# octree-nn/octfusion

Hardware: AMD Instinct MI355X
Metric: denoising-steps/sec (depth-8 octree, batch 8) (higher is better)
Workload: dtype f32 storage, fp16x3 products (fp16 hi + lo operand pairs = 22 significand bits, three fp16 MFMAs per product, fp32 accumulate)

## Files before the change

include/ofx.h:

```cpp
#ifndef OFX_H_
#define OFX_H_

#include <stddef.h>
#include <stdint.h>

#ifdef __cplusplus
extern "C" {
#endif

#define OFX_OK 0
#define OFX_EINVAL (-1)
#define OFX_ELAUNCH (-2)
#define OFX_ENODEV (-3)

#define OFX_ACT_NONE 0
#define OFX_ACT_SILU 1
#define OFX_ACT_GELU 2

#define OFX_MAX_DEPTH 16

int ofx_version(void);
const char* ofx_status_string(int status);
int ofx_device_check(void);
const char* ofx_build_hash(void);
// ... 58 lines not shown
int ofx_graph_reverse_count(const int32_t* seg_ptr, const int32_t* col, int64_t n_nodes, int32_t* rev_cnt,
                            void* stream);
int ofx_graph_reverse_fill(const int32_t* seg_ptr, const int32_t* col, int64_t n_nodes, const int32_t* rev_ptr,
                           int32_t* cursor, int32_t* rev_row, float* rev_w, void* stream);
int ofx_graph_primary_w(const int32_t* seg_ptr, const int32_t* col, const float* w, int64_t n_nodes, int32_t* nbr,
                        void* stream);
int ofx_graph_multi_flag_w(const int32_t* seg_ptr, const float* w, int64_t n_nodes, int32_t* flag, void* stream);
int ofx_graph_primary_ext_w(const int32_t* seg_ptr, const int32_t* col, const float* w, int64_t n_nodes,
                            const int32_t* rank, int32_t* nbr_ext, int32_t* multi_seg, void* stream);
int ofx_graphconv_bwd_data(const float* dy, int64_t ldy, int cout, int64_t n_nodes, const int32_t* nbr_rev,
                           const int32_t* rev_ptr, const int32_t* rev_row, const float* rev_w,
                           const int32_t* nbr_ext_rev, const int32_t* multi_seg, int64_t n_multi, float* aux,
                           const float* WpT, int64_t KpT, int cin, float* dx, int64_t ldx, void* ws, size_t ws_bytes,
                           void* stream);
int ofx_graphconv_bwd_weight(const float* x, int64_t ldx, int cin, int64_t n_nodes, const int32_t* nbr,
                             const int32_t* seg_ptr, const int32_t* col, const int32_t* nbr_ext,
                             const int32_t* multi_seg, int64_t n_multi, float* aux, const float* type_frac, int64_t ldt,
                             int nt_pad, const float* dy, int64_t ldy, int cout, float* dWp, int64_t Kp, void* ws,
                             size_t ws_bytes, void* stream);
int ofx_gn_backward(const float* x, int64_t ldx, const float* dy, int64_t ldy, int64_t n, int C,
                    const int32_t* batch_id, int batch_size, const float* count, int groups, float count_eps,
                    const float* mean, const float* rstd, const float* w, const float* bias, int act, double* sums,
                    float* coef, float* dx, int64_t lddx, float* dgamma, float* dbeta, void* stream);
int ofx_gemm_tn_f32(const float* P, int64_t ldp, const float* Q, int64_t ldq, int64_t rows, int64_t K, int64_t N,
                    float* out, void* ws, size_t ws_bytes, void* stream);
int ofx_table_reverse_count(const int32_t* nbr, int64_t n_out, int ndir, int64_t n_in, int32_t* rev_cnt, void* stream);
int ofx_table_reverse_fill(const int32_t* nbr, int64_t n_out, int ndir, int64_t n_in, const int32_t* rev_ptr,
                           int32_t* cursor, int32_t* rev_row, float* rev_w, void* stream);
int ofx_seg_primary_w(const int32_t* seg_ptr, const int32_t* col, const float* w, int64_t nseg, int32_t* nbr,
                      void* stream);
int ofx_seg_multi_flag_w(const int32_t* seg_ptr, const float* w, int64_t nseg, int32_t* flag, void* stream);
int ofx_seg_primary_ext_w(const int32_t* seg_ptr, const int32_t* col, const float* w, int64_t nseg, int64_t n_src,
                          const int32_t* rank, int32_t* nbr_ext, int32_t* multi_seg, void* stream);
int ofx_gridconv_bwd_data(const float* dy, int64_t ldy, int cout, int64_t n_out, int64_t n_in, const int32_t* nbr_rev,
                          const int32_t* rev_ptr, const int32_t* rev_row, const float* rev_w,
                          const int32_t* nbr_ext_rev, const int32_t* multi_seg, int64_t n_multi, float* aux,
                          const float* WpT, int cin, float* dx, int64_t ldx, void* ws, size_t ws_bytes, void* stream);
int ofx_gridconv_bwd_weight(const float* x, int64_t ldx, int cin, int64_t n_in, int64_t n_out, const int32_t* nbr27,
                            const int32_t* nbr27_ext, const float* zero_row, const float* dy, int64_t ldy, int cout,
                            float* dWp, void* ws, size_t ws_bytes, void* stream);
int ofx_adamw_step(float* param, const float* grad, float* exp_avg, float* exp_avg_sq, int64_t n, float lr,
                   float beta1, float beta2, float eps, float weight_decay, int step, void* stream);
int ofx_ema_update(float* ema, const float* param, int64_t n, float beta, void* stream);
int ofx_mpu_eval(const ofx_tree_t* tree, int depth_start, int depth_end, const float* pts, int64_t n_pts,
                 const float* code, float* sdf, uint8_t* mask, void* stream);
int ofx_mpu_eval_grid(const ofx_tree_t* tree, int depth_start, int depth_end, const float* code, int size,
                      float step, float bbmin, int batch_index, int64_t head, int64_t count, float* sdf,
                      uint8_t* mask, void* stream);
int ofx_mpu_eval_grad(const ofx_tree_t* tree, int depth_start, int depth_end, const float* pts, int64_t n_pts,
                      const float* code, float* sdf, float* grad, uint8_t* mask, void* stream);
int ofx_mpu_backward(const ofx_tree_t* tree, int depth_start, int depth_end, const float* pts, int64_t n_pts,
                     const float* code, const float* dsdf, const float* dgrad, float* dcode, void* stream);
int ofx_octree_ce(const float* logits, int64_t ld, const int32_t* child, int64_t n, float dscale, double* sums,
                  float* dlogits, int64_t ldd, void* stream);
int ofx_sdf_reg_loss(const float* sdf, const float* grad, const float* sdf_gt, const float* grad_gt, int64_t n,
                     float w_sdf, float w_grad, double* sums, float* dsdf, float* dgrad, void* stream);
int ofx_kl_sample_fwd(const float* params, int64_t ld, const float* noise, int64_t n, int embed_dim, float* z,
                      double* kl_sum, void* stream);
int ofx_kl_sample_bwd(const float* params, int64_t ld, const float* noise, const float* dz, int64_t n,
                      int embed_dim, float kl_scale, float* dparams, int64_t ldp, void* stream);
int ofx_graph_multi_flag(const int32_t* seg_ptr, int64_t n_nodes, int32_t* flag, void* stream);
int ofx_graph_primary_ext(const int32_t* seg_ptr, const int32_t* col, int64_t n_nodes,
                          const int32_t* rank, int32_t* nbr_ext, int32_t* multi_seg, void* stream);
int ofx_graph_type_frac(const int32_t* seg_ptr, const int32_t* col, const uint8_t* node_type,
                        int64_t n_nodes, int nt, float* type_frac, int64_t ld, void* stream);

int ofx_set_precision(int mode);
int ofx_get_precision(void);
int64_t ofx_packed_floats(int64_t Kp, int64_t N);
int64_t ofx_packed_k(int64_t K);
int64_t ofx_graphconv_packed_k(int cin, int nt);
int ofx_pack_weights(const float* W, int64_t sk, int64_t sn, int64_t K, int64_t N,
                     int cin, int nt, float* Wp, int64_t Kp, void* stream);

int ofx_gemm_f32(const float* A, int64_t lda, const int32_t* a_rows, int64_t M, int64_t K,
                 const float* Wp, int64_t Kp, int64_t N, const float* bias,
                 const float* res, int64_t ldr, float* out, int64_t ldc,
                 const int32_t* out_rows, void* ws, size_t ws_bytes, void* stream);
int ofx_gemm_f32_planes(const float* A, int64_t lda, const int32_t* a_rows, int64_t M, int64_t K,
                        const float* Wp, int64_t Kp, int64_t N, const float* bias,
                        const float* res, int64_t ldr, float* out, int64_t ldc,
                        const int32_t* out_rows, void* ws, size_t ws_bytes, int out_mode, void* stream);

int ofx_graphconv_fwd(const float* x, int64_t ldx, int cin, int64_t n_nodes,
                      const int32_t* nbr, const int32_t* seg_ptr, const int32_t* col,
                      const int32_t* nbr_ext, const int32_t* multi_seg, int64_t n_multi, float* aux,
                      const float* type_frac, int64_t ldt, int nt_pad,
                      const float* Wp, int64_t Kp, int cout, const float* bias,
                      const float* emb, int64_t lde, const int32_t* batch_id,
                      const float* res, int64_t ldr, float* out, int64_t ldc,
                      double* stats , int64_t stats_ld,
                      void* ws, size_t ws_bytes, void* stream);

int ofx_graphconv_narrow_in(const float* x, int64_t ldx, int cin, int64_t n_nodes, const int32_t* seg_ptr,
                            const int32_t* col, const uint8_t* node_type, int nt, const float* W, int cout,
                            const float* bias, const int32_t* batch_id, float* out, int64_t ldc,
                            double* stats , int64_t stats_ld, void* ws, size_t ws_bytes, void* stream);
int ofx_graphconv_narrow_in_tab(const float* x, int64_t ldx, int cin, int64_t n_nodes, const int32_t* seg_ptr,
                                const int32_t* col, const int32_t* nbr_ext, const int32_t* multi_seg, int64_t n_multi,
                                void* aux, const uint8_t* node_type, int nt, const float* W, int cout, const float* bias,
                                const int32_t* batch_id, float* out, int64_t ldc, double* stats ,
                                int64_t stats_ld, void* ws, size_t ws_bytes, void* stream);
int ofx_narrow_out_pack(const float* W, int C, int nt, int cout, int pw, float* Wd, void* stream);
int ofx_narrow_out_type_term(const float* type_frac, int64_t ldt, int nt, int64_t n_nodes, const float* W, int C,
                             int cout, const float* bias, float* type_term, void* stream);
int ofx_graphconv_narrow_out(const float* P, int64_t ldp, int cout, int64_t n_nodes, const int32_t* seg_ptr,
                             const int32_t* col, const float* type_term , float* out, int64_t ldc,
                             void* stream);

int ofx_planes_split(const float* x, int64_t ldx, int64_t n, int C, int Cpad, int mode, void* out,
                     int64_t ldo_bytes, void* stream);
int ofx_planes_merge(const void* planes, int64_t ldp_bytes, int64_t n, int C, int mode, float* out, int64_t ldo,
                     void* stream);
int ofx_gn_apply_planes(const float* x, int64_t ldx, int64_t n, int C, const int32_t* batch_id, const float* mean,
                        const float* rstd, const double* sums, const float* count, int groups, float eps,
                        float count_eps, const float* w, const float* bias, int act, int mode, void* out,
                        int64_t ldo_bytes, const int32_t* seg_ptr, const int32_t* col, const int32_t* multi_seg,
                        int64_t n_multi, void* aux , const int32_t* aux_plan ,
                        int64_t aux_left, void* stream);
int ofx_gn_apply_planes_oct(const float* x, int64_t ldx, int64_t n, int C, const int32_t* batch_id, const float* mean,
                            const float* rstd, const double* sums, const float* count, int groups, float eps,
                            float count_eps, const float* w, const float* bias, int act, int mode, void* out,
                            int64_t ldo_bytes, int64_t n_multi, void* aux, const int32_t* oct_ptr,
                            const int32_t* oct_ent, int64_t n_own, int shift, const int32_t* left_head,
                            const int32_t* left_src, int64_t n_left, void* stream);
int ofx_gn_apply_rows(void);
int64_t ofx_planes_packed_ktiles(int cin, int nt, int mode);
int64_t ofx_planes_packed_bytes(int cin, int nt, int cout, int mode);
int ofx_pack_weights_planes(const float* W, int64_t sk, int64_t sn, int cin, int nt, int cout, int mode, void* out,
                            void* stream);
int ofx_graphconv_fwd_planes(const void* xp, int64_t ldx_bytes, int cin, int64_t n_nodes, const int32_t* seg_ptr,
                             const int32_t* col, const int32_t* nbr_ext, const int32_t* multi_seg, int64_t n_multi,
                             void* aux, size_t aux_bytes, const void* tfp, int64_t ldt_bytes, int nt, const void* W2,
                             int cout, const float* bias, const float* emb, int64_t lde, const int32_t* batch_id,
                             const float* res, int64_t ldr, float* out, int64_t ldc, double* stats ,
                             int64_t stats_ld, void* ws, size_t ws_bytes, void* sync , size_t sync_bytes,
                             int mode, int aux_ready, void* stream);
int ofx_set_gconv_persistent(int on);
int64_t ofx_gemm_planes_packed_bytes(int K, int N, int mode);
int ofx_pack_gemm_planes(const float* W, int64_t sk, int64_t sn, int K, int N, int mode, void* out, void* stream);
int ofx_gemm_planes(const void* ap, int64_t lda_bytes, int64_t n_a, int64_t M, int K, const int32_t* row_tab,
                    const void* W2, int N, const float* bias, float* out, int64_t ldc, int out_mode, void* ws,
                    size_t ws_bytes, void* sync, size_t sync_bytes, int mode, void* stream);
int ofx_set_gconv_cus(int cus);
int ofx_gconv3_plan(int64_t n_rows, int cout, int nkt, int wm, int ni, int cus, int32_t* out, int64_t out_len);
int ofx_set_gconv2_tile(int wm);

int ofx_grid_conv_table(int mode, int depth_out, int batch_size, int32_t pad, int32_t* nbr27,
                        void* stream);
int64_t ofx_conv3d_packed_k(int cin);
int ofx_pack_conv3d(const float* W, int cin, int cout, float* Wp, void* stream);
int ofx_gridconv_fwd(const float* x, int64_t ldx, int cin, int64_t n_in, int64_t n_out,
                     const int32_t* nbr27 ,
                     const int32_t* nbr27_ext ,
                     const float* zero_row ,
                     const float* Wp, int cout, const float* bias, const float* emb, int64_t lde,
                     const int32_t* batch_id, const float* res, int64_t ldr, float* out,
                     int64_t ldc, void* ws, size_t ws_bytes, void* stream);
int ofx_gather_gemm_f32(const float* x, int64_t ldx, int cin, int ntap, int64_t n_src, int64_t n_out, const int32_t* tab,
                        const float* zero_row, const float* Wp, int64_t Kp, int cout, const float* bias,
                        const float* res, int64_t ldr, float* out, int64_t ldc, const int32_t* out_rows, void* ws,
                        size_t ws_bytes, int out_mode, void* stream);
int ofx_set_attention_split(int on);
int ofx_attention(const float* qkv, int64_t ldq, int batch_size, int T, int heads, int ch,
                  float* out, int64_t ldo, void* stream);

int ofx_attention_bwd(const float* qkv, int64_t ldq, const float* dout, int64_t ldo, int batch_size, int T, int heads,
                      int ch, float* rowstat, float* dqkv, int64_t ldd, void* stream);

int ofx_gather_mean(const float* x, int64_t ldx, int cin, int64_t n_nodes,
                    const int32_t* seg_ptr, const int32_t* col, float* col_data,
                    void* stream);

int ofx_gn_stats(const float* x, int64_t ldx, int64_t n, int C, const int32_t* batch_id,
                 int batch_size, double* sums, void* stream);
int ofx_gn_stats_acc(const float* x, int64_t ldx, int64_t n, int C, const int32_t* batch_id, int batch_size,
                     double* sums, void* stream);
int ofx_gn_finalize(const double* sums, const float* count, int batch_size, int C, int groups,
                    float eps, float count_eps, float* mean, float* rstd, void* stream);
int ofx_gn_apply(const float* x, int64_t ldx, int64_t n, int C, const int32_t* batch_id,
                 const float* mean , const float* rstd , const double* sums ,
                 const float* count, int groups, float eps, float count_eps, const float* w, const float* bias,
                 int act, float* out, int64_t ldo, void* stream);

int ofx_gn_fused_rows(const float* x, int64_t ldx, int rows_per_batch, int batch_size, int C, int groups, float eps,
                      float count_eps, const float* w, const float* bias, int act, float* out, int64_t ldo,
                      void* stream);

int ofx_set_gn_rows16(int on);

int ofx_rows_copy(const float* src, int64_t lds, const int32_t* smap, float* dst, int64_t ldd,
                  const int32_t* dmap, int64_t n, int C, void* stream);
int ofx_rows_copy_planes(const float* src, int64_t lds, const int32_t* smap, float* dst, int64_t ldd,
                         const int32_t* dmap, int64_t n, int C, int mode, void* stream);
int ofx_act(const float* x, float* y, int64_t n, int act, void* stream);
int ofx_timestep_embedding(const float* t, int batch_size, int dim, float max_period,
                           float* out, void* stream);
int ofx_learned_sinusoid(const float* t, const float* w, int batch_size, int half, float* out, void* stream);
int ofx_linear_small(const float* a, int64_t lda, int M, int K, const float* W, int64_t ldw, int N, const float* bias,
                     const float* res, int64_t ldr, int act_in, int act_out, float* out, int64_t ldo, void* stream);
int ofx_ddim_eps_update(float* x, const float* eps, const float* coef, float* x0_out, int64_t n,
                        void* stream);
int ofx_ddim_x0_update(float* x, const float* x0, const float* noise, const float* coef,
                       int64_t n, void* stream);

size_t ofx_mc_ws_bytes(int batch, int size);
int ofx_mc_count(const float* sdf, int batch, int size, float level, void* ws, int64_t* counts, void* stream);
int ofx_mc_emit(const float* sdf, int batch, int size, float level, float step, float bbmin, float scale, void* ws,
                const int64_t* vert_off, const int64_t* tri_off, float* verts, int32_t* faces, void* stream);
int ofx_mc_table_host(int8_t* tri_table, uint8_t* ntri);

size_t ofx_mesh_cc_ws_bytes(int64_t total_verts, int64_t total_faces, int batch);
int ofx_mesh_cc_label(const int32_t* faces, const int64_t* vert_off, const int64_t* tri_off, int batch,
                      int64_t total_verts, int64_t total_faces, int32_t* label, void* ws, int32_t* status,
                      void* stream);
int ofx_mesh_cc_table(const int32_t* faces, const int32_t* label, const int64_t* vert_off, const int64_t* tri_off,
                      int batch, int64_t total_verts, int64_t total_faces, int32_t* comp_of_vert, int32_t* comp_off,
                      void* ws, const int32_t* status, void* stream);
int ofx_mesh_cc_stats(const float* verts, const int32_t* faces, const int32_t* label, const int64_t* vert_off,
                      const int64_t* tri_off, int batch, int64_t total_verts, int64_t total_faces, int64_t n_comp,
                      int32_t* table, void* ws, const int32_t* status, void* stream);
int ofx_mesh_cc_select(const float* verts, const int32_t* faces, const int32_t* label, const int64_t* vert_off,
                       const int64_t* tri_off, int batch, int64_t total_verts, int64_t total_faces,
                       int32_t* winner_label, int64_t* keep_counts, void* ws, const int32_t* status, void* stream);
int ofx_mesh_cc_extract(const float* verts, const int32_t* faces, const int64_t* vert_off, const int64_t* tri_off,
                        int batch, int64_t total_verts, int64_t total_faces, const int64_t* new_vert_off,
                        const int64_t* new_tri_off, float* out_verts, int32_t* out_faces, void* ws,
                        const int32_t* status, void* stream);

#define OFX_EMD_MAX_POINTS 2048
size_t ofx_surface_sample_ws_bytes(int batch, int64_t total_faces);
int ofx_surface_sample(const float* verts, const int32_t* faces, const int64_t* offs, const int64_t* ids, int batch,
                       int64_t total_faces, int n, uint64_t seed, int normalize, void* ws, float* out, void* stream);
int ofx_nn_matrix(const float* a, int64_t na, int n, const float* b, int64_t nb, int m, float* d, void* stream);
int ofx_emd_matrix(const float* x, int64_t nx, const float* y, int64_t ny, int n, int m, float* e, void* stream);
uint64_t ofx_metrics_hash(uint64_t seed, int64_t shape, int64_t point, int draw);

#ifdef __cplusplus
}
#endif
#endif
// ... 1 lines not shown
```

octfusion_amd/_lib.py:

```python
import ctypes
import os

import torch

_HERE = os.path.dirname(os.path.abspath(__file__))
LIB_PATH = os.environ.get('OFX_LIB', os.path.join(_HERE, 'libofx.so'))

c_p = ctypes.c_void_p
c_i = ctypes.c_int
c_l = ctypes.c_int64
c_f = ctypes.c_float
c_sz = ctypes.c_size_t
c_u64 = ctypes.c_uint64


class OfxTree(ctypes.Structure):
    _fields_ = [('depth', c_i), ('full_depth', c_i), ('batch_size', c_i),
                ('child_all', c_p), ('key_all', c_p), ('leafrank_all', c_p),
                ('nnum_host', c_p), ('nnum_nempty_host', c_p)]


_SIGS = {
    'ofx_version': (c_i, [], False),
    'ofx_status_string': (ctypes.c_char_p, [c_i], False),
# ... 23 lines not shown
    'ofx_graph_reverse_count': (c_i, [c_p, c_p, c_l, c_p, c_p], True),
    'ofx_graph_reverse_fill': (c_i, [c_p, c_p, c_l, c_p, c_p, c_p, c_p, c_p], True),
    'ofx_graph_primary_w': (c_i, [c_p, c_p, c_p, c_l, c_p, c_p], True),
    'ofx_graph_multi_flag_w': (c_i, [c_p, c_p, c_l, c_p, c_p], True),
    'ofx_graph_primary_ext_w': (c_i, [c_p, c_p, c_p, c_l, c_p, c_p, c_p, c_p], True),
    'ofx_graphconv_bwd_data': (c_i, [c_p, c_l, c_i, c_l, c_p, c_p, c_p, c_p, c_p, c_p, c_l, c_p, c_p, c_l, c_i, c_p,
                                     c_l, c_p, c_sz, c_p], True),
    'ofx_graphconv_bwd_weight': (c_i, [c_p, c_l, c_i, c_l, c_p, c_p, c_p, c_p, c_p, c_l, c_p, c_p, c_l, c_i, c_p, c_l,
                                       c_i, c_p, c_l, c_p, c_sz, c_p], True),
    'ofx_gn_backward': (c_i, [c_p, c_l, c_p, c_l, c_l, c_i, c_p, c_i, c_p, c_i, c_f, c_p, c_p, c_p, c_p, c_i, c_p, c_p,
                              c_p, c_l, c_p, c_p, c_p], True),
    'ofx_gemm_tn_f32': (c_i, [c_p, c_l, c_p, c_l, c_l, c_l, c_l, c_p, c_p, c_sz, c_p], True),
    'ofx_table_reverse_count': (c_i, [c_p, c_l, c_i, c_l, c_p, c_p], True),
    'ofx_table_reverse_fill': (c_i, [c_p, c_l, c_i, c_l, c_p, c_p, c_p, c_p, c_p], True),
    'ofx_seg_primary_w': (c_i, [c_p, c_p, c_p, c_l, c_p, c_p], True),
    'ofx_seg_multi_flag_w': (c_i, [c_p, c_p, c_l, c_p, c_p], True),
    'ofx_seg_primary_ext_w': (c_i, [c_p, c_p, c_p, c_l, c_l, c_p, c_p, c_p, c_p], True),
    'ofx_gridconv_bwd_data': (c_i, [c_p, c_l, c_i, c_l, c_l, c_p, c_p, c_p, c_p, c_p, c_p, c_l, c_p, c_p, c_i, c_p, c_l,
                                    c_p, c_sz, c_p], True),
    'ofx_gridconv_bwd_weight': (c_i, [c_p, c_l, c_i, c_l, c_l, c_p, c_p, c_p, c_p, c_l, c_i, c_p, c_p, c_sz, c_p], True),
    'ofx_attention_bwd': (c_i, [c_p, c_l, c_p, c_l, c_i, c_i, c_i, c_i, c_p, c_p, c_l, c_p], True),
    'ofx_adamw_step': (c_i, [c_p, c_p, c_p, c_p, c_l, c_f, c_f, c_f, c_f, c_f, c_i, c_p], True),
    'ofx_ema_update': (c_i, [c_p, c_p, c_l, c_f, c_p], True),
    'ofx_gn_fused_rows': (c_i, [c_p, c_l, c_i, c_i, c_i, c_i, c_f, c_f, c_p, c_p, c_i, c_p, c_l, c_p], True),
    'ofx_set_gn_rows16': (c_i, [c_i], True),
    'ofx_mpu_eval': (c_i, [ctypes.POINTER(OfxTree), c_i, c_i, c_p, c_l, c_p, c_p, c_p, c_p], True),
    'ofx_mpu_eval_grid': (c_i, [ctypes.POINTER(OfxTree), c_i, c_i, c_p, c_i, c_f, c_f, c_i, c_l, c_l, c_p, c_p, c_p], True),
    'ofx_mpu_eval_grad': (c_i, [ctypes.POINTER(OfxTree), c_i, c_i, c_p, c_l, c_p, c_p, c_p, c_p, c_p], True),
    'ofx_mpu_backward': (c_i, [ctypes.POINTER(OfxTree), c_i, c_i, c_p, c_l, c_p, c_p, c_p, c_p, c_p], True),
    'ofx_octree_ce': (c_i, [c_p, c_l, c_p, c_l, c_f, c_p, c_p, c_l, c_p], True),
    'ofx_sdf_reg_loss': (c_i, [c_p, c_p, c_p, c_p, c_l, c_f, c_f, c_p, c_p, c_p, c_p], True),
    'ofx_kl_sample_fwd': (c_i, [c_p, c_l, c_p, c_l, c_i, c_p, c_p, c_p], True),
    'ofx_kl_sample_bwd': (c_i, [c_p, c_l, c_p, c_p, c_l, c_i, c_f, c_p, c_l, c_p], True),
    'ofx_graph_fill': (c_i, [ctypes.POINTER(OfxTree), c_i, c_p, c_p, c_p], True),
    'ofx_graph_expand': (c_i, [c_p, c_l, c_p, c_p, c_p, c_p, c_p], True),
    'ofx_graph_type_frac': (c_i, [c_p, c_p, c_p, c_l, c_i, c_p, c_l, c_p], True),
    'ofx_set_precision': (c_i, [c_i], True),
    'ofx_set_range_words': (c_i, [c_p], True),
    'ofx_get_precision': (c_i, [], False),
    'ofx_gn_apply_rows': (c_i, [], False),
    'ofx_set_attention_split': (c_i, [c_i], True),
    'ofx_gather_gemm_f32': (c_i, [c_p, c_l, c_i, c_i, c_l, c_l, c_p, c_p, c_p, c_l, c_i, c_p, c_p, c_l, c_p, c_l, c_p, c_p, c_sz, c_i, c_p], True),
    'ofx_graphconv_narrow_in_tab': (c_i, [c_p, c_l, c_i, c_l, c_p, c_p, c_p, c_p, c_l, c_p, c_p, c_i, c_p, c_i, c_p, c_p, c_p, c_l, c_p, c_l,
                                          c_p, c_sz, c_p], True),
    'ofx_graphconv_narrow_in': (c_i, [c_p, c_l, c_i, c_l, c_p, c_p, c_p, c_i, c_p, c_i, c_p, c_p, c_p, c_l, c_p, c_l, c_p, c_sz, c_p], True),
    'ofx_narrow_out_pack': (c_i, [c_p, c_i, c_i, c_i, c_i, c_p, c_p], True),
    'ofx_narrow_out_type_term': (c_i, [c_p, c_l, c_i, c_l, c_p, c_i, c_i, c_p, c_p, c_p], True),
    'ofx_graphconv_narrow_out': (c_i, [c_p, c_l, c_i, c_l, c_p, c_p, c_p, c_p, c_l, c_p], True),
    'ofx_packed_floats': (c_l, [c_l, c_l], False),
    'ofx_packed_k': (c_l, [c_l], False),
    'ofx_graphconv_packed_k': (c_l, [c_i, c_i], False),
    'ofx_pack_weights': (c_i, [c_p, c_l, c_l, c_l, c_l, c_i, c_i, c_p, c_l, c_p], True),
    'ofx_gemm_f32': (c_i, [c_p, c_l, c_p, c_l, c_l, c_p, c_l, c_l, c_p, c_p, c_l, c_p, c_l, c_p, c_p, c_sz, c_p], True),
    'ofx_gemm_f32_planes': (c_i, [c_p, c_l, c_p, c_l, c_l, c_p, c_l, c_l, c_p, c_p, c_l, c_p, c_l, c_p, c_p, c_sz, c_i, c_p], True),
    'ofx_graphconv_fwd': (c_i, [c_p, c_l, c_i, c_l, c_p, c_p, c_p, c_p, c_p, c_l, c_p, c_p, c_l, c_i, c_p, c_l,
                                c_i, c_p, c_p, c_l, c_p, c_p, c_l, c_p, c_l, c_p, c_l, c_p, c_sz, c_p], True),
    'ofx_planes_split': (c_i, [c_p, c_l, c_l, c_i, c_i, c_i, c_p, c_l, c_p], True),
    'ofx_planes_merge': (c_i, [c_p, c_l, c_l, c_i, c_i, c_p, c_l, c_p], True),
    'ofx_gn_apply_planes': (c_i, [c_p, c_l, c_l, c_i, c_p, c_p, c_p, c_p, c_p, c_i, c_f, c_f, c_p, c_p, c_i, c_i, c_p,
                                  c_l, c_p, c_p, c_p, c_l, c_p, c_p, c_l, c_p], True),
    'ofx_gn_apply_planes_oct': (c_i, [c_p, c_l, c_l, c_i, c_p, c_p, c_p, c_p, c_p, c_i, c_f, c_f, c_p, c_p, c_i, c_i, c_p,
                                      c_l, c_l, c_p, c_p, c_p, c_l, c_i, c_p, c_p, c_l, c_p], True),
    'ofx_planes_packed_ktiles': (c_l, [c_i, c_i, c_i], False),
    'ofx_planes_packed_bytes': (c_l, [c_i, c_i, c_i, c_i], False),
    'ofx_pack_weights_planes': (c_i, [c_p, c_l, c_l, c_i, c_i, c_i, c_i, c_p, c_p], True),
    'ofx_graphconv_fwd_planes': (c_i, [c_p, c_l, c_i, c_l, c_p, c_p, c_p, c_p, c_l, c_p, c_sz, c_p, c_l, c_i, c_p, c_i,
                                       c_p, c_p, c_l, c_p, c_p, c_l, c_p, c_l, c_p, c_l, c_p, c_sz, c_p, c_sz, c_i, c_i,
                                       c_p], True),
    'ofx_set_gconv_persistent': (c_i, [c_i], True),
    'ofx_set_gconv_cus': (c_i, [c_i], True),
    'ofx_gemm_planes_packed_bytes': (c_l, [c_i, c_i, c_i], False),
    'ofx_pack_gemm_planes': (c_i, [c_p, c_l, c_l, c_i, c_i, c_i, c_p, c_p], True),
    'ofx_gemm_planes': (c_i, [c_p, c_l, c_l, c_l, c_i, c_p, c_p, c_i, c_p, c_p, c_l, c_i, c_p, c_sz, c_p, c_sz, c_i, c_p], False),
    'ofx_gconv3_plan': (c_i, [c_l, c_i, c_i, c_i, c_i, c_i, c_p, c_l], False),
    'ofx_set_gconv2_tile': (c_i, [c_i], True),
    'ofx_graph_multi_flag': (c_i, [c_p, c_l, c_p, c_p], True),
    'ofx_graph_primary_ext': (c_i, [c_p, c_p, c_l, c_p, c_p, c_p, c_p], True),
    'ofx_graph_primary': (c_i, [c_p, c_p, c_l, c_p, c_p], True),
    'ofx_grid_conv_table': (c_i, [c_i, c_i, c_i, c_i, c_p, c_p], True),
    'ofx_conv3d_packed_k': (c_l, [c_i], False),
    'ofx_pack_conv3d': (c_i, [c_p, c_i, c_i, c_p, c_p], True),
    'ofx_gridconv_fwd': (c_i, [c_p, c_l, c_i, c_l, c_l, c_p, c_p, c_p, c_p, c_i, c_p, c_p, c_l, c_p, c_p, c_l, c_p,
                               c_l, c_p, c_sz, c_p], True),
    'ofx_attention': (c_i, [c_p, c_l, c_i, c_i, c_i, c_i, c_p, c_l, c_p], True),
    'ofx_gather_mean': (c_i, [c_p, c_l, c_i, c_l, c_p, c_p, c_p, c_p], True),
    'ofx_gn_stats': (c_i, [c_p, c_l, c_l, c_i, c_p, c_i, c_p, c_p], True),
    'ofx_gn_stats_acc': (c_i, [c_p, c_l, c_l, c_i, c_p, c_i, c_p, c_p], True),
    'ofx_gn_finalize': (c_i, [c_p, c_p, c_i, c_i, c_i, c_f, c_f, c_p, c_p, c_p], True),
    'ofx_gn_apply': (c_i, [c_p, c_l, c_l, c_i, c_p, c_p, c_p, c_p, c_p, c_i, c_f, c_f, c_p, c_p, c_i, c_p, c_l, c_p], True),
    'ofx_rows_copy': (c_i, [c_p, c_l, c_p, c_p, c_l, c_p, c_l, c_i, c_p], True),
    'ofx_rows_copy_planes': (c_i, [c_p, c_l, c_p, c_p, c_l, c_p, c_l, c_i, c_i, c_p], True),
    'ofx_act': (c_i, [c_p, c_p, c_l, c_i, c_p], True),
    'ofx_timestep_embedding': (c_i, [c_p, c_i, c_i, c_f, c_p, c_p], True),
    'ofx_learned_sinusoid': (c_i, [c_p, c_p, c_i, c_i, c_p, c_p], True),
    'ofx_linear_small': (c_i, [c_p, c_l, c_i, c_i, c_p, c_l, c_i, c_p, c_p, c_l, c_i, c_i, c_p, c_l, c_p], True),
    'ofx_ddim_eps_update': (c_i, [c_p, c_p, c_p, c_p, c_l, c_p], True),
    'ofx_ddim_x0_update': (c_i, [c_p, c_p, c_p, c_p, c_l, c_p], True),
    'ofx_mc_ws_bytes': (c_sz, [c_i, c_i], False),
    'ofx_mc_count': (c_i, [c_p, c_i, c_i, c_f, c_p, c_p, c_p], True),
    'ofx_mc_emit': (c_i, [c_p, c_i, c_i, c_f, c_f, c_f, c_f, c_p, c_p, c_p, c_p, c_p, c_p], True),
    'ofx_mc_table_host': (c_i, [c_p, c_p], True),
    'ofx_mesh_cc_ws_bytes': (c_sz, [c_l, c_l, c_i], False),
    'ofx_mesh_cc_label': (c_i, [c_p, c_p, c_p, c_i, c_l, c_l, c_p, c_p, c_p, c_p], True),
    'ofx_mesh_cc_table': (c_i, [c_p, c_p, c_p, c_p, c_i, c_l, c_l, c_p, c_p, c_p, c_p, c_p], True),
    'ofx_mesh_cc_stats': (c_i, [c_p, c_p, c_p, c_p, c_p, c_i, c_l, c_l, c_l, c_p, c_p, c_p, c_p], True),
    'ofx_mesh_cc_select': (c_i, [c_p, c_p, c_p, c_p, c_p, c_i, c_l, c_l, c_p, c_p, c_p, c_p, c_p], True),
    'ofx_mesh_cc_extract': (c_i, [c_p, c_p, c_p, c_p, c_i, c_l, c_l, c_p, c_p, c_p, c_p, c_p, c_p, c_p], True),
    'ofx_surface_sample_ws_bytes':(c_sz, [c_i, c_l], False),
    'ofx_surface_sample': (c_i, [c_p, c_p, c_p, c_p, c_i, c_l, c_i, c_u64, c_i, c_p, c_p, c_p], True),
    'ofx_nn_matrix': (c_i, [c_p, c_l, c_i, c_p, c_l, c_i, c_p, c_p], True),
    'ofx_emd_matrix': (c_i, [c_p, c_l, c_p, c_l, c_i, c_i, c_p, c_p], True),
    'ofx_metrics_hash': (c_u64, [c_u64, c_l, c_l, c_i], False),
}

EXPORTS = sorted(_SIGS)


class OfxError(RuntimeError):
    pass


_lib = None


def lib():
    global _lib
    if _lib is None:
        if not os.path.exists(LIB_PATH):
            raise OfxError('libofx.so not built: run `python -m octfusion_amd.build` '
                           '(the product has no CPU / eager fallback)')
        L = ctypes.CDLL(LIB_PATH)
        for name, (res, args, _) in _SIGS.items():
            fn = getattr(L, name)
            fn.restype = res
            fn.argtypes = args
        _check_fresh(L)
        _lib = L
    return _lib


def _check_fresh(L):
    if 'OFX_LIB' in os.environ:
        return
    from . import build
    try:
        want = build.source_hash()
    except OSError:
        return
    have = L.ofx_build_hash().decode()
    if have != want:
        raise OfxError('libofx.so is stale: built from sources %s, the tree is %s -- run `python -m octfusion_amd.build`'
                       % (have, want))


PROFILE = None
META = None


def _timed(prof, name, args, always):
    global META
    meta, META = META, None
    e0 = torch.cuda.Event(enable_timing=True)
    e1 = torch.cuda.Event(enable_timing=True)
    e0.record()
    rc = getattr(lib(), name)(*args)
    e1.record()
# ... 45 lines not shown
```

octfusion_amd/csrc/ofx_gemm.hip:

```cpp
#include "ofx_gemm_common.h"

constexpr int BM = 128;
constexpr int BK = 32;
constexpr int A_LD = BK + 4;
constexpr int MODE_DENSE = 0;
constexpr int MODE_GATHER = 1;


__device__ __forceinline__ float4 gather_seg4(const GemmArgs& g, int64_t row, int dir, int cc) {
  const int64_t s = row * g.ndir + dir;
  const int32_t a = g.seg_ptr[s], e = g.seg_ptr[s + 1];
  float4 acc = f4zero();
  if (g.edge_w) {
    for (int32_t p = a; p < e; ++p) {
      const float w = g.edge_w[p];
      const float4 v = *reinterpret_cast<const float4*>(g.x + (int64_t)g.col[p] * g.ldx + cc);
      acc.x += w * v.x; acc.y += w * v.y; acc.z += w * v.z; acc.w += w * v.w;
    }
    return acc;
  }
  for (int32_t p = a; p < e; ++p) f4add(acc, *reinterpret_cast<const float4*>(g.x + (int64_t)g.col[p] * g.ldx + cc));
  if (e - a > 1) {
    const float inv = 1.f / (float)(e - a);
    acc.x *= inv; acc.y *= inv; acc.z *= inv; acc.w *= inv;
  }
  return acc;
}

__device__ __forceinline__ float gather_elem(const GemmArgs& g, int64_t row, int64_t k) {
  if (k >= (int64_t)g.ndir * g.cin) return 0.f;
  const int dir = (int)(k / g.cin), c = (int)(k - (int64_t)dir * g.cin);
  const int32_t nb = g.nbr[row * g.ndir + dir];
  if (nb >= 0) return g.x[(int64_t)nb * g.ldx + c];
  if (nb == -1) return 0.f;
  const int64_t s = row * g.ndir + dir;
  const int32_t a = g.seg_ptr[s], e = g.seg_ptr[s + 1];
  float acc = 0.f;
  if (g.edge_w) {
    for (int32_t p = a; p < e; ++p) acc += g.edge_w[p] * g.x[(int64_t)g.col[p] * g.ldx + c];
    return acc;
  }
  for (int32_t p = a; p < e; ++p) acc += g.x[(int64_t)g.col[p] * g.ldx + c];
  if (e - a > 1) acc /= (float)(e - a);
  return acc;
}

__device__ __forceinline__ void load_a_dense(const GemmArgs& g, int64_t m0, int64_t k0, float4 (&va)[4]) {
  const int c4 = threadIdx.x & 7, r0 = threadIdx.x >> 3;
  const int64_t k = k0 + c4 * 4;
  const bool vec = ((g.lda & 3) == 0) && (k + 3 < g.K) && ((((uintptr_t)g.A) & 15) == 0);
#pragma unroll
  for (int i = 0; i < 4; ++i) {
    const int64_t m = m0 + r0 + 32 * i;
    float4 v = f4zero();
    if (m < g.M) {
      const int64_t ar = g.a_rows ? (int64_t)g.a_rows[m] : m;
      const float* p = g.A + ar * g.lda + k;
      if (vec) {
        v = *reinterpret_cast<const float4*>(p);
      } else {
        if (k + 0 < g.K) v.x = p[0];
        if (k + 1 < g.K) v.y = p[1];
        if (k + 2 < g.K) v.z = p[2];
        if (k + 3 < g.K) v.w = p[3];
      }
    }
    va[i] = v;
  }
}

template <int BN>
__device__ __forceinline__ void load_b_tile(const GemmArgs& g, int64_t n0, int64_t k0, float4 (&vb)[BN / 32]) {
#pragma unroll
  for (int i = 0; i < BN / 32; ++i) {
    const int idx = threadIdx.x + 256 * i;
    const int kql = idx / BN, n = idx % BN;
    const int64_t nn = n0 + n;
    vb[i] = (nn < g.N) ? *reinterpret_cast<const float4*>(g.Wp + (((k0 >> 2) + kql) * g.N + nn) * 4) : f4zero();
  }
}



// ... 341 lines not shown
      float* bs = b_st + (buf ^ 1) * 8 * BN * 4;
      *reinterpret_cast<float4*>(as) = va0;
      *reinterpret_cast<float4*>(as + 32 * A_LD) = va1;
      *reinterpret_cast<float4*>(as + 64 * A_LD) = va2;
      *reinterpret_cast<float4*>(as + 96 * A_LD) = va3;
      *reinterpret_cast<float4*>(bs) = vb0;
      if (NB > 1) *reinterpret_cast<float4*>(bs + 1024) = vb1;
      if (NB > 2) { *reinterpret_cast<float4*>(bs + 2048) = vb2; *reinterpret_cast<float4*>(bs + 3072) = vb3; }
      ia0 = ib0; ia1 = ib1; ia2 = ib2; ia3 = ib3;
      __syncthreads();
    }
  }

  for (int kt = t_begin; kt < kt_end; ++kt) {
    const int cc = (kt - nkt_g) * BK + c4 * 4;
    va0 = ldg4(tfp + m_0 * ldt + cc);
    va1 = ldg4(tfp + m_1 * ldt + cc);
    va2 = ldg4(tfp + m_2 * ldt + cc);
    va3 = ldg4(tfp + m_3 * ldt + cc);
    const gfp wk = wp + (int64_t)kt * 8 * Ncols * 4;
    vb0 = ldg4(wk + bo0);
    if (NB > 1) vb1 = ldg4(wk + bo1);
    if (NB > 2) { vb2 = ldg4(wk + bo2); vb3 = ldg4(wk + bo3); }
    *reinterpret_cast<float4*>(a_st) = va0;
    *reinterpret_cast<float4*>(a_st + 32 * A_LD) = va1;
    *reinterpret_cast<float4*>(a_st + 64 * A_LD) = va2;
    *reinterpret_cast<float4*>(a_st + 96 * A_LD) = va3;
    *reinterpret_cast<float4*>(b_st) = vb0;
    if (NB > 1) *reinterpret_cast<float4*>(b_st + 1024) = vb1;
    if (NB > 2) { *reinterpret_cast<float4*>(b_st + 2048) = vb2; *reinterpret_cast<float4*>(b_st + 3072) = vb3; }
    __syncthreads();
    mfma_tile<WM, WN, MI, NI>(a_ld, b_ld, acc);
    __syncthreads();
  }

  epilogue_store<WM, WN, MI, NI>(g, acc, m0, n0, wm, wn, l31, h, split);
}


typedef __bf16 bf16x8_t __attribute__((ext_vector_type(8)));
typedef _Float16 f16x8h_t __attribute__((ext_vector_type(8)));
typedef unsigned u32x4h __attribute__((ext_vector_type(4)));

__device__ __forceinline__ unsigned cvt_pk_bf16(float a, float b) {
  unsigned r;
  asm("v_cvt_pk_bf16_f32 %0, %1, %2" : "=v"(r) : "v"(a), "v"(b));
  return r;
}
__device__ __forceinline__ void split_bf16x4(const float4& v, uint2& hi, uint2& lo) {
  hi.x = cvt_pk_bf16(v.x, v.y);
  hi.y = cvt_pk_bf16(v.z, v.w);
  const float hx = __uint_as_float(hi.x << 16), hy = __uint_as_float(hi.x & 0xffff0000u);
  const float hz = __uint_as_float(hi.y << 16), hw = __uint_as_float(hi.y & 0xffff0000u);
  lo.x = cvt_pk_bf16(v.x - hx, v.y - hy);
  lo.y = cvt_pk_bf16(v.z - hz, v.w - hw);
}
__device__ __forceinline__ unsigned cvt_pk_f16(float a, float b) {
  const _Float16 x = (_Float16)a, y = (_Float16)b;
  return (unsigned)__builtin_bit_cast(unsigned short, x) | ((unsigned)__builtin_bit_cast(unsigned short, y) << 16);
}
__device__ __forceinline__ float f16_lo_f32(unsigned p) { return (float)__builtin_bit_cast(_Float16, (unsigned short)(p & 0xffffu)); }
__device__ __forceinline__ float f16_hi_f32(unsigned p) { return (float)__builtin_bit_cast(_Float16, (unsigned short)(p >> 16)); }
__device__ __forceinline__ float sat_f16(float v) { return fminf(fmaxf(v, -65504.f), 65504.f); }
template <int H16>
__device__ __forceinline__ void split16x4(const float4& v, uint2& hi, uint2& lo) {
  if constexpr (H16 == 0) {
    split_bf16x4(v, hi, lo);
  } else {
    const float x = v.x, y = v.y, z = v.z, w = v.w;
    hi.x = cvt_pk_f16(x, y);
    hi.y = cvt_pk_f16(z, w);
    lo.x = cvt_pk_f16(x - f16_lo_f32(hi.x), y - f16_hi_f32(hi.x));
    lo.y = cvt_pk_f16(z - f16_lo_f32(hi.y), w - f16_hi_f32(hi.y));
  }
}
template <int H16>
__device__ __forceinline__ f32x16 mfma16(u32x4h a, u32x4h b, f32x16 c) {
  if constexpr (H16 == 0)
    return __builtin_amdgcn_mfma_f32_32x32x16_bf16(__builtin_bit_cast(bf16x8_t, a), __builtin_bit_cast(bf16x8_t, b), c, 0, 0, 0);
  else
    return __builtin_amdgcn_mfma_f32_32x32x16_f16(__builtin_bit_cast(f16x8h_t, a), __builtin_bit_cast(f16x8h_t, b), c, 0, 0, 0);
}

template <int MODE, int WM, int WN, int MI, int NI, int H16>
__global__ void __launch_bounds__(256, 2) gemm_pairs_x3_kernel(const GemmArgs g) {
  constexpr int BN = WN * NI * 32;
  constexpr int A_BYTES = BM * 80;
  constexpr int BUF_BYTES = 2 * A_BYTES;
  static_assert(WM * MI * 32 == BM, "BM");
  extern __shared__ __attribute__((aligned(16))) char smem8[];
  typedef unsigned u32x4 __attribute__((ext_vector_type(4)));
  typedef const u32x4 __attribute__((address_space(1)))* gqp;

  const int ntile = g.ntm * g.ntn;
  const int nblk = ntile * g.nsplit;
  int bid = blockIdx.x;
  {
    const int q = nblk / 8, r = nblk % 8, xcd = bid % 8, j = bid / 8;
    bid = (xcd < r ? xcd * (q + 1) : r * (q + 1) + (xcd - r) * q) + j;
  }
  const int split = bid / ntile;
  bid -= split * ntile;
  const int tm = bid / g.ntn, tn = bid - tm * g.ntn;
  const int64_t m0 = (int64_t)tm * BM, n0 = (int64_t)tn * BN;

  const int lane = threadIdx.x & 63, wid = threadIdx.x >> 6;
  const int wm = wid / WN, wn = wid % WN;
  const int l31 = lane & 31, h = lane >> 5;
  const int c4 = threadIdx.x & 7;
  const int r0 = ((threadIdx.x >> 4) & 3) + 8 * (threadIdx.x >> 6) + 4 * ((threadIdx.x >> 3) & 1);

  const gfp xp = (gfp)sgpr64((uint64_t)(MODE == MODE_DENSE ? g.A : g.x));
  const gfp tfp = (gfp)sgpr64((uint64_t)g.tf);
  const gqp w16 = (gqp)sgpr64((uint64_t)g.W16);
  const gip tab = (gip)sgpr64((uint64_t)g.nbr_ext);
  const int64_t ldx = (int64_t)sgpr64((uint64_t)(MODE == MODE_DENSE ? g.lda : g.ldx));
  const int64_t ldt = (int64_t)sgpr64((uint64_t)g.ldt), n_src = (int64_t)sgpr64((uint64_t)g.n_src);
  const int64_t Ncols = (int64_t)sgpr64((uint64_t)g.N);
  const int64_t lo_off = (int64_t)sgpr64((uint64_t)(g.Kp / 8 * g.N));
  const int64_t aux_delta = (int64_t)sgpr64((uint64_t)((g.aux - g.x) - g.n_src * g.ldx));
  const int ndir = g.ndir;

  f32x16 acc[MI][NI];
#pragma unroll
  for (int i = 0; i < MI; ++i)
#pragma unroll
    for (int j = 0; j < NI; ++j)
#pragma unroll
      for (int r = 0; r < 16; ++r) acc[i][j][r] = 0.f;

  const int nkt_all = (int)(g.Kp / BK);
  const int kt_begin = split * g.kt_per_split;
  const int kt_end = (kt_begin + g.kt_per_split < nkt_all) ? kt_begin + g.kt_per_split : nkt_all;
  const int tpd = MODE == MODE_DENSE ? nkt_all : g.cin / BK;
  const int nkt_g = MODE == MODE_DENSE ? nkt_all : ndir * tpd;
  const int g_begin = kt_begin < nkt_g ? kt_begin : nkt_g;
  const int g_end = kt_end < nkt_g ? kt_end : nkt_g;
  const int t_begin = kt_begin > nkt_g ? kt_begin : nkt_g;

  int64_t m_0 = m0 + r0, m_1 = m_0 + 32, m_2 = m_0 + 64, m_3 = m_0 + 96;
  const int64_t mmax = g.M - 1;
  m_0 = m_0 < mmax ? m_0 : mmax; m_1 = m_1 < mmax ? m_1 : mmax;
  m_2 = m_2 < mmax ? m_2 : mmax; m_3 = m_3 < mmax ? m_3 : mmax;
  const gip t0 = tab + m_0 * ndir;
  const gip t1 = tab + m_1 * ndir;
  const gip t2 = tab + m_2 * ndir;
  const gip t3 = tab + m_3 * ndir;
  int64_t dr0 = m_0, dr1 = m_1, dr2 = m_2, dr3 = m_3;
  if (MODE == MODE_DENSE && g.a_rows) { dr0 = g.a_rows[m_0]; dr1 = g.a_rows[m_1]; dr2 = g.a_rows[m_2]; dr3 = g.a_rows[m_3]; }
  const gfp dp0 = xp + dr0 * ldx, dp1 = xp + dr1 * ldx, dp2 = xp + dr2 * ldx, dp3 = xp + dr3 * ldx;
  const int kclamp = (int)g.K - 4;

  int64_t bcol[NI];
#pragma unroll
  for (int j = 0; j < NI; ++j) {
    int64_t nn = n0 + (wn * NI + j) * 32 + l31;
    bcol[j] = (nn < Ncols ? nn : Ncols - 1) + (int64_t)h * Ncols;
  }
  char* const a_st = smem8 + (r0 * 80 + c4 * 8);
  const char* const a_ld = smem8 + ((wm * MI * 32 + l31) * 80 + 16 * h);

  struct BFrag { u32x4 h[2][NI], l[2][NI]; };
  struct RegSet { float4 a0, a1, a2, a3; };
  struct IdxSet { uint32_t i0, i1, i2, i3; };

  auto load_bfrag = [&](int ktw, BFrag& F) {
    const gqp wk = w16 + (int64_t)ktw * 4 * Ncols;
#pragma unroll
    for (int c = 0; c < 2; ++c)
#pragma unroll
      for (int j = 0; j < NI; ++j) {
        F.h[c][j] = wk[(int64_t)(2 * c) * Ncols + bcol[j]];
        F.l[c][j] = wk[lo_off + (int64_t)(2 * c) * Ncols + bcol[j]];
      }
  };
  auto store_a = [&](int buf, const RegSet& R) {
    char* a = a_st + buf * BUF_BYTES;
    uint2 hi, lo;
    split16x4<H16>(R.a0, hi, lo);
    *reinterpret_cast<uint2*>(a) = hi; *reinterpret_cast<uint2*>(a + A_BYTES) = lo;
    split16x4<H16>(R.a1, hi, lo);
    *reinterpret_cast<uint2*>(a + 32 * 80) = hi; *reinterpret_cast<uint2*>(a + 32 * 80 + A_BYTES) = lo;
    split16x4<H16>(R.a2, hi, lo);
    *reinterpret_cast<uint2*>(a + 64 * 80) = hi; *reinterpret_cast<uint2*>(a + 64 * 80 + A_BYTES) = lo;
    split16x4<H16>(R.a3, hi, lo);
    *reinterpret_cast<uint2*>(a + 96 * 80) = hi; *reinterpret_cast<uint2*>(a + 96 * 80 + A_BYTES) = lo;
  };
  auto compute = [&](int buf, const BFrag& F) {
    const char* a = a_ld + buf * BUF_BYTES;
    u32x4h ah[2][MI], al[2][MI];
#pragma unroll
    for (int c = 0; c < 2; ++c)
#pragma unroll
      for (int i = 0; i < MI; ++i) {
        ah[c][i] = *reinterpret_cast<const u32x4h*>(a + i * 32 * 80 + 32 * c);
        al[c][i] = *reinterpret_cast<const u32x4h*>(a + i * 32 * 80 + 32 * c + A_BYTES);
      }
#pragma unroll
    for (int c = 0; c < 2; ++c) {
#pragma unroll
      for (int i = 0; i < MI; ++i)
#pragma unroll
        for (int j = 0; j < NI; ++j)
          acc[i][j] = mfma16<H16>(al[c][i], F.h[c][j], acc[i][j]);
#pragma unroll
      for (int i = 0; i < MI; ++i)
#pragma unroll
        for (int j = 0; j < NI; ++j)
          acc[i][j] = mfma16<H16>(ah[c][i], F.l[c][j], acc[i][j]);
#pragma unroll
      for (int i = 0; i < MI; ++i)
#pragma unroll
        for (int j = 0; j < NI; ++j)
          acc[i][j] = mfma16<H16>(ah[c][i], F.h[c][j], acc[i][j]);
    }
  };

  if (g_begin < g_end) {
    RegSet R0, R1;
    IdxSet I0 = {0, 0, 0, 0}, I1 = {0, 0, 0, 0};
    BFrag F0, F1;
    auto clampg = [&](int it) { return it < nkt_g ? it : nkt_g - 1; };
    auto ktw_of = [&](int it) {
      const int itc = clampg(it);
      return MODE == MODE_DENSE ? itc : (itc % ndir) * tpd + itc / ndir;
    };
    auto load_idx = [&](int it, IdxSet& I) {
      if (MODE == MODE_DENSE) return;
      const int dc = clampg(it) % ndir;
      I.i0 = (uint32_t)t0[dc]; I.i1 = (uint32_t)t1[dc]; I.i2 = (uint32_t)t2[dc]; I.i3 = (uint32_t)t3[dc];
    };
    auto load_rows = [&](int it, const IdxSet& I, RegSet& R) {
      const int itc = clampg(it);
      if (MODE == MODE_DENSE) {
        int cc = itc * BK + c4 * 4;
        cc = cc < kclamp ? cc : kclamp;
        R.a0 = ldg4(dp0 + cc); R.a1 = ldg4(dp1 + cc); R.a2 = ldg4(dp2 + cc); R.a3 = ldg4(dp3 + cc);
      } else {
        const int cc = (itc / ndir) * BK + c4 * 4;
        R.a0 = ldg4(xp + src_off(I.i0, ldx, n_src, aux_delta) + cc);
        R.a1 = ldg4(xp + src_off(I.i1, ldx, n_src, aux_delta) + cc);
        R.a2 = ldg4(xp + src_off(I.i2, ldx, n_src, aux_delta) + cc);
        R.a3 = ldg4(xp + src_off(I.i3, ldx, n_src, aux_delta) + cc);
      }
    };
    auto load_bchunk = [&](int ktw, int c, BFrag& F) {
      const gqp wk = w16 + (int64_t)ktw * 4 * Ncols + (int64_t)(2 * c) * Ncols;
#pragma unroll
      for (int j = 0; j < NI; ++j) { F.h[c][j] = wk[bcol[j]]; F.l[c][j] = wk[lo_off + bcol[j]]; }
    };
    auto store_half = [&](int buf, const float4& v0, const float4& v1, int row_off) {
      char* a = a_st + buf * BUF_BYTES + row_off * 80;
      uint2 hi, lo;
      split16x4<H16>(v0, hi, lo);
      *reinterpret_cast<uint2*>(a) = hi; *reinterpret_cast<uint2*>(a + A_BYTES) = lo;
      split16x4<H16>(v1, hi, lo);
      *reinterpret_cast<uint2*>(a + 32 * 80) = hi; *reinterpret_cast<uint2*>(a + 32 * 80 + A_BYTES) = lo;
    };
#define OFX_FENCE() __builtin_amdgcn_sched_barrier(0)
    auto step = [&](int it, int buf, const IdxSet& Iuse, IdxSet& Iload, const BFrag& Fcur, BFrag& Fnext,
                    RegSet& Rnew, const RegSet& Rold) {
      const char* a = a_ld + buf * BUF_BYTES;
      const int ktw = ktw_of(it + 1);
      u32x4h ah[2][MI], al[2][MI];
#pragma unroll
      for (int c = 0; c < 2; ++c)
#pragma unroll
        for (int i = 0; i < MI; ++i) {
          ah[c][i] = *reinterpret_cast<const u32x4h*>(a + i * 32 * 80 + 32 * c);
          al[c][i] = *reinterpret_cast<const u32x4h*>(a + i * 32 * 80 + 32 * c + A_BYTES);
        }
      load_idx(it + 3, Iload);
      OFX_FENCE();
#define OFX_MFMA_GROUP(AOP, BOP, C)                                                                        \
      _Pragma("unroll") for (int i = 0; i < MI; ++i)                                                        \
        _Pragma("unroll") for (int j = 0; j < NI; ++j)                                                      \
          acc[i][j] = mfma16<H16>(AOP[C][i], Fcur.BOP[C][j], acc[i][j]);
      OFX_MFMA_GROUP(al, h, 0);
      OFX_FENCE();
      load_bchunk(ktw, 0, Fnext);
      OFX_FENCE();
      OFX_MFMA_GROUP(ah, l, 0);
      OFX_FENCE();
      load_bchunk(ktw, 1, Fnext);
      OFX_FENCE();
      OFX_MFMA_GROUP(ah, h, 0);
      OFX_FENCE();
      load_rows(it + 2, Iuse, Rnew);
      OFX_FENCE();
      OFX_MFMA_GROUP(al, h, 1);
      OFX_FENCE();
      store_half(buf ^ 1, Rold.a0, Rold.a1, 0);
      OFX_FENCE();
      OFX_MFMA_GROUP(ah, l, 1);
      OFX_FENCE();
      store_half(buf ^ 1, Rold.a2, Rold.a3, 64);
      OFX_FENCE();
      OFX_MFMA_GROUP(ah, h, 1);
#undef OFX_MFMA_GROUP
      __syncthreads();
    };

    load_idx(g_begin, I0);
    load_idx(g_begin + 1, I1);
    OFX_FENCE();
    load_rows(g_begin, I0, R0);
    load_bchunk(ktw_of(g_begin), 0, F0);
    load_bchunk(ktw_of(g_begin), 1, F0);
    OFX_FENCE();
    load_idx(g_begin + 2, I0);
    OFX_FENCE();
    load_rows(g_begin + 1, I1, R1);
    OFX_FENCE();
    store_half(0, R0.a0, R0.a1, 0);
    store_half(0, R0.a2, R0.a3, 64);
    __syncthreads();
    int it = g_begin;
    for (; it + 1 < g_end; it += 2) {
      step(it, 0, I0, I1, F0, F1, R0, R1);
      step(it + 1, 1, I1, I0, F1, F0, R1, R0);
    }
    if (it < g_end) step(it, 0, I0, I1, F0, F1, R0, R1);
    __syncthreads();
#undef OFX_FENCE
  }

  for (int kt = t_begin; kt < kt_end; ++kt) {
    const int cc = (kt - nkt_g) * BK + c4 * 4;
    RegSet R;
    BFrag F;
    R.a0 = ldg4(tfp + m_0 * ldt + cc);
    R.a1 = ldg4(tfp + m_1 * ldt + cc);
    R.a2 = ldg4(tfp + m_2 * ldt + cc);
    R.a3 = ldg4(tfp + m_3 * ldt + cc);
    load_bfrag(kt, F);
    store_a(0, R);
    __syncthreads();
    compute(0, F);
    __syncthreads();
  }

  epilogue_store<WM, WN, MI, NI>(g, acc, m0, n0, wm, wn, l31, h, split);
}

__device__ __forceinline__ uint32_t bf16_rne_bits(float f) {
  const uint32_t u = __float_as_uint(f);
  return (u + 0x7fffu + ((u >> 16) & 1u)) >> 16;
}
__global__ void pack_bf16x3_kernel(const float* __restrict__ Wp, int64_t Kp, int64_t N, uint16_t* __restrict__ W16,
                                   int h16) {
  const int64_t total = Kp * N;
  const float wscale = h16 ? reinterpret_cast<const float*>(W16 + 2 * total)[1] : 1.f;
  for (int64_t t = (int64_t)blockIdx.x * blockDim.x + threadIdx.x; t < total; t += (int64_t)gridDim.x * blockDim.x) {
    const int64_t kg = t / (N * 8), rem = t - kg * N * 8;
    const int64_t n = rem / 8;
    const int kk = (int)(rem - n * 8);
    const int64_t k = kg * 8 + kk;
    const float w = Wp[((k >> 2) * N + n) * 4 + (k & 3)];
    if (h16) {
      const float ws = sat_f16(w * wscale);
      const _Float16 hi = (_Float16)ws;
      const _Float16 lo = (_Float16)(ws - (float)hi);
      W16[t] = __builtin_bit_cast(unsigned short, hi);
      W16[total + t] = __builtin_bit_cast(unsigned short, lo);
    } else {
      const uint32_t hi = bf16_rne_bits(w);
      const float wl = w - __uint_as_float(hi << 16);
      W16[t] = (uint16_t)hi;
      W16[total + t] = (uint16_t)bf16_rne_bits(wl);
    }
  }
}
static int g_precision = 3;
static int pack_bf16x3(const float* Wp, int64_t Kp, int64_t N, hipStream_t st) {
  uint16_t* W16 = reinterpret_cast<uint16_t*>(const_cast<float*>(Wp) + Kp * N);
  if (ofx_launch_weight_scale(Wp, 1, 0, Kp * N, 1, g_precision == 3 ? 1 : 0, const_cast<float*>(Wp) + 2 * Kp * N, st))
    return OFX_ELAUNCH;
  pack_bf16x3_kernel<<<ofx_grid(Kp * N, 256), 256, 0, st>>>(Wp, Kp, N, W16, g_precision == 3 ? 1 : 0);
  return hipGetLastError() == hipSuccess ? OFX_OK : OFX_ELAUNCH;
}

extern "C" int ofx_set_precision(int mode) {
  if (mode < 0 || mode > 3) return OFX_EINVAL;
  g_precision = mode;
  return OFX_OK;
}
extern "C" int ofx_get_precision(void) { return g_precision; }
extern "C" int64_t ofx_packed_floats(int64_t Kp, int64_t N) { return 2 * Kp * N + 32; }

__global__ void __launch_bounds__(256) multi_mean_kernel(const float* __restrict__ x, int64_t ldx, int cin,
                                                         const int32_t* __restrict__ seg_ptr,
                                                         const int32_t* __restrict__ col,
                                                         const int32_t* __restrict__ multi_seg, int64_t V,
                                                         float* __restrict__ aux, int64_t ldaux,
                                                         const float* __restrict__ w) {
  const int c4n = cin >> 2;
  const int64_t total = (V + 1) * c4n;
  for (int64_t t = (int64_t)blockIdx.x * blockDim.x + threadIdx.x; t < total; t += (int64_t)gridDim.x * blockDim.x) {
// ... 27 lines not shown
    for (int s = 0; s < g.nsplit; ++s) v += g.ws[(int64_t)s * total + t];
    if (g.oscale_p) v *= *g.oscale_p;
    if (g.bias) v += g.bias[n];
    if (g.emb) v += g.emb[(int64_t)g.bid[m] * g.lde + n];
    if (g.res) v += g.res[m * g.ldr + n];
    int64_t om = m;
    if (g.out_rows) { om = g.out_rows[m]; if (om < 0) continue; }
    g.out[om * g.ldc + n] = v;
  }
}

__global__ void __launch_bounds__(256) splitk_reduce_v4_kernel(const GemmArgs g) {
  const int64_t n4 = g.N >> 2, total4 = g.M * n4, total = g.M * g.N;
  for (int64_t t = (int64_t)blockIdx.x * blockDim.x + threadIdx.x; t < total4; t += (int64_t)gridDim.x * blockDim.x) {
    const int64_t m = t / n4, n = (t - m * n4) * 4;
    const float* p = g.ws + m * g.N + n;
    float4 v = f4zero();
    int s = 0;
    for (; s + 7 < g.nsplit; s += 8) {
      float4 a[8];
#pragma unroll
      for (int u = 0; u < 8; ++u) a[u] = *reinterpret_cast<const float4*>(p + (int64_t)(s + u) * total);
#pragma unroll
      for (int u = 0; u < 8; ++u) f4add(v, a[u]);
    }
    for (; s + 3 < g.nsplit; s += 4) {
      const float4 a0 = *reinterpret_cast<const float4*>(p + (int64_t)s * total);
      const float4 a1 = *reinterpret_cast<const float4*>(p + (int64_t)(s + 1) * total);
      const float4 a2 = *reinterpret_cast<const float4*>(p + (int64_t)(s + 2) * total);
      const float4 a3 = *reinterpret_cast<const float4*>(p + (int64_t)(s + 3) * total);
      f4add(v, a0); f4add(v, a1); f4add(v, a2); f4add(v, a3);
    }
    for (; s < g.nsplit; ++s) f4add(v, *reinterpret_cast<const float4*>(p + (int64_t)s * total));
    if (g.oscale_p) { const float osc = *g.oscale_p; v.x *= osc; v.y *= osc; v.z *= osc; v.w *= osc; }
    if (g.bias) f4add(v, *reinterpret_cast<const float4*>(g.bias + n));
    if (g.emb) f4add(v, *reinterpret_cast<const float4*>(g.emb + (int64_t)g.bid[m] * g.lde + n));
    if (g.res) f4add(v, *reinterpret_cast<const float4*>(g.res + m * g.ldr + n));
    int64_t om = m;
    if (g.out_rows) { om = g.out_rows[m]; if (om < 0) continue; }
    if (g.out_planes) ofx_store_planes4(g.out, om * g.ldc + n, v, g.out_planes);
    else *reinterpret_cast<float4*>(g.out + om * g.ldc + n) = v;
  }
}

template <int MODE, int WM, int WN, int MI, int NI>
static int launch_cfg(GemmArgs& g, hipStream_t st) {
  constexpr int BN = WN * NI * 32;
  constexpr size_t lds = (2 * BM * A_LD + 2 * 8 * BN * 4) * sizeof(float);
  static bool attr_set[OFX_MAX_DEVICES] = {};
  if (lds > 64 * 1024 &&
      !ofx_raise_lds_limit(reinterpret_cast<const void*>(&gemm_kernel<MODE, WM, WN, MI, NI>), (int)lds, attr_set))
    return OFX_ELAUNCH;
  gemm_kernel<MODE, WM, WN, MI, NI><<<g.ntm * g.ntn * g.nsplit, 256, lds, st>>>(g);
  return OFX_OK;
}

template <int MODE, int WM, int WN, int MI, int NI>
static int launch_fast_cfg(GemmArgs& g, hipStream_t st) {
  constexpr int BN = WN * NI * 32;
  constexpr size_t lds = (2 * BM * A_LD + 2 * 8 * BN * 4) * sizeof(float);
  static bool attr_set[OFX_MAX_DEVICES] = {};
  if (lds > 64 * 1024 &&
      !ofx_raise_lds_limit(reinterpret_cast<const void*>(&gemm_fast_kernel<MODE, WM, WN, MI, NI>), (int)lds, attr_set))
    return OFX_ELAUNCH;
  gemm_fast_kernel<MODE, WM, WN, MI, NI><<<g.ntm * g.ntn * g.nsplit, 256, lds, st>>>(g);
  return OFX_OK;
}

template <int MODE, int WM, int WN, int MI, int NI, int H16>
static int launch_bf16x3_h(GemmArgs& g, hipStream_t st) {
  constexpr int BN = WN * NI * 32;
  constexpr size_t lds = 2 * (2 * BM * 80);
  static bool attr_set[OFX_MAX_DEVICES] = {};
  if (lds > 64 * 1024 &&
      !ofx_raise_lds_limit(reinterpret_cast<const void*>(&gemm_pairs_x3_kernel<MODE, WM, WN, MI, NI, H16>), (int)lds, attr_set))
    return OFX_ELAUNCH;
  gemm_pairs_x3_kernel<MODE, WM, WN, MI, NI, H16><<<g.ntm * g.ntn * g.nsplit, 256, lds, st>>>(g);
  return OFX_OK;
}
template <int MODE, int WM, int WN, int MI, int NI>
static int launch_bf16x3_cfg(GemmArgs& g, hipStream_t st) {
  return g_precision == 3 ? launch_bf16x3_h<MODE, WM, WN, MI, NI, 1>(g, st) : launch_bf16x3_h<MODE, WM, WN, MI, NI, 0>(g, st);
}

__global__ void __launch_bounds__(256) stats_reduce_kernel(const float* __restrict__ part, int64_t nwr, int wr_rows,
                                                            int64_t N, const int32_t* __restrict__ bid,
                                                            double* __restrict__ stats, int64_t stats_ld) {
  __shared__ double red[3][64][2];
  const int c = threadIdx.x & 63, rg = threadIdx.x >> 6;
  const int64_t n = (int64_t)blockIdx.y * 64 + c;
  const int64_t w0 = (int64_t)blockIdx.x * 64;
  const int64_t nc = n < N ? n : N - 1;
  int b[16];
  float2 v[16];
#pragma unroll
  for (int i = 0; i < 16; ++i) {
    const int64_t w = w0 + rg * 16 + i;
    const int64_t wc = w < nwr ? w : nwr - 1;
    b[i] = bid[wc * wr_rows];
    v[i] = *reinterpret_cast<const float2*>(part + (wc * N + nc) * 2);
    if (w >= nwr) { b[i] = -1; v[i] = make_float2(0.f, 0.f); }
  }
  const int bfirst = bid[w0 * wr_rows];
  bool ok = true;
#pragma unroll
  for (int i = 0; i < 16; ++i) ok = ok && (b[i] == bfirst || b[i] < 0);
  const bool uni = __syncthreads_and(ok);
  auto flush = [&](int bb, double s, double q) {
    double* o = stats + ((int64_t)bb * stats_ld + n) * 2;
    unsafeAtomicAdd(o, s); unsafeAtomicAdd(o + 1, q);
  };
  if (uni) {
    double s = 0.0, q = 0.0;
#pragma unroll
    for (int i = 0; i < 16; ++i) { s += (double)v[i].x; q += (double)v[i].y; }
    if (rg > 0) { red[rg - 1][c][0] = s; red[rg - 1][c][1] = q; }
    __syncthreads();
    if (rg == 0 && n < N) {
#pragma unroll
      for (int r = 0; r < 3; ++r) { s += red[r][c][0]; q += red[r][c][1]; }
      flush(bfirst, s, q);
    }
  } else if (n < N) {
    double s = 0.0, q = 0.0;
    int sb = -1;
#pragma unroll
    for (int i = 0; i < 16; ++i) {
      if (b[i] < 0) continue;
      if (b[i] != sb) {
        if (sb >= 0) flush(sb, s, q);
        sb = b[i]; s = 0.0; q = 0.0;
      }
      s += (double)v[i].x; q += (double)v[i].y;
    }
    if (sb >= 0) flush(sb, s, q);
  }
}

int ofx_launch_stats_reduce(const GemmArgs& g, int wr_rows, hipStream_t st) {
  const int64_t nwr = ofx_cdiv(g.M, wr_rows);
  stats_reduce_kernel<<<dim3((unsigned)ofx_cdiv(nwr, 64), (unsigned)ofx_cdiv(g.N, 64)), 256, 0, st>>>(
      g.stats_part, nwr, wr_rows, g.N, g.bid, g.stats, g.stats_ld);
  OFX_LAUNCH_CHECK();
  return OFX_OK;
}

template <int MODE>
static int launch_gemm(GemmArgs& g, float* ws, size_t ws_bytes, hipStream_t st) {
  if (g.M <= 0 || g.N <= 0) return OFX_OK;
  {
    auto al16 = [](const void* p) { return (reinterpret_cast<uintptr_t>(p) & 15) == 0; };
    g.vec4 = g.N % 4 == 0 && al16(g.out) && g.ldc % 4 == 0 && (!g.res || (al16(g.res) && g.ldr % 4 == 0)) &&
             (!g.emb || (al16(g.emb) && g.lde % 4 == 0)) && (!g.bias || al16(g.bias));
  }
  const int bn = g.N <= 32 ? 32 : (g.N <= 64 ? 64 : 128);
  g.ntm = (int)ofx_cdiv(g.M, BM);
  g.ntn = (int)ofx_cdiv(g.N, bn);
  const int nkt = (int)(g.Kp / BK);
  int nsplit = 1;
  const int tiles = g.ntm * g.ntn;
  if (ws && tiles < 256 && nkt >= 8) {
    nsplit = (int)ofx_cdiv(512, tiles);
    if (nsplit > nkt / 4) nsplit = nkt / 4;
    if (nsplit > 64) nsplit = 64;
    const size_t per = (size_t)g.M * g.N * sizeof(float);
    if ((size_t)nsplit * per > ws_bytes) nsplit = (int)(ws_bytes / per);
    if (nsplit < 2) nsplit = 1;
  }
  g.kt_per_split = (int)ofx_cdiv(nkt, nsplit);
  nsplit = (int)ofx_cdiv(nkt, g.kt_per_split);
  g.nsplit = nsplit;
  g.ws = ws;
  int rc;
  bool fast;
  if (MODE == MODE_GATHER) {
    fast = g.fast && g.nbr_ext && g.aux && (!g.out_rows || g.gather_out_rows);
  } else {
    fast = ((g.lda & 3) == 0) && ((g.K & 3) == 0) && g.K >= 4 && ((((uintptr_t)g.A) & 15) == 0);
    if (fast) { g.ndir = 1; g.n_src = 0; g.aux = g.A; g.tf = g.A; g.ldt = g.lda; g.nbr_ext = (const int32_t*)g.A; }
  }
  g.W16 = (g_precision != 1) ? reinterpret_cast<const uint16_t*>(g.Wp + g.Kp * g.N) : nullptr;
  const int wr_rows = bn == 32 ? 32 : 64;
  const int64_t nwr = ofx_cdiv(g.M, wr_rows);
  if (!(g.stats && g.vec4 && nsplit == 1 && g.stats_part &&
        (size_t)nwr * g.N * 2 * sizeof(float) <= g.stats_part_bytes && (((uintptr_t)g.stats_part) & 15) == 0))
    g.stats_part = nullptr;
  g.oscale_p = (fast && g.W16) ? g.Wp + 2 * g.Kp * g.N : nullptr;
  if (fast && g.W16) {
    if (bn == 32) rc = launch_bf16x3_cfg<MODE, 4, 1, 1, 1>(g, st);
    else if (bn == 64) rc = launch_bf16x3_cfg<MODE, 2, 2, 2, 1>(g, st);
    else rc = launch_bf16x3_cfg<MODE, 2, 2, 2, 2>(g, st);
  } else if (fast) {
    if (bn == 32) rc = launch_fast_cfg<MODE, 4, 1, 1, 1>(g, st);
    else if (bn == 64) rc = launch_fast_cfg<MODE, 2, 2, 2, 1>(g, st);
    else rc = launch_fast_cfg<MODE, 2, 2, 2, 2>(g, st);
  } else if (bn == 32) rc = launch_cfg<MODE, 4, 1, 1, 1>(g, st);
  else if (bn == 64) rc = launch_cfg<MODE, 2, 2, 2, 1>(g, st);
  else rc = launch_cfg<MODE, 2, 2, 2, 2>(g, st);
  if (rc) return rc;
  if (nsplit > 1) {
    const bool ws16 = (((uintptr_t)g.ws) & 15) == 0;
    if (g.vec4 && ws16) splitk_reduce_v4_kernel<<<ofx_grid(g.M * (g.N >> 2), 256), 256, 0, st>>>(g);
    else splitk_reduce_kernel<<<ofx_grid(g.M * g.N, 256), 256, 0, st>>>(g);
  }
  if (g.stats_part) {
    rc = ofx_launch_stats_reduce(g, wr_rows, st);
    if (rc) return rc;
  }
  OFX_LAUNCH_CHECK();
  return OFX_OK;
}

static inline int64_t pad32(int64_t v) { return (v + 31) / 32 * 32; }
static int pack_bf16x3(const float* Wp, int64_t Kp, int64_t N, hipStream_t st);

extern "C" int64_t ofx_packed_k(int64_t K) { return pad32(K); }
extern "C" int64_t ofx_graphconv_packed_k(int cin, int nt) {
  return pad32(7 * (int64_t)cin) + (nt > 1 ? pad32(7 * (int64_t)nt) : 0);
}

__global__ void pack_weights_kernel(const float* __restrict__ W, int64_t sk, int64_t sn, int64_t K, int64_t N, int cin,
                                    int nt, float* __restrict__ Wp, int64_t Kp) {
  const int64_t total = (Kp / 4) * N;
  const int ntc = nt > 1 ? nt : 0;
  const int64_t Kf = (7 * (int64_t)cin + 31) / 32 * 32;
  for (int64_t t = (int64_t)blockIdx.x * blockDim.x + threadIdx.x; t < total; t += (int64_t)gridDim.x * blockDim.x) {
    const int64_t kq = t / N, n = t - kq * N;
    float v[4];
#pragma unroll
    for (int kk = 0; kk < 4; ++kk) {
      const int64_t k = kq * 4 + kk;
      int64_t src = -1;
      if (cin > 0) {
        if (k < 7 * (int64_t)cin) {
          const int64_t dir = k / cin, c = k - dir * cin;
          src = dir * (cin + ntc) + c;
        } else if (k >= Kf && ntc > 0 && k - Kf < 7 * (int64_t)ntc) {
          const int64_t kt = k - Kf, dir = kt / ntc, ty = kt - dir * ntc;
          src = dir * (cin + ntc) + cin + ty;
        }
      } else if (k < K) {
        src = k;
      }
      v[kk] = src >= 0 ? W[src * sk + n * sn] : 0.f;
    }
    *reinterpret_cast<float4*>(Wp + t * 4) = make_float4(v[0], v[1], v[2], v[3]);
  }
}

extern "C" int ofx_pack_weights(const float* W, int64_t sk, int64_t sn, int64_t K, int64_t N, int cin, int nt,
                                float* Wp, int64_t Kp, void* stream) {
  if (!W || !Wp || K < 1 || N < 1 || (Kp & 31) || cin < 0 || nt < 0) return OFX_EINVAL;
  if (cin > 0) {
    if (Kp != ofx_graphconv_packed_k(cin, nt) || K != 7 * (int64_t)(cin + (nt > 1 ? nt : 0))) return OFX_EINVAL;
  } else if (Kp != pad32(K)) {
    return OFX_EINVAL;
  }
  if (((uintptr_t)Wp & 15) != 0) return OFX_EINVAL;
  pack_weights_kernel<<<ofx_grid((Kp / 4) * N, 256), 256, 0, ofx_stream(stream)>>>(W, sk, sn, K, N, cin, nt, Wp, Kp);
  if (int rc = pack_bf16x3(Wp, Kp, N, ofx_stream(stream))) return rc;
  OFX_LAUNCH_CHECK();
  return OFX_OK;
}

__global__ void pack_conv3d_kernel(const float* __restrict__ W, int cin, int64_t N, float* __restrict__ Wp, int64_t Kp) {
  const int64_t total = (Kp / 4) * N;
  for (int64_t t = (int64_t)blockIdx.x * blockDim.x + threadIdx.x; t < total; t += (int64_t)gridDim.x * blockDim.x) {
    const int64_t kq = t / N, n = t - kq * N;
    float v[4];
#pragma unroll
    for (int kk = 0; kk < 4; ++kk) {
      const int64_t k = kq * 4 + kk;
      float w = 0.f;
      if (k < 27 * (int64_t)cin) {
        const int64_t tap = k / cin, c = k - tap * cin;
        w = W[(n * cin + c) * 27 + tap];
      }
      v[kk] = w;
    }
    *reinterpret_cast<float4*>(Wp + t * 4) = make_float4(v[0], v[1], v[2], v[3]);
  }
}

extern "C" int64_t ofx_conv3d_packed_k(int cin) { return pad32(27 * (int64_t)cin); }

extern "C" int ofx_pack_conv3d(const float* W, int cin, int cout, float* Wp, void* stream) {
  if (!W || !Wp || cin < 1 || cout < 1 || ((uintptr_t)Wp & 15)) return OFX_EINVAL;
  const int64_t Kp = ofx_conv3d_packed_k(cin);
  pack_conv3d_kernel<<<ofx_grid((Kp / 4) * cout, 256), 256, 0, ofx_stream(stream)>>>(W, cin, cout, Wp, Kp);
  if (int rc = pack_bf16x3(Wp, Kp, cout, ofx_stream(stream))) return rc;
  OFX_LAUNCH_CHECK();
  return OFX_OK;
}

extern "C" int ofx_gemm_f32_planes(const float* A, int64_t lda, const int32_t* a_rows, int64_t M, int64_t K,
                                   const float* Wp, int64_t Kp, int64_t N, const float* bias, const float* res, int64_t ldr,
                                   float* out, int64_t ldc, const int32_t* out_rows, void* ws, size_t ws_bytes,
                                   int out_mode, void* stream) {
  if (M == 0 && K >= 1 && N >= 1) return OFX_OK;
  if (M < 0 || K < 1 || N < 1 || !Wp || !out || (M > 0 && !A) || Kp != pad32(K) || lda < K || ldc < N ||
      (res && ldr < N) || ((uintptr_t)Wp & 15))
    return OFX_EINVAL;
  if (out_mode != 0 && out_mode != 2 && out_mode != 3) return OFX_EINVAL;
  if (out_mode && ((N & 3) || (ldc & 31) || ((uintptr_t)out & 127) || (res && ((ldr & 3) || ((uintptr_t)res & 15))) ||
                   (bias && ((uintptr_t)bias & 15)) || ((uintptr_t)ws & 15)))
    return OFX_EINVAL;
  GemmArgs g = {};
  g.A = A; g.lda = lda; g.a_rows = a_rows;
  g.M = M; g.K = K; g.Wp = Wp; g.Kp = Kp; g.N = N; g.bias = bias;
  g.res = res; g.ldr = ldr; g.out = out; g.ldc = ldc; g.out_rows = out_rows; g.out_planes = out_mode;
  return launch_gemm<MODE_DENSE>(g, (float*)ws, ws_bytes, ofx_stream(stream));
}
extern "C" int ofx_gemm_f32(const float* A, int64_t lda, const int32_t* a_rows, int64_t M, int64_t K, const float* Wp,
                            int64_t Kp, int64_t N, const float* bias, const float* res, int64_t ldr, float* out,
                            int64_t ldc, const int32_t* out_rows, void* ws, size_t ws_bytes, void* stream) {
  return ofx_gemm_f32_planes(A, lda, a_rows, M, K, Wp, Kp, N, bias, res, ldr, out, ldc, out_rows, ws, ws_bytes, 0, stream);
}

static int gather_common(GemmArgs& g, const float* x, int64_t ldx, int cin, int ndir, int64_t n_rows,
                         const int32_t* nbr, const int32_t* seg_ptr, const int32_t* col, const float* Wp, int64_t Kp,
                         int cout, const float* bias, const float* emb, int64_t lde, const int32_t* batch_id,
                         const float* res, int64_t ldr, float* out, int64_t ldc) {
  if (n_rows < 0 || cin < 1 || cout < 1 || !x || !nbr || !Wp || !out || ldx < cin || ldc < cout ||
      (res && ldr < cout) || (emb && (!batch_id || lde < cout)) || ((uintptr_t)Wp & 15))
    return OFX_EINVAL;
  g.x = x; g.ldx = ldx; g.cin = cin; g.ndir = ndir;
  g.fast = (cin % 32 == 0) && ((ldx & 3) == 0) && (((uintptr_t)x & 15) == 0);
  g.nbr = nbr; g.seg_ptr = seg_ptr; g.col = col;
  g.Kf = pad32((int64_t)ndir * cin);
  g.M = n_rows; g.K = Kp; g.Wp = Wp; g.Kp = Kp; g.N = cout; g.bias = bias;
  g.emb = emb; g.lde = lde; g.bid = batch_id; g.res = res; g.ldr = ldr; g.out = out; g.ldc = ldc;
  return OFX_OK;
}

__global__ void __launch_bounds__(256) col_rows_kernel(const GemmArgs g, int64_t row0, int64_t rows,
                                                       float* __restrict__ colbuf) {
  const int64_t k4n = g.Kp >> 2, total = rows * k4n;
  for (int64_t t = (int64_t)blockIdx.x * blockDim.x + threadIdx.x; t < total; t += (int64_t)gridDim.x * blockDim.x) {
    const int64_t r = t / k4n, k = (t - r * k4n) * 4;
    const int64_t row = row0 + r;
    float v[4];
#pragma unroll
    for (int kk = 0; kk < 4; ++kk)
      v[kk] = (k + kk < g.Kf) ? gather_elem(g, row, k + kk) : g.tf[row * g.ldt + (k + kk - g.Kf)];
    *reinterpret_cast<float4*>(colbuf + t * 4) = make_float4(v[0], v[1], v[2], v[3]);
  }
}

template <int MODE> static int launch_gemm(GemmArgs& g, float* ws, size_t ws_bytes, hipStream_t st);

static int launch_gather_via_col(const GemmArgs& g, float* ws, size_t ws_bytes, hipStream_t st) {
  if (!ws || (((uintptr_t)ws) & 15)) return -1;
  size_t tail = ws_bytes / 8;
  if (tail > (size_t(16) << 20)) tail = size_t(16) << 20;
  tail &= ~size_t(15);
  const size_t row_bytes = (size_t)g.Kp * sizeof(float);
  int64_t chunk = (int64_t)((ws_bytes - tail) / row_bytes) / 128 * 128;
  if (chunk < 128) return -1;
  float* tail_ws = reinterpret_cast<float*>(reinterpret_cast<char*>(ws) + (ws_bytes - tail));
  for (int64_t r0 = 0; r0 < g.M; r0 += chunk) {
    const int64_t rows = g.M - r0 < chunk ? g.M - r0 : chunk;
    col_rows_kernel<<<ofx_grid(rows * (g.Kp >> 2), 256), 256, 0, st>>>(g, r0, rows, ws);
    GemmArgs d = {};
    d.A = ws; d.lda = g.Kp; d.M = rows; d.K = g.Kp; d.Wp = g.Wp; d.Kp = g.Kp; d.N = g.N; d.bias = g.bias;
    d.emb = g.emb; d.lde = g.lde; d.bid = g.bid ? g.bid + r0 : nullptr;
    d.res = g.res ? g.res + r0 * g.ldr : nullptr; d.ldr = g.ldr;
    d.out = g.out + r0 * g.ldc; d.ldc = g.ldc;
    d.stats = g.stats; d.stats_ld = g.stats_ld;
    if (g.stats) { d.stats_part = tail_ws; d.stats_part_bytes = tail; }
    const int rc = launch_gemm<MODE_DENSE>(d, g.stats ? nullptr : tail_ws, tail, st);
    if (rc) return rc;
  }
  return OFX_OK;
}

extern "C" int ofx_graphconv_fwd(const float* x, int64_t ldx, int cin, int64_t n_nodes, const int32_t* nbr,
                                 const int32_t* seg_ptr, const int32_t* col, const int32_t* nbr_ext,
                                 const int32_t* multi_seg, int64_t n_multi, float* aux, const float* type_frac,
                                 int64_t ldt, int nt_pad, const float* Wp, int64_t Kp, int cout, const float* bias,
                                 const float* emb, int64_t lde, const int32_t* batch_id, const float* res, int64_t ldr,
                                 float* out, int64_t ldc, double* stats, int64_t stats_ld, void* ws, size_t ws_bytes,
                                 void* stream) {
  if (n_nodes == 0 && cin >= 1 && cout >= 1) return OFX_OK;
  GemmArgs g = {};
  int rc = gather_common(g, x, ldx, cin, 7, n_nodes, nbr, seg_ptr, col, Wp, Kp, cout, bias, emb, lde, batch_id, res,
                         ldr, out, ldc);
  if (rc) return rc;
  if (!seg_ptr || !col) return OFX_EINVAL;
  if (nt_pad < 0 || (nt_pad & 31) || Kp != g.Kf + nt_pad) return OFX_EINVAL;
  if (nt_pad > 0 && (!type_frac || ldt < nt_pad || (ldt & 3) || ((uintptr_t)type_frac & 15))) return OFX_EINVAL;
  g.tf = type_frac; g.ldt = ldt;
  if (stats) {
    if (!batch_id || stats_ld < cout) return OFX_EINVAL;
    g.stats = stats; g.stats_ld = stats_ld; g.bid = batch_id;
    g.stats_part = (float*)ws; g.stats_part_bytes = ws_bytes;
    ws = nullptr;
  }
  hipStream_t st = ofx_stream(stream);
  if (g.fast && nbr_ext && aux && n_nodes > 0 && (((uintptr_t)aux & 15) == 0)) {
    if (n_multi < 0 || (n_multi > 0 && !multi_seg)) return OFX_EINVAL;
    multi_mean_kernel<<<ofx_grid((n_multi + 1) * (cin / 4), 256), 256, 0, st>>>(x, ldx, cin, seg_ptr, col, multi_seg,
                                                                               n_multi, aux, ldx, nullptr);
    g.nbr_ext = nbr_ext; g.aux = aux; g.ldaux = ldx; g.n_src = n_nodes;
    if (!g.tf) { g.tf = x; g.ldt = ldx; }
  }
  if (!g.nbr_ext && n_nodes > 0) {
    rc = launch_gather_via_col(g, stats ? g.stats_part : (float*)ws, stats ? g.stats_part_bytes : ws_bytes, st);
    if (rc >= 0) return rc;
  }
  return launch_gemm<MODE_GATHER>(g, (float*)ws, ws_bytes, st);
}

extern "C" int ofx_graphconv_bwd_data(const float* dy, int64_t ldy, int cout, int64_t n_nodes, const int32_t* nbr_rev,
                                      const int32_t* rev_ptr, const int32_t* rev_row, const float* rev_w,
                                      const int32_t* nbr_ext_rev, const int32_t* multi_seg, int64_t n_multi, float* aux,
                                      const float* WpT, int64_t KpT, int cin, float* dx, int64_t ldx, void* ws,
                                      size_t ws_bytes, void* stream) {
  if (n_nodes == 0 && cin >= 1 && cout >= 1) return OFX_OK;
  GemmArgs g = {};
  int rc = gather_common(g, dy, ldy, cout, 7, n_nodes, nbr_rev, rev_ptr, rev_row, WpT, KpT, cin, nullptr, nullptr, 0,
                         nullptr, nullptr, 0, dx, ldx);
  if (rc) return rc;
  if (!rev_ptr || !rev_row || !rev_w || KpT != g.Kf) return OFX_EINVAL;
  g.edge_w = rev_w;
  hipStream_t st = ofx_stream(stream);
  if (g.fast && nbr_ext_rev && aux && (((uintptr_t)aux & 15) == 0)) {
    if (n_multi < 0 || (n_multi > 0 && !multi_seg)) return OFX_EINVAL;
    multi_mean_kernel<<<ofx_grid((n_multi + 1) * (cout / 4), 256), 256, 0, st>>>(dy, ldy, cout, rev_ptr, rev_row,
                                                                                multi_seg, n_multi, aux, ldy, rev_w);
    g.nbr_ext = nbr_ext_rev; g.aux = aux; g.ldaux = ldy; g.n_src = n_nodes;
    g.tf = dy; g.ldt = ldy;
  } else {
// ... 294 lines not shown
    OFX_LAUNCH_CHECK();
    return OFX_OK;
  }
  if (!nbr27) return OFX_EINVAL;
  GemmArgs g = {};
  g.x = x; g.ldx = ldx; g.cin = cin; g.ndir = 27; g.nbr = nbr27; g.tf = x; g.ldt = ldx; g.Kf = Kp; g.Kp = Kp; g.M = n_out;
  int slices = (int)ofx_cdiv(512, tiles);
  if (slices > 64) slices = 64;
  const size_t part_bytes = ((size_t)slices * total * sizeof(float) + 255) & ~size_t(255);
  if (part_bytes >= ws_bytes) return OFX_EINVAL;
  int64_t chunk = (int64_t)((ws_bytes - part_bytes) / ((size_t)Kp * sizeof(float))) / 32 * 32;
  if (chunk < 32) return OFX_EINVAL;
  float* colbuf = reinterpret_cast<float*>(reinterpret_cast<char*>(ws) + part_bytes);
  a.P = colbuf; a.ldp = Kp;
  int first = 1;
  for (int64_t r0 = 0; r0 < n_out; r0 += chunk) {
    const int64_t rows = n_out - r0 < chunk ? n_out - r0 : chunk;
    col_rows_kernel<<<ofx_grid(rows * (Kp >> 2), 256), 256, 0, st>>>(g, r0, rows, colbuf);
    a.Q = dy + r0 * ldy; a.rows = rows; a.row0 = r0;
    a.rows_per_slice = ofx_cdiv(ofx_cdiv(rows, slices), 32) * 32;
    const int sl = (int)ofx_cdiv(rows, a.rows_per_slice);
    launch_tn<true>(a, dim3((unsigned)ofx_cdiv(Kp, 128), (unsigned)ofx_cdiv(cout, 128), (unsigned)sl), st);
    tn_reduce_kernel<<<ofx_grid(total, 256), 256, 0, st>>>(a.part, sl, total, dWp, first ? 0 : 1);
    first = 0;
  }
  OFX_LAUNCH_CHECK();
  return OFX_OK;
}

extern "C" int ofx_gemm_tn_f32(const float* P, int64_t ldp, const float* Q, int64_t ldq, int64_t rows, int64_t K,
                               int64_t N, float* out, void* ws, size_t ws_bytes, void* stream) {
  if (rows < 0 || K < 4 || N < 4 || (K & 3) || (N & 3) || !out || !ws || ldp < K || ldq < N || ((ldp | ldq) & 3) ||
      (rows > 0 && (!P || !Q)) || (((uintptr_t)P | (uintptr_t)Q | (uintptr_t)ws) & 15))
    return OFX_EINVAL;
  hipStream_t st = ofx_stream(stream);
  const int64_t total = K * N;
  if (rows == 0) {
    if (hipMemsetAsync(out, 0, (size_t)total * sizeof(float), st) != hipSuccess) return OFX_ELAUNCH;
    return OFX_OK;
  }
  const int tiles = (int)(ofx_cdiv(K, 128) * ofx_cdiv(N, 128));
  int slices = (int)ofx_cdiv(1024, tiles);
  if (slices > 256) slices = 256;
  if (slices > (int)ofx_cdiv(rows, 32)) slices = (int)ofx_cdiv(rows, 32);
  while (slices > 1 && (size_t)slices * total * sizeof(float) > ws_bytes) --slices;
  if ((size_t)slices * total * sizeof(float) > ws_bytes) return OFX_EINVAL;
  TnArgs a = {};
  a.P = P; a.ldp = ldp; a.Q = Q; a.ldq = ldq; a.Kp = K; a.N = N; a.Kf = K; a.rows = rows; a.row0 = 0;
  a.rows_per_slice = ofx_cdiv(ofx_cdiv(rows, slices), 32) * 32;
  slices = (int)ofx_cdiv(rows, a.rows_per_slice);
  a.part = (float*)ws;
  launch_tn<true>(a, dim3((unsigned)ofx_cdiv(K, 128), (unsigned)ofx_cdiv(N, 128), (unsigned)slices), st);
  tn_reduce_kernel<<<ofx_grid(total, 256), 256, 0, st>>>(a.part, slices, total, out, 0);
  OFX_LAUNCH_CHECK();
  return OFX_OK;
}

extern "C" int ofx_gridconv_fwd(const float* x, int64_t ldx, int cin, int64_t n_in, int64_t n_out,
                                const int32_t* nbr27, const int32_t* nbr27_ext, const float* zero_row,
                                const float* Wp, int cout,
                                const float* bias, const float* emb, int64_t lde, const int32_t* batch_id,
                                const float* res, int64_t ldr, float* out, int64_t ldc, void* ws, size_t ws_bytes,
                                void* stream) {
  if (n_out == 0 && cin >= 1 && cout >= 1) return OFX_OK;
  GemmArgs g = {};
  const int64_t Kp = ofx_conv3d_packed_k(cin);
  int rc = gather_common(g, x, ldx, cin, 27, n_out, nbr27 ? nbr27 : nbr27_ext, nullptr, nullptr, Wp, Kp, cout, bias,
                         emb, lde, batch_id, res, ldr, out, ldc);
  if (rc) return rc;
  if (n_in < 1) return OFX_EINVAL;
  if (g.fast && nbr27_ext && zero_row && (((uintptr_t)zero_row & 15) == 0)) {
    g.nbr_ext = nbr27_ext; g.aux = zero_row; g.ldaux = ldx; g.n_src = n_in;
    g.tf = x; g.ldt = ldx;
  } else if (!nbr27) {
    return OFX_EINVAL;
  }
  if (!g.nbr_ext) {
    rc = launch_gather_via_col(g, (float*)ws, ws_bytes, ofx_stream(stream));
    if (rc >= 0) return rc;
  }
  return launch_gemm<MODE_GATHER>(g, (float*)ws, ws_bytes, ofx_stream(stream));
}

extern "C" int ofx_gather_gemm_f32(const float* x, int64_t ldx, int cin, int ntap, int64_t n_src, int64_t n_out,
                                   const int32_t* tab, const float* zero_row, const float* Wp, int64_t Kp, int cout,
                                   const float* bias, const float* res, int64_t ldr, float* out, int64_t ldc,
                                   const int32_t* out_rows, void* ws, size_t ws_bytes, int out_mode, void* stream) {
  if (n_out == 0 && cin >= 1 && cout >= 1) return OFX_OK;
  if (ntap < 1 || ntap > 64 || n_src < 1 || !tab || !zero_row || ((uintptr_t)zero_row & 15) || (cin & 31) || (ldx & 3) ||
      ((uintptr_t)x & 15) || Kp != pad32((int64_t)ntap * cin))
    return OFX_EINVAL;
  if (out_mode != 0 && out_mode != 2 && out_mode != 3) return OFX_EINVAL;
  if (out_mode && ((cout & 3) || (ldc & 31) || ((uintptr_t)out & 127) || (res && ((ldr & 3) || ((uintptr_t)res & 15))) ||
                   (bias && ((uintptr_t)bias & 15)) || ((uintptr_t)ws & 15)))
    return OFX_EINVAL;
  GemmArgs g = {};
  int rc = gather_common(g, x, ldx, cin, ntap, n_out, tab, nullptr, nullptr, Wp, Kp, cout, bias, nullptr, 0, nullptr, res,
                         ldr, out, ldc);
  if (rc) return rc;
  if (!g.fast) return OFX_EINVAL;
  g.nbr_ext = tab; g.aux = zero_row; g.ldaux = ldx; g.n_src = n_src;
  g.tf = x; g.ldt = ldx;
  g.out_rows = out_rows; g.gather_out_rows = 1; g.out_planes = out_mode;
  return launch_gemm<MODE_GATHER>(g, (float*)ws, ws_bytes, ofx_stream(stream));
}

__global__ void __launch_bounds__(256) gather_mean_kernel(const float* __restrict__ x, int64_t ldx, int cin, int64_t nseg,
                                                          const int32_t* __restrict__ seg_ptr,
                                                          const int32_t* __restrict__ col, float* __restrict__ out) {
  const int c4n = cin >> 2;
  const int64_t total = nseg * c4n;
  for (int64_t t = (int64_t)blockIdx.x * blockDim.x + threadIdx.x; t < total; t += (int64_t)gridDim.x * blockDim.x) {
    const int64_t s = t / c4n;
    const int c = (int)(t - s * c4n) * 4;
    const int32_t a = seg_ptr[s], e = seg_ptr[s + 1];
    float4 acc = f4zero();
    for (int32_t p = a; p < e; ++p) f4add(acc, *reinterpret_cast<const float4*>(x + (int64_t)col[p] * ldx + c));
    if (e - a > 1) {
      const float inv = 1.f / (float)(e - a);
      acc.x *= inv; acc.y *= inv; acc.z *= inv; acc.w *= inv;
    }
    *reinterpret_cast<float4*>(out + s * cin + c) = acc;
  }
}
__global__ void __launch_bounds__(256) gather_mean_scalar_kernel(const float* __restrict__ x, int64_t ldx, int cin,
                                                                 int64_t nseg, const int32_t* __restrict__ seg_ptr,
                                                                 const int32_t* __restrict__ col,
                                                                 float* __restrict__ out) {
  const int64_t total = nseg * cin;
  for (int64_t t = (int64_t)blockIdx.x * blockDim.x + threadIdx.x; t < total; t += (int64_t)gridDim.x * blockDim.x) {
    const int64_t s = t / cin;
    const int c = (int)(t - s * cin);
    const int32_t a = seg_ptr[s], e = seg_ptr[s + 1];
    float acc = 0.f;
    for (int32_t p = a; p < e; ++p) acc += x[(int64_t)col[p] * ldx + c];
    if (e - a > 1) acc /= (float)(e - a);
    out[t] = acc;
  }
}

extern "C" int ofx_gather_mean(const float* x, int64_t ldx, int cin, int64_t n_nodes, const int32_t* seg_ptr,
                               const int32_t* col, float* col_data, void* stream) {
  if (!x || !seg_ptr || !col || !col_data || cin < 1 || ldx < cin || n_nodes < 0) return OFX_EINVAL;
  const int64_t nseg = n_nodes * 7;
  hipStream_t st = ofx_stream(stream);
  const bool vec = (cin % 4 == 0) && ((ldx & 3) == 0) && (((uintptr_t)x & 15) == 0) && (((uintptr_t)col_data & 15) == 0);
  if (vec)
    gather_mean_kernel<<<ofx_grid(nseg * (cin / 4), 256), 256, 0, st>>>(x, ldx, cin, nseg, seg_ptr, col, col_data);
  else
    gather_mean_scalar_kernel<<<ofx_grid(nseg * cin, 256), 256, 0, st>>>(x, ldx, cin, nseg, seg_ptr, col, col_data);
  OFX_LAUNCH_CHECK();
  return OFX_OK;
}
```

octfusion_amd/csrc/ofx_norm.hip:

```cpp
#include "ofx_planes.h"

constexpr int GN_ROWS_PER_BLOCK = 64;

static inline int64_t gn_stats_rows(int64_t n, int batch_size, int C = 128) {
  const int64_t chunks = (n + GN_ROWS_PER_BLOCK - 1) / GN_ROWS_PER_BLOCK;
  const int64_t bytes_per_batch = n * (int64_t)C * 4 / (batch_size > 0 ? batch_size : 1);
  int64_t per_batch = bytes_per_batch / (512 << 10);
  per_batch = per_batch < 8 ? 8 : (per_batch > 128 ? 128 : per_batch);
  int64_t cap = per_batch * (int64_t)batch_size;
  if (cap < 64) cap = 64;
  return chunks <= cap ? GN_ROWS_PER_BLOCK : GN_ROWS_PER_BLOCK * ((chunks + cap - 1) / cap);
}

__global__ void __launch_bounds__(256) gn_stats_kernel(const float* __restrict__ x, int64_t ldx, int64_t n, int C,
                                                       const int32_t* __restrict__ bid, double* __restrict__ sums,
                                                       int64_t rpb) {
  __shared__ int sb[256];
  __shared__ float sv[256][8];
  const int CT = C >> 2;
  const int RP = 256 / CT;
  const int cl = threadIdx.x % CT, rl = threadIdx.x / CT;
  int cb = -1;
  float s[4] = {0, 0, 0, 0}, q[4] = {0, 0, 0, 0};
  auto flush_direct = [&](int b, const float* ps, const float* pq) {
    if (b < 0) return;
    double* o = sums + ((int64_t)b * C + cl * 4) * 2;
#pragma unroll
    for (int k = 0; k < 4; ++k) {
      unsafeAtomicAdd(o + 2 * k, (double)ps[k]);
      unsafeAtomicAdd(o + 2 * k + 1, (double)pq[k]);
    }
  };
  auto accum = [&](int b, const float4& v) {
    if (b != cb) {
      flush_direct(cb, s, q);
      cb = b;
      s[0] = s[1] = s[2] = s[3] = 0.f;
      q[0] = q[1] = q[2] = q[3] = 0.f;
    }
    s[0] += v.x; s[1] += v.y; s[2] += v.z; s[3] += v.w;
    q[0] += v.x * v.x; q[1] += v.y * v.y; q[2] += v.z * v.z; q[3] += v.w * v.w;
  };
  const int64_t r_begin = (int64_t)blockIdx.x * rpb;
  const int64_t r_end = r_begin + rpb < n ? r_begin + rpb : n;
  if (rl < RP) {
    int64_t r = r_begin + rl;
    for (; r + 3 * (int64_t)RP < r_end; r += 4 * (int64_t)RP) {
      const int b0 = bid[r], b1 = bid[r + RP], b2 = bid[r + 2 * RP], b3 = bid[r + 3 * RP];
      const float4 v0 = *reinterpret_cast<const float4*>(x + r * ldx + cl * 4);
      const float4 v1 = *reinterpret_cast<const float4*>(x + (r + RP) * ldx + cl * 4);
      const float4 v2 = *reinterpret_cast<const float4*>(x + (r + 2 * RP) * ldx + cl * 4);
      const float4 v3 = *reinterpret_cast<const float4*>(x + (r + 3 * RP) * ldx + cl * 4);
      accum(b0, v0); accum(b1, v1); accum(b2, v2); accum(b3, v3);
    }
    for (; r < r_end; r += RP) accum(bid[r], *reinterpret_cast<const float4*>(x + r * ldx + cl * 4));
  }
  sb[threadIdx.x] = (rl < RP) ? cb : -1;
#pragma unroll
  for (int k = 0; k < 4; ++k) { sv[threadIdx.x][k] = s[k]; sv[threadIdx.x][4 + k] = q[k]; }
  __syncthreads();
  if (rl == 0) {
    double ds[4] = {0, 0, 0, 0}, dq[4] = {0, 0, 0, 0};
    for (int j = 0; j < RP; ++j) {
      const int t = j * CT + cl;
      const int b = sb[t];
      if (b < 0) continue;
      if (b == cb) {
#pragma unroll
        for (int k = 0; k < 4; ++k) { ds[k] += (double)sv[t][k]; dq[k] += (double)sv[t][4 + k]; }
      } else {
        flush_direct(b, &sv[t][0], &sv[t][4]);
      }
    }
    if (cb >= 0) {
      double* o = sums + ((int64_t)cb * C + cl * 4) * 2;
#pragma unroll
      for (int k = 0; k < 4; ++k) { unsafeAtomicAdd(o + 2 * k, ds[k]); unsafeAtomicAdd(o + 2 * k + 1, dq[k]); }
    }
  }
}

extern "C" int ofx_gn_stats(const float* x, int64_t ldx, int64_t n, int C, const int32_t* batch_id, int batch_size,
                            double* sums, void* stream) {
  if (!x || !batch_id || !sums || n < 0 || C < 4 || (C & 3) || C > 1024 || ldx < C || (ldx & 3) ||
      ((uintptr_t)x & 15) || batch_size < 1)
    return OFX_EINVAL;
  hipStream_t st = ofx_stream(stream);
  if (hipMemsetAsync(sums, 0, sizeof(double) * 2 * (size_t)batch_size * C, st) != hipSuccess) return OFX_ELAUNCH;
  if (n > 0) gn_stats_kernel<<<(int)ofx_cdiv(n, gn_stats_rows(n, batch_size, C)), 256, 0, st>>>(x, ldx, n, C, batch_id, sums,
                                                                                             gn_stats_rows(n, batch_size, C));
  OFX_LAUNCH_CHECK();
  return OFX_OK;
}

extern "C" int ofx_gn_stats_acc(const float* x, int64_t ldx, int64_t n, int C, const int32_t* batch_id, int batch_size,
                                double* sums, void* stream) {
  if (!x || !batch_id || !sums || n < 0 || C < 4 || (C & 3) || C > 1024 || ldx < C || (ldx & 3) ||
      ((uintptr_t)x & 15) || batch_size < 1)
    return OFX_EINVAL;
  if (n > 0) gn_stats_kernel<<<(int)ofx_cdiv(n, gn_stats_rows(n, batch_size, C)), 256, 0, ofx_stream(stream)>>>(
      x, ldx, n, C, batch_id, sums, gn_stats_rows(n, batch_size, C));
  OFX_LAUNCH_CHECK();
  return OFX_OK;
}

__global__ void gn_finalize_kernel(const double* __restrict__ sums, const float* __restrict__ count, int B, int C, int G,
                                   float eps, float count_eps, float* __restrict__ mean, float* __restrict__ rstd) {
  const int cpg = C / G;
  for (int t = blockIdx.x * blockDim.x + threadIdx.x; t < B * G; t += gridDim.x * blockDim.x) {
    const int b = t / G, g = t - b * G;
    double S = 0, SS = 0;
    for (int c = g * cpg; c < (g + 1) * cpg; ++c) {
      S += sums[((int64_t)b * C + c) * 2];
      SS += sums[((int64_t)b * C + c) * 2 + 1];
    }
    const float cnt = count[b] * (float)cpg;
    const float inv = 1.0f / (cnt + count_eps);
    const double m = S * (double)inv;
    const double ssd = SS - 2.0 * m * S + (double)cnt * m * m;
    const double var = (ssd > 0 ? ssd : 0) * (double)inv;
    const float rs = (float)(1.0 / sqrt(var + (double)eps));
    for (int c = g * cpg; c < (g + 1) * cpg; ++c) {
      mean[(int64_t)b * C + c] = (float)m;
      rstd[(int64_t)b * C + c] = rs;
    }
  }
}

extern "C" int ofx_gn_finalize(const double* sums, const float* count, int batch_size, int C, int groups, float eps,
                               float count_eps, float* mean, float* rstd, void* stream) {
  if (!sums || !count || !mean || !rstd || batch_size < 1 || C < 1 || groups < 1 || C % groups) return OFX_EINVAL;
  gn_finalize_kernel<<<ofx_grid((int64_t)batch_size * groups, 64), 64, 0, ofx_stream(stream)>>>(
      sums, count, batch_size, C, groups, eps, count_eps, mean, rstd);
  OFX_LAUNCH_CHECK();
  return OFX_OK;
}

__device__ __forceinline__ float ofx_apply_act(float v, int act) {
  if (act == OFX_ACT_SILU) return v / (1.f + __expf(-v));
  if (act == OFX_ACT_GELU) return 0.5f * v * (1.f + erff(v * 0.70710678118654752440f));
  return v;
}

constexpr int GN_APPLY_ROWS = 64;
struct GnFin { const double* sums; const float* count; int G; float eps, count_eps; };
__device__ __forceinline__ void gn_group_stats(const GnFin& f, int b, int g, int C, float& mean, float& rstd) {
  const int cpg = C / f.G;
  double S = 0, SS = 0;
  for (int c = g * cpg; c < (g + 1) * cpg; ++c) {
    S += f.sums[((int64_t)b * C + c) * 2];
    SS += f.sums[((int64_t)b * C + c) * 2 + 1];
  }
  const float cnt = f.count[b] * (float)cpg;
  const float inv = 1.0f / (cnt + f.count_eps);
  const double m = S * (double)inv;
  const double ssd = SS - 2.0 * m * S + (double)cnt * m * m;
  const double var = (ssd > 0 ? ssd : 0) * (double)inv;
  mean = (float)m;
  rstd = (float)(1.0 / sqrt(var + (double)f.eps));
}
template <int MODE, bool FIN>
__global__ void __launch_bounds__(256) gn_apply_kernel(const float* __restrict__ x, int64_t ldx, int64_t n, int C,
                                                       const int32_t* __restrict__ bid, const float* __restrict__ mean,
                                                       const float* __restrict__ rstd, const GnFin fin,
                                                       const float* __restrict__ w,
                                                       const float* __restrict__ bias, int act, char* __restrict__ out,
                                                       int64_t ldo, int64_t aux_blocks,
                                                       const int32_t* __restrict__ seg_ptr,
                                                       const int32_t* __restrict__ col,
                                                       const int32_t* __restrict__ multi_seg, int64_t n_multi,
                                                       char* __restrict__ aux, const int32_t* __restrict__ aux_plan) {
  const int CT = C >> 2, RP = 256 / CT;
  const int cl = threadIdx.x % CT, rl = threadIdx.x / CT;
  __shared__ float fin_ms[FIN ? 2 * 2 * 1024 : 1];
  constexpr int AUX_LDS = 64;
  __shared__ int aux_v[AUX_LDS], aux_n[AUX_LDS], aux_src[AUX_LDS][4];
  int fb0 = -1, fb1 = -1;
  const int64_t gT = gridDim.x;
  const int64_t a_before = aux_blocks > 0 ? ((int64_t)blockIdx.x * aux_blocks) / gT : 0;
  const bool is_aux = aux_blocks > 0 && (((int64_t)blockIdx.x + 1) * aux_blocks) / gT > a_before;
  const int64_t aux_id = a_before, main_id = (int64_t)blockIdx.x - a_before;
  const int64_t r_begin0 = main_id * GN_APPLY_ROWS;
  const int64_t r_end0 = r_begin0 + GN_APPLY_ROWS < n ? r_begin0 + GN_APPLY_ROWS : n;
  const bool pre = FIN && !is_aux && rl < RP && r_begin0 + rl + 3 * (int64_t)RP < r_end0;
  float4 pv0, pv1, pv2, pv3;
  int pb0 = 0, pb1 = 0, pb2 = 0, pb3 = 0;
  if (pre) {
    const int64_t r = r_begin0 + rl;
    const int c_ = cl * 4;
    pb0 = bid[r]; pb1 = bid[r + RP]; pb2 = bid[r + 2 * RP]; pb3 = bid[r + 3 * RP];
    pv0 = *reinterpret_cast<const float4*>(x + r * ldx + c_);
    pv1 = *reinterpret_cast<const float4*>(x + (r + RP) * ldx + c_);
    pv2 = *reinterpret_cast<const float4*>(x + (r + 2 * RP) * ldx + c_);
    pv3 = *reinterpret_cast<const float4*>(x + (r + 3 * RP) * ldx + c_);
  }
  if (FIN) {
    if (!is_aux) {
      fb0 = bid[r_begin0];
      fb1 = bid[r_end0 - 1];
    } else {
      const int64_t v0 = aux_id * RP, v1e = v0 + RP - 1 < n_multi ? v0 + RP - 1 : n_multi;
      if (n_multi > 0) {
        fb0 = bid[multi_seg[(v0 > 0 ? v0 : 1) - 1] / 7];
        fb1 = bid[multi_seg[(v1e > 0 ? v1e : 1) - 1] / 7];
      }
    }
    const int cpg = C / fin.G;
    for (int t = threadIdx.x; t < 2 * fin.G && fb0 >= 0; t += 256) {
      const int slot = t / fin.G, g = t - slot * fin.G;
      if (slot == 1 && fb1 == fb0) continue;
      float mm, rr;
      gn_group_stats(fin, slot ? fb1 : fb0, g, C, mm, rr);
      for (int cc = g * cpg; cc < (g + 1) * cpg; ++cc) {
        fin_ms[(slot * 2 + 0) * 1024 + cc] = mm;
        fin_ms[(slot * 2 + 1) * 1024 + cc] = rr;
      }
    }
    __syncthreads();
  }
  int own_b = 0, own_e = 0;
  if (!is_aux && aux && aux_plan && MODE != 0) {
    const int64_t mb_ = (n + GN_APPLY_ROWS - 1) / GN_APPLY_ROWS;
    own_b = aux_plan[main_id]; own_e = aux_plan[main_id + 1];
    const int i = own_b + (int)threadIdx.x;
    if (i < own_e && (int)threadIdx.x < AUX_LDS) {
      const int v = aux_plan[mb_ + 1 + i];
      const int64_t sgm = multi_seg[v - 1];
      const int32_t pa = seg_ptr[sgm], pz = seg_ptr[sgm + 1];
      aux_v[threadIdx.x] = v;
      aux_n[threadIdx.x] = pz - pa;
#pragma unroll
      for (int k = 0; k < 4; ++k) aux_src[threadIdx.x][k] = col[pa + k < pz ? pa + k : pa];
      if (pz - pa > 4) aux_n[threadIdx.x] = -(int)(pa + 1);
    }
  }
  const bool active = rl < RP;
  const int c = cl * 4;
  const float4 ww = *reinterpret_cast<const float4*>(w + c);
  const float4 bb = *reinterpret_cast<const float4*>(bias + c);
  int cb = -1;
  float4 m = make_float4(0.f, 0.f, 0.f, 0.f), rs = m;
  auto norm = [&](int b, const float4& v) {
    if (b != cb) {
// ... 794 lines not shown
```

octfusion_amd/graph_unet_hr.py:

```python
import inspect

import torch
import torch.nn as nn

from . import ops
from .modules import (GraphConv, GraphDownsample, GraphResBlockEmbed, GraphUpsample, _Linear,
                      graphnormalization)


def level_plan(input_depth, channel_mult, num_res_blocks):
    enc, dec = [], []
    d = input_depth
    last = len(channel_mult) - 1
    for level in range(len(channel_mult)):
        enc += [('res', d, level)] * num_res_blocks[level]
        if level != last:
            enc.append(('down', d, level))
            d -= 1
    for level in range(last, -1, -1):
        for i in range(num_res_blocks[level] + 1):
            dec.append(('res', d, level))
            if level and i == num_res_blocks[level]:
                dec.append(('up', d, level))
                d += 1
# ... 121 lines not shown
            lab = None
            if self.num_classes is not None:
                assert label.shape == (doctree.batch_size,)
                lab = self.label_emb(label)
            e_act = self.time_embed[2](self.time_embed[0](t_emb, act_out='silu'), res=lab, act_out='silu')
            return e_act, self._all_emb_outs(e_act)
        emb_main, emb_fork = ops.fork_stream(x.device)
        if emb_fork is not None:
            with torch.cuda.stream(emb_fork):
                emb_act, emb_outs = embed()
            if unet_lr is not None and hasattr(unet_lr, 'precompute_embeddings'):
                unet_lr.precompute_embeddings(timesteps, label, doctree.batch_size)
        else:
            emb_act, emb_outs = embed()

        dev = x.device
        n_at = {dd: doctree.csr(dd)[2] for dd in range(self._d_mid, self.input_depth + 1)}
        cat_bufs = []
        for (c_h, c_skip, dd) in self._cat_plan:
            cat_bufs.append(torch.empty(n_at[dd], c_h + c_skip, dtype=torch.float32, device=dev))

        def skip_slot(i):
            c_h, c_skip, _ = self._cat_plan[i]
            return cat_bufs[i][:, c_h:]

        d = self.input_depth
        if as_middle:
            h = x
            ops.rows_copy(x, skip_slot(0), x.shape[0])
            hs = [skip_slot(0)]
        else:
            h = self.input_blocks[0](x, doctree, d, out=skip_slot(0))
            hs = [h]
        if emb_fork is not None:
            emb_main.wait_stream(emb_fork)
        for k, ((kind, dd, _), module) in enumerate(zip(self._enc, self.input_blocks[1:])):
            slot = skip_slot(k + 1)
            if kind == 'res':
                h = module(h, emb, doctree, dd, emb_act=emb_act, out=slot, emb_out=emb_outs[id(module)])
            else:
                h = module(h, doctree, dd, out=slot)
            hs.append(h)
        d = self._d_mid

        if unet_lr is not None:
            c_mid = self.middle_block1.out_channels
            mid = torch.empty(n_at[d], 2 * c_mid, dtype=torch.float32, device=dev)
            h = self.middle_block1(h, emb, doctree, d, emb_act=emb_act, out=mid[:, :c_mid], emb_out=emb_outs[id(self.middle_block1)])
            if 'out' in inspect.signature(unet_lr.forward_as_middle).parameters:
                h_lr = unet_lr.forward_as_middle(h, doctree, timesteps, label, context, out=mid[:, c_mid:])
            else:
                h_lr = unet_lr.forward_as_middle(h, doctree, timesteps, label, context)
            if h_lr.data_ptr() == mid[:, c_mid:].data_ptr() and h_lr.shape[1] == c_mid:
                h = ops.cat_channels(h, h_lr, buf=mid)
            else:
                h = ops.cat_channels(h, h_lr)
            h = self.middle_block2(h, emb, doctree, d, emb_act=emb_act, emb_out=emb_outs[id(self.middle_block2)])

        n_skip = len(hs)
        j = 0
        pending = h
        for idx, ((kind, dd, _), module) in enumerate(zip(self._dec, self.output_blocks)):
            nxt_is_res = idx + 1 < len(self._dec) and self._dec[idx + 1][0] == 'res'
            out_slot = None
            if nxt_is_res:
                c_h_n = self._cat_plan[n_skip - 1 - (j + (1 if kind == 'res' else 0))][0]
                out_slot = cat_bufs[n_skip - 1 - (j + (1 if kind == 'res' else 0))][:, :c_h_n]
            if kind == 'res':
                si = n_skip - 1 - j
                c_h = self._cat_plan[si][0]
                left = cat_bufs[si][:, :c_h]
                if pending.data_ptr() != left.data_ptr():
                    ops.rows_copy(pending, left, pending.shape[0])
                    st = ops.get_stats(pending)
                    if st is not None:
                        setattr(left, ops.STATS_ATTR, st)
                    pending = left
                hcat = ops.cat_channels(pending, hs[si], buf=cat_bufs[si])
                pending = module(hcat, emb, doctree, dd, emb_act=emb_act, out=out_slot, emb_out=emb_outs[id(module)])
                j += 1
            else:
                pending = module(pending, doctree, dd, out=out_slot)
        h = pending
        h = self.end_norm(h, doctree, self.input_depth, act='silu', out=out_mid if as_middle else None)
        if as_middle:
            return h
        out = self.out(h, doctree, self.input_depth)
        assert out.shape[0] == x.shape[0]
        return out
```

octfusion_amd/graph_unet_lr.py:

```python
import math

import torch
import torch.nn as nn

from . import ops
from .modules import _Linear


class _GridCache:

    _cache = {}

    @classmethod
    def get(cls, batch_size, device):
        key = (batch_size, device.type, device.index)
        c = cls._cache.get(key)
        if c is None:
            c = cls(batch_size, device)
            cls._cache[key] = c
        return c

    def __init__(self, batch_size, device):
        self.B = batch_size
        self.device = device
# ... 4 lines not shown
    def table(self, mode, depth_out, fast):
        k = (mode, depth_out, fast)
        if k not in self._tab:
            d_in = depth_out + (0, 1, -1)[mode]
            pad = self.B * 8 ** d_in if fast else -1
            self._tab[k] = ops.grid_conv_table(mode, depth_out, self.B, self.device, pad)
        return self._tab[k]

    def rev(self, mode, depth_out):
        k = ('rev', mode, depth_out)
        if k not in self._tab:
            from ._lib import call, ptr, stream, lib
            d_in = depth_out + (0, 1, -1)[mode]
            n_in, n_out = self.B * 8 ** d_in, self.B * 8 ** depth_out
            tab = self.table(mode, depth_out, False)
            dev = self.device
            nseg = n_in * 27
            cnt = torch.empty(nseg, dtype=torch.int32, device=dev)
            call('ofx_table_reverse_count', ptr(tab), n_out, 27, n_in, ptr(cnt), stream())
            rev_ptr = torch.empty(nseg + 1, dtype=torch.int32, device=dev)
            ws = torch.empty(lib().ofx_scan_ws_bytes(nseg), dtype=torch.uint8, device=dev)
            call('ofx_scan_i32', ptr(cnt), ptr(rev_ptr), nseg, ptr(ws), stream())
            E = int(rev_ptr[-1].item())
            rev_row = torch.empty(max(E, 1), dtype=torch.int32, device=dev)
            rev_w = torch.empty(max(E, 1), dtype=torch.float32, device=dev)
            call('ofx_table_reverse_fill', ptr(tab), n_out, 27, n_in, ptr(rev_ptr), ptr(cnt), ptr(rev_row), ptr(rev_w),
                 stream())
            nbr = torch.empty(nseg, dtype=torch.int32, device=dev)
            call('ofx_seg_primary_w', ptr(rev_ptr), ptr(rev_row), ptr(rev_w), nseg, ptr(nbr), stream())
            call('ofx_seg_multi_flag_w', ptr(rev_ptr), ptr(rev_w), nseg, ptr(cnt), stream())
            rank = torch.empty(nseg + 1, dtype=torch.int32, device=dev)
            call('ofx_scan_i32', ptr(cnt), ptr(rank), nseg, ptr(ws), stream())
            V = int(rank[-1].item())
            nbr_ext = torch.empty(nseg, dtype=torch.int32, device=dev)
            multi_seg = torch.empty(max(V, 1), dtype=torch.int32, device=dev)
            call('ofx_seg_primary_ext_w', ptr(rev_ptr), ptr(rev_row), ptr(rev_w), nseg, n_out, ptr(rank), ptr(nbr_ext),
                 ptr(multi_seg), stream())
            self._tab[k] = dict(rev_ptr=rev_ptr, rev_row=rev_row, rev_w=rev_w, nbr=nbr, nbr_ext=nbr_ext,
                                multi_seg=multi_seg, V=V, n_in=n_in, n_out=n_out)
        return self._tab[k]

    def batch_id(self, depth):
        if depth not in self._bid:
            per = 8 ** depth
            self._bid[depth] = (torch.arange(self.B * per, device=self.device) // per).to(torch.int32)
            self._cnt[depth] = torch.full((self.B,), float(per), dtype=torch.float32, device=self.device)
        return self._bid[depth]

    def count(self, depth):
        self.batch_id(depth)
        return self._cnt[depth]


class GridState:

    def __init__(self, batch_size, depth, device):
        self.B, self.depth = batch_size, depth
        self.cache = _GridCache.get(batch_size, device)

    def at(self, depth):
        g = GridState.__new__(GridState)
        g.B, g.depth, g.cache = self.B, depth, self.cache
        return g


def _dense_io(x):
    assert x.dim() == 5 and x.shape[2] == x.shape[3] == x.shape[4], 'dense blocks take cubic [b, c, S, S, S] grids'
    S = x.shape[2]
    depth = S.bit_length() - 1
    assert 1 << depth == S, 'grid edge must be a power of two'
    B = x.shape[0]
    rows = ops.voxel2octree_cf(x.float().contiguous(), depth)
    return rows, GridState(B, depth, x.device), (lambda r, d: ops.octree2voxel_cf(r, B, d))


class GroupNorm32(nn.GroupNorm):

    @torch.no_grad()
    def forward(self, x, gs, act=None, out=None):
        return ops.group_norm(x, gs.cache.batch_id(gs.depth), gs.cache.count(gs.depth), gs.B, self.weight,
                              self.bias, self.num_groups, self.eps, act, out, count_eps=0.0,
                              rows_per_batch=8 ** gs.depth)


def convnormalization(channels):
    return GroupNorm32(min(channels, 32), channels)


class our_Identity(nn.Module):
    def forward(self, x, *args, **kwargs):
        return x


class GridConv3d(nn.Module):

    def __init__(self, cin, cout, mode=0):
        super().__init__()
        self.in_channels, self.out_channels, self.mode = cin, cout, mode
        self.weight = nn.Parameter(torch.empty(cout, cin, 3, 3, 3))
        self.bias = nn.Parameter(torch.empty(cout))
        nn.init.kaiming_uniform_(self.weight, a=math.sqrt(5))
        bound = 1 / math.sqrt(cin * 27)
        nn.init.uniform_(self.bias, -bound, bound)
        self._pw = ops.PackedConv3d()

    def out_depth(self, depth):
        return depth + (0, -1, 1)[self.mode]

    @torch.no_grad()
    def forward(self, x, gs, emb=None, res=None, out=None):
        d_out = self.out_depth(gs.depth)
        n_out = gs.B * 8 ** d_out
        bid = gs.cache.batch_id(d_out) if emb is not None else None
        mode = self.mode
        return ops.gridconv(x, lambda fast: gs.cache.table(mode, d_out, fast), n_out, self._pw.get(self.weight),
                            self.bias, emb, bid, res, out)


class _PointConv(nn.Module):

    def __init__(self, cin, cout, kdims):
        super().__init__()
        self.weight = nn.Parameter(torch.empty(cout, cin, *([1] * kdims)))
        self.bias = nn.Parameter(torch.empty(cout))
        nn.init.kaiming_uniform_(self.weight, a=math.sqrt(5))
        nn.init.uniform_(self.bias, -1 / math.sqrt(cin), 1 / math.sqrt(cin))
        self._pw = ops.PackedWeight()

    @torch.no_grad()
    def forward(self, x, res=None, out=None):
        w = self.weight.view(self.weight.shape[0], self.weight.shape[1])
        return ops.gemm(x, self._pw.get(w, 'nk'), self.bias, res, out)


class ConvUpsample(nn.Module):

    def __init__(self, channels, use_conv=True, dims=3):
        super().__init__()
        self.channels = channels
        self.conv = GridConv3d(channels, channels, mode=2)

    def forward(self, x, gs=None, out=None):
        if gs is None:
            rows, gs, back = _dense_io(x)
            return back(self.conv(rows, gs), gs.depth + 1)
        return self.conv(x, gs, out=out), gs.at(gs.depth + 1)


class ConvDownsample(nn.Module):

    def __init__(self, channels, use_conv=True, dims=3):
        super().__init__()
        self.channels = channels
        self.op = GridConv3d(channels, channels, mode=1)

    def forward(self, x, gs=None):
        if gs is None:
            rows, gs, back = _dense_io(x)
            return back(self.op(rows, gs), gs.depth - 1)
        return self.op(x, gs), gs.at(gs.depth - 1)


class ResnetBlock(nn.Module):

    def __init__(self, world_dims, dim_in, dim_out, emb_dim, dropout=0.1, use_text_condition=False):
        super().__init__()
        assert world_dims == 3 and not use_text_condition
        self.time_mlp = nn.Sequential(nn.SiLU(), _Linear(emb_dim, dim_out))
        self.block1 = nn.Sequential(convnormalization(dim_in), nn.SiLU(), GridConv3d(dim_in, dim_out))
        conv2 = GridConv3d(dim_out, dim_out)
        for p in conv2.parameters():
            p.detach().zero_()
        self.block2 = nn.Sequential(convnormalization(dim_out), nn.SiLU(), nn.Dropout(dropout), conv2)
        self.res_conv = _PointConv(dim_in, dim_out, 3) if dim_in != dim_out else nn.Identity()

    @torch.no_grad()
    def forward(self, x, emb_act, gs=None, out=None, t=None):
        if gs is None:
            rows, gs, back = _dense_io(x)
            return back(self.forward(rows, ops.act(emb_act.float().contiguous(), 'silu'), gs), gs.depth)
        skip, main, fork = x, None, None
        if not isinstance(self.res_conv, nn.Identity):
            main, fork = ops.fork_stream(x.device, level=2)
            if fork is not None:
                with torch.cuda.stream(fork):
                    skip = self.res_conv(x)
            else:
                skip = self.res_conv(x)
        h = self.block1[0](x, gs, act='silu')
        if t is None:
            t = self.time_mlp[1](emb_act)
        h = self.block1[2](h, gs, emb=t)
        h = self.block2[0](h, gs, act='silu', out=h)
        if fork is not None:
            main.wait_stream(fork)
        return self.block2[3](h, gs, res=skip, out=out)


class QKVAttention(nn.Module):
    """reference modules.py:538-547 -- computed by ofx_attention."""


class AttentionBlock(nn.Module):

    def __init__(self, channels, num_heads=1):
        super().__init__()
        self.channels = channels
        self.num_heads = num_heads
        self.norm = convnormalization(channels)
        self.qkv = _PointConv(channels, channels * 3, 1)
        self.attention = QKVAttention()
        self.proj_out = _PointConv(channels, channels, 1)
        for p in self.proj_out.parameters():
            p.detach().zero_()

    @torch.no_grad()
    def forward(self, x, gs=None, out=None):
        if gs is None:
            rows, gs, back = _dense_io(x)
            return back(self.forward(rows, gs), gs.depth)
        qkv = self.qkv(self.norm(x, gs))
        h = ops.attention(qkv, gs.B, 8 ** gs.depth, self.num_heads)
        return self.proj_out(h, res=x, out=out)


class _AttnSeq(nn.Sequential):

    def forward(self, x, gs, out=None):
        return self[2](self[0](x, gs, act='silu'), gs, out=out)


class LearnedSinusoidalPosEmb(nn.Module):

    def __init__(self, dim):
        super().__init__()
        assert dim % 2 == 0
        self.weights = nn.Parameter(torch.randn(dim // 2))

    def forward(self, x):
        x = x[:, None]
        freqs = x * self.weights[None, :] * 2 * math.pi
        return torch.cat((x, freqs.sin(), freqs.cos()), dim=-1)


class UNet3DModel(nn.Module):
    def __init__(self, full_depth, in_split_channels, model_channels, out_split_channels,
                 attention_resolutions, dropout=0, channel_mult=(1, 2, 4, 8), dims=2, num_classes=None,
                 use_checkpoint=False, num_heads=-1, use_text_condition=False, context_dim=None,
                 n_embed=None, **kwargs):
        super().__init__()
        assert dims == 3
        self.full_depth = full_depth
        self.in_channels = in_split_channels
        self.model_channels = model_channels
        self.out_channels = out_split_channels
        self.attention_resolutions = attention_resolutions
        self.channel_mult = list(channel_mult)
        self.num_classes = num_classes
        self.num_heads = num_heads
        mc = model_channels
        chans = [mc] + [mc * m for m in self.channel_mult]
        in_out = list(zip(chans[:-1], chans[1:]))
        ted = mc * 4
        self.time_pos_emb = LearnedSinusoidalPosEmb(mc)
        self.time_emb = nn.Sequential(_Linear(mc + 1, ted), nn.SiLU(), _Linear(ted, ted))
        if num_classes is not None:
            self.label_emb = nn.Embedding(num_classes, ted)
        self.input_emb = GridConv3d(2 * self.in_channels, mc)

        def attn(c, ds):
            if ds in attention_resolutions:
                return _AttnSeq(convnormalization(c), nn.SiLU(), AttentionBlock(c, num_heads=num_heads))
            return our_Identity()

        self.downs = nn.ModuleList()
        self.ups = nn.ModuleList()
        nres = len(in_out)
        ds = 1
        for ind, (ci, co) in enumerate(in_out):
            last = ind >= nres - 1
            self.downs.append(nn.ModuleList([
                ResnetBlock(dims, ci, co, emb_dim=ted, dropout=dropout), attn(co, ds),
                ConvDownsample(co, dims=dims) if not last else our_Identity()]))
            if not last:
                ds *= 2
        mid = chans[-1]
        self.mid_block1 = ResnetBlock(dims, mid, mid, emb_dim=ted, dropout=dropout)
        self.mid_self_attn = attn(mid, ds)
        self.mid_block2 = ResnetBlock(dims, mid, mid, emb_dim=ted, dropout=dropout)
        for ci, co in reversed(in_out[1:]):
            self.ups.append(nn.ModuleList([
                ResnetBlock(dims, co * 2, ci, emb_dim=ted, dropout=dropout), attn(ci, ds),
                ConvUpsample(ci, dims=dims)]))
            ds //= 2
        self.end = nn.Sequential(convnormalization(mc), nn.SiLU())
        self.out = GridConv3d(mc, self.out_channels)

    @torch.no_grad()
    def _embed(self, timesteps, label, batch_size):
        pe = ops.learned_sinusoid(timesteps.float(), self.time_pos_emb.weights)
        lab = None
        if self.num_classes is not None:
            assert label.shape == (batch_size,)
            lab = self.label_emb(label)
# ... 105 lines not shown
```

octfusion_amd/modules.py:

```python
import math

import torch
import torch.nn as nn

from . import ops


def _gn_groups(channels, group=32):
    if channels <= 32:
        group = channels // 4
    elif channels % group != 0:
        group = 30
    assert channels % group == 0
    return group


class GraphConv(nn.Module):

    def __init__(self, in_channels, out_channels, n_edge_type=7, avg_degree=7, n_node_type=0,
                 use_bias=False):
        super().__init__()
        assert n_edge_type == 7, 'the dual octree graph has 7 edge types'
        self.in_channels = in_channels
        self.out_channels = out_channels
        self.use_bias = use_bias
        self.n_edge_type = n_edge_type
        self.avg_degree = avg_degree
        self.n_node_type = n_node_type
        node_channel = n_node_type if n_node_type > 1 else 0
        self.weights = nn.Parameter(torch.empty(n_edge_type * (in_channels + node_channel), out_channels))
        if use_bias:
            self.bias = nn.Parameter(torch.empty(out_channels))
        self.reset_parameters()
        self._pw = ops.PackedWeight()
        self._pw2 = ops.PackedPlanes()
        self._pno = ops.PackedNarrowOut()
        self.emit_stats = True

    def planes_mode(self, doctree, d, cin=None):
        mode = ops.planes_mode()
        if not mode:
            return 0
        cin = self.in_channels if cin is None else (cin if ops.planes_pairs(mode) else 64)
        N = doctree.csr(d)[2]
        tiles = ((N + 255) // 256) * ((self.out_channels + 127) // 128)
        if (cin % (32 if ops.planes_pairs(mode) else 64) or self.out_channels % 4 or self.out_channels < 64 or
                tiles < ops.PLANES_MIN_TILES):
            return 0
        return mode

    def reset_parameters(self):
        fan_in = self.avg_degree * self.in_channels
        fan_out = self.avg_degree * self.out_channels
        a = math.sqrt(3.0) * math.sqrt(2.0 / float(fan_in + fan_out))
        nn.init.uniform_(self.weights, -a, a)
        if self.use_bias:
            nn.init.zeros_(self.bias)

    @torch.no_grad()
    def forward(self, x, doctree, d, emb=None, res=None, out=None, split_input=False):
        nt = self.n_node_type if self.n_node_type > 1 else 0
        seg_ptr, col, N, E = doctree.csr(d)
        assert x.shape[0] == N, 'x has %d rows, graph depth %d has %d nodes' % (x.shape[0], d, N)
        stats = None
        if self.emit_stats and N * self.out_channels >= (1 << 14) and self.out_channels % 4 == 0:
            stats = ops.stats_zeros(doctree.batch_size * self.out_channels * 2, x.device)
        mode = ops.planes_of(x)
        cin_k = self.in_channels
        if not mode and emb is None and res is None:
            if ops.narrow_in_ok(self.in_channels, self.out_channels, nt):
                y = ops.graphconv_narrow_in(x, seg_ptr, col, self.weights, self.in_channels, nt,
                                            doctree.node_type8(d) if nt else None, self.bias if self.use_bias else None,
                                            doctree.batch_id32(d) if stats is not None else None, out, stats,
                                            ext=doctree.ext(d))
                if stats is not None:
                    setattr(y, ops.STATS_ATTR, stats)
                return y
            if ops.NARROW_OUT and self.out_channels <= 8 and self.in_channels % 32 == 0 and N >= 4096:
                pno = self._pno.get(self.weights, self.in_channels, nt)
                bias = self.bias if self.use_bias else None
                tkey = ('narrow_tt', d, nt, self.weights.data_ptr(), self.weights._version,
                        None if bias is None else (bias.data_ptr(), bias._version))
                tt = doctree._tf.get(tkey)
                if tt is None and (nt or bias is not None):
                    tt = doctree._tf[tkey] = pno.type_term(doctree.type_frac(d, nt) if nt else None, nt, N, self.in_channels, bias)
                return ops.graphconv_narrow_out(x, seg_ptr, col, pno, self.in_channels, tt, out)
        if not mode and split_input:
            mode = self.planes_mode(doctree, d)
            if mode:
                x = ops.planes_split(x, mode)
        if not mode and self.in_channels < 32:
            mode = self.planes_mode(doctree, d, cin=32)
            if mode:
                cin_k = 32 if ops.planes_pairs(mode) else 64
                x = ops.planes_split(x, mode, Cpad=cin_k)
        if mode:
            pw2 = self._pw2.get(self.weights, self.in_channels, nt, mode, cin_pad=cin_k)
            y = ops.graphconv_planes(x, mode, seg_ptr, col, doctree.ext(d), pw2, cin_k, nt,
                                     doctree.type_frac_planes(d, nt, mode) if nt else None,
                                     self.bias if self.use_bias else None, emb,
                                     doctree.batch_id32(d) if (emb is not None or stats is not None) else None,
                                     res, out, stats=stats)
            if stats is not None:
                setattr(y, ops.STATS_ATTR, stats)
            return y
        pw = self._pw.get(self.weights, 'graphconv', self.in_channels, nt)
        tf = doctree.type_frac(d, nt) if nt else None
        y = ops.graphconv(x, doctree.nbr(d), seg_ptr, col, pw, self.in_channels, tf,
                          self.bias if self.use_bias else None, emb,
                          doctree.batch_id32(d) if (emb is not None or stats is not None) else None, res, out,
                          ext=doctree.ext(d), stats=stats)
        if stats is not None:
            setattr(y, ops.STATS_ATTR, stats)
        return y

    def extra_repr(self):
        return 'channel_in={}, channel_out={}, n_edge_type={}, avg_degree={}, n_node_type={}'.format(
            self.in_channels, self.out_channels, self.n_edge_type, self.avg_degree, self.n_node_type)


class DualOctreeGroupNorm(nn.Module):

    def __init__(self, in_channels, group=32, nempty=False):
        super().__init__()
        self.eps = 1e-5
        self.nempty = nempty
        self.in_channels = in_channels
        self.group = _gn_groups(in_channels, group)
        self.channels_per_group = in_channels // self.group
        self.weights = nn.Parameter(torch.ones(1, in_channels))
        self.bias = nn.Parameter(torch.zeros(1, in_channels))

    @torch.no_grad()
    def forward(self, data, doctree, depth, act=None, out=None, planes=0):
        assert doctree.batch_id32(depth).shape[0] == data.shape[0]
        stats = ops.get_stats(data)
        if ops.planes_pairs(planes) and out is not None and not ops.planes_ok(out, planes):
            out = None
        aux_graph = None
        if planes:
            seg_ptr, col, _, _ = doctree.csr(depth)
            _, multi_seg, n_multi = doctree.ext(depth)
            oct_plan = doctree.oct_plan(depth) if ops.AUX_PLAN == 'oct' else None
            block_plan = doctree.aux_plan(depth) if ops.AUX_PLAN and oct_plan is None else None
            aux_graph = ops.AuxGraph(seg_ptr, col, multi_seg, n_multi, oct_plan, block_plan)
        y = ops.group_norm(data, doctree.batch_id32(depth), doctree.count(depth), doctree.batch_size,
                           self.weights, self.bias, self.group, self.eps, act, out, stats=stats, planes=planes,
                           aux_graph=aux_graph)
        if out is data and stats is not None:
            delattr(data, ops.STATS_ATTR)
        return y

    def extra_repr(self):
        return 'in_channels={}, group={}, nempty={}'.format(self.in_channels, self.group, self.nempty)


class _Linear(nn.Module):

    def __init__(self, cin, cout, bias=True):
        super().__init__()
        self.in_features, self.out_features = cin, cout
        self.weight = nn.Parameter(torch.empty(cout, cin))
        self.bias = nn.Parameter(torch.empty(cout)) if bias else None
        nn.init.kaiming_uniform_(self.weight, a=math.sqrt(5))
        if bias:
            bound = 1 / math.sqrt(cin)
            nn.init.uniform_(self.bias, -bound, bound)
        self._pw = ops.PackedWeight()

# ... 282 lines not shown
```

octfusion_amd/ops.py:

```python
import contextlib
import os
from typing import NamedTuple

import torch

from . import _lib
from ._lib import call, call_may_decline, ptr, stream

ACT = {None: 0, 'none': 0, 'silu': 1, 'gelu': 2}

GRAPHCONV_PROFILE = None
_NO_BRACKET = contextlib.nullcontext()


@contextlib.contextmanager
def _timed_layer(prof, *rec):
    e0 = torch.cuda.Event(enable_timing=True)
    e1 = torch.cuda.Event(enable_timing=True)
    e0.record()
    yield
    e1.record()
    prof.append((e0, e1) + rec)


# ... 307 lines not shown

def reset_range_words(device):
    t = _SCRATCH.get(_scratch_key('range', device))
    if t is not None:
        t.zero_()


def range_error(device, result=None):
    t = _SCRATCH.get(_scratch_key('range', device))
    n = int(t[0].item()) if t is not None else 0
    bad = result is not None and not bool(torch.isfinite(result).all())
    return {'operands_beyond_fp16': n, 'result_non_finite': bad} if (n or bad) else None


def raise_on_range_error(device, result=None):
    err = range_error(device, result)
    if err is None:
        return
    range_words(device).zero_()
    was = get_precision()
    if was not in ('fp16x3', 'fp16'):
        raise _lib.OfxError('non-finite result on %s in precision %s (%s)' % (device, was, err))
    if AUTO_RANGE_FALLBACK and was == 'fp16x3':
        set_precision('bf16x3')
    raise OfxRangeError('fp16x3 range guard on %s: %s -- operands beyond +-65504 do not fit the fp16 operand pairs; the '
                        'results of this call are invalid%s' % (device, err, '; the process now computes in bf16x3: call again'
                                                               if AUTO_RANGE_FALLBACK and was == 'fp16x3' else ''))


def workspace(device, nbytes=96 << 20):
    def make():
        _no_capture('the split-K / hand-off workspace')
        return torch.empty(nbytes, dtype=torch.uint8, device=device)
    t = _scratch('ws', device, True, make)
    if t.numel() < nbytes:
        t = _SCRATCH[_scratch_key('ws', device, True)] = make()
    return t


def scan_i32(x):
    _chk(x, torch.int32)
    n = x.numel()
    out = torch.empty(n + 1, dtype=torch.int32, device=x.device)
    ws = torch.empty(_lib.lib().ofx_scan_ws_bytes(n), dtype=torch.uint8, device=x.device)
    call('ofx_scan_i32', ptr(x), ptr(out), n, ptr(ws), stream())
    return out


class PackedWeight:

    def __init__(self):
        self.t = None
        self.key = None
        self.K = self.N = self.Kp = 0

    def get(self, w, mode, cin=0, nt=0):
        key = (w.data_ptr(), w._version, tuple(w.shape), mode, cin, nt, _lib.lib().ofx_get_precision() == 3)
        if key == self.key:
            return self
        _chk(w)
        w = w.detach()
        if not w.is_contiguous():
            w = w.contiguous()
        L = _lib.lib()
        if mode == 'kn' or mode == 'graphconv':
            K, N = w.shape
            sk, sn = N, 1
        elif mode == 'nk':
            N, K = w.shape
            sk, sn = 1, K
        else:
            raise ValueError(mode)
        if mode == 'graphconv':
            Kp = L.ofx_graphconv_packed_k(cin, nt)
        else:
            cin = nt = 0
            Kp = L.ofx_packed_k(K)
        out = torch.empty(L.ofx_packed_floats(Kp, N), dtype=torch.float32, device=w.device)
        call('ofx_pack_weights', ptr(w), sk, sn, K, N, cin, nt, ptr(out), Kp, stream())
        self.t, self.key, self.K, self.N, self.Kp = out, key, K, N, Kp
        return self


def gemm(a, pw, bias=None, res=None, out=None, a_rows=None, out_rows=None, m=None, out_planes=0):
    a, lda = _row_major(a)
    M = m if m is not None else (a_rows.numel() if a_rows is not None else a.shape[0])
    if a.shape[1] != pw.K:
        raise ValueError('K mismatch: %d vs %d' % (a.shape[1], pw.K))
    out, ldc = _out2d(out, M, pw.N, a.device)
    res, ldr = _row_major(res)
    _chk(bias)
    _chk(a_rows, torch.int32)
    _chk(out_rows, torch.int32)
    ws = workspace(a.device)
    _meta('dense_gemm', 2.0 * M * pw.K * pw.N, 4.0 * (M * pw.K + pw.K * pw.N + M * pw.N * (2 if res is not None else 1)),
          (M, pw.K, pw.N))
    if out_planes:
        args = ('ofx_gemm_f32_planes', ptr(a), lda, ptr(a_rows), M, pw.K, ptr(pw.t), pw.Kp, pw.N, ptr(bias),
                ptr(res), ldr, ptr(out), ldc, ptr(out_rows), ptr(ws), ws.numel(), out_planes, stream())
    else:
        args = ('ofx_gemm_f32', ptr(a), lda, ptr(a_rows), M, pw.K, ptr(pw.t), pw.Kp, pw.N, ptr(bias),
                ptr(res), ldr, ptr(out), ldc, ptr(out_rows), ptr(ws), ws.numel(), stream())
    if pw.N <= 64 or pw.K <= 64:
        with policy_scope('small_gemm'):
            call(*args)
    else:
        call(*args)
    return out


def gather_gemm(x, tab, ntap, pw, n_out, bias=None, res=None, out=None, out_rows=None, out_planes=0):
    x, ldx = _row_major(x)
    cin = x.shape[1]
    assert pw.K == ntap * cin and cin % 32 == 0
    _chk(tab, torch.int32)
    out, ldc = _out2d(out, n_out, pw.N, x.device)
    res, ldr = _row_major(res)
    _chk(bias)
    _chk(out_rows, torch.int32)
    ws = workspace(x.device)
    _meta('dense_gemm', 2.0 * n_out * pw.K * pw.N, 4.0 * (n_out * pw.K + pw.K * pw.N + n_out * pw.N), (n_out, pw.K, pw.N))
    call('ofx_gather_gemm_f32', ptr(x), ldx, cin, ntap, x.shape[0], n_out, ptr(tab), ptr(zero_row(x.device)), ptr(pw.t), pw.Kp,
         pw.N, ptr(bias), ptr(res), ldr, ptr(out), ldc, ptr(out_rows), ptr(ws), ws.numel(), out_planes, stream())
    return out


GEMM_PLANES = os.environ.get('OFX_GEMM_PLANES', '0') == '1'


class PackedGemmPlanes:

    def __init__(self):
        self.t = None
        self.key = None

    def get(self, w2d, mode):
        key = (w2d.data_ptr(), w2d._version, tuple(w2d.shape), tuple(w2d.stride()), mode)
        if key != self.key:
            _chk(w2d)
            K, N = w2d.shape
            nb = _lib.lib().ofx_gemm_planes_packed_bytes(K, N, mode)
            assert nb > 0
            t = torch.empty(nb, dtype=torch.uint8, device=w2d.device)
            assert t.data_ptr() % 128 == 0
            call('ofx_pack_gemm_planes', ptr(w2d.detach()), w2d.stride(0), w2d.stride(1), K, N, mode, ptr(t), stream())
            self.t, self.key, self.K, self.N = t, key, K, N
        return self


def gemm_planes(a_planes, pgp, out, out_planes=0, bias=None):
    mode = planes_of(a_planes)
    M, K = a_planes.shape
    assert planes_pairs(mode) and K == pgp.K and a_planes.stride(1) == 1
    dev = a_planes.device
    out, ldc = _out2d(out, M, pgp.N, dev)
    tabs = _scratch('row_tab', dev, False, dict)
    tab = tabs.get(M)
    if tab is None:
        if len(tabs) > 64:
            tabs.clear()
        _no_capture('the row table of a dense planes GEMM')
        tab = torch.zeros(M * 7 + 4, dtype=torch.int32, device=dev)
        tab[:M * 7].view(M, 7)[:, 0] = torch.arange(M, dtype=torch.int32, device=dev)
        tabs[M] = tab
    ws = workspace(dev)
    sync = sync_words(dev)
    _meta('dense_gemm', 2.0 * M * K * pgp.N, 4.0 * (M * K + K * pgp.N + M * pgp.N), (M, K, pgp.N, 'planes'))
    return call_may_decline('ofx_gemm_planes', ptr(a_planes), a_planes.stride(0) * 4, M, M, K, ptr(tab), ptr(pgp.t), pgp.N,
# ... 72 lines not shown
        else:
            call(*args)
    return out


NARROW_IN = os.environ.get('OFX_NARROW_IN', '1') == '1'
NARROW_OUT = os.environ.get('OFX_NARROW_OUT', '1') == '1'


def narrow_in_ok(cin, cout, nt):
    return NARROW_IN and cin <= 8 and cout in (64, 128) and 7 * (cin + nt) <= 96


NARROW_IN_TAB = os.environ.get('OFX_NARROW_IN_TAB', '1') == '1'
NARROW_IN_TAB_MIN_ROWS = int(os.environ.get('OFX_NARROW_IN_TAB_MIN_ROWS', str(1 << 19)))


def graphconv_narrow_in(x, seg_ptr, col, weights, cin, nt, node_type=None, bias=None, batch_id=None, out=None, stats=None,
                        ext=None):
    x, ldx = _row_major(x)
    w = weights.detach()
    if not w.is_contiguous():
        w = w.contiguous()
    _chk(w)
    N, cout = x.shape[0], w.shape[1]
    assert x.shape[1] == cin and w.shape[0] == 7 * (cin + nt)
    out, ldc = _out2d(out, N, cout, x.device)
    if nt:
        _chk(node_type, torch.uint8)
    _chk(bias)
    _chk(stats, torch.float64)
    if stats is not None:
        _chk(batch_id, torch.int32)
    E = col.numel()
    flops = 2.0 * N * w.shape[0] * cout
    nbytes = 4.0 * (E * cin + N * cout + w.numel()) + 8.0 * E
    with _layer_bracket(flops, nbytes, cout, ('graph', N, cin, cout)):
        ws = workspace(x.device)
        _meta('graphconv_narrow', flops, nbytes, (N, cin, cout, 'narrow_in'))
        if ext is not None and NARROW_IN_TAB and N >= NARROW_IN_TAB_MIN_ROWS:
            nbr_ext, multi_seg, n_multi = ext
            aux = torch.empty((N + n_multi + 1) * (8 if cin <= 4 else 16), dtype=torch.float32, device=x.device)
            call('ofx_graphconv_narrow_in_tab', ptr(x), ldx, cin, N, ptr(seg_ptr), ptr(col), ptr(nbr_ext), ptr(multi_seg),
                 n_multi, ptr(aux), ptr(node_type) if nt else None, nt, ptr(w), cout, ptr(bias),
                 ptr(batch_id) if stats is not None else None, ptr(out), ldc, ptr(stats), cout, ptr(ws), ws.numel(),
                 stream())
        else:
            call('ofx_graphconv_narrow_in', ptr(x), ldx, cin, N, ptr(seg_ptr), ptr(col), ptr(node_type) if nt else None, nt,
                 ptr(w), cout, ptr(bias), ptr(batch_id) if stats is not None else None, ptr(out), ldc, ptr(stats), cout,
                 ptr(ws), ws.numel(), stream())
    return out


class PackedNarrowOut:

    def __init__(self):
        self.key = None
        self.pw = PackedWeight()

    def get(self, w, C, nt):
        key = (w.data_ptr(), w._version, tuple(w.shape), C, nt)
        if key != self.key:
            wd = w.detach()
            if not wd.is_contiguous():
                wd = wd.contiguous()
            _chk(wd)
            cout = wd.shape[1]
            self.width = 32 if 7 * cout <= 32 else 64
            self.wd = torch.empty(C, self.width, dtype=torch.float32, device=w.device)
            call('ofx_narrow_out_pack', ptr(wd), C, nt, cout, self.width, ptr(self.wd), stream())
            self.w = wd
            self.key = key
        return self

    def type_term(self, type_frac, nt, N, C, bias):
        cout = self.w.shape[1]
        tt = torch.empty(N, cout, dtype=torch.float32, device=self.w.device)
        _chk(bias)
        call('ofx_narrow_out_type_term', ptr(type_frac) if nt else None, type_frac.stride(0) if nt else 0, nt, N, ptr(self.w),
             C, cout, ptr(bias), ptr(tt), stream())
        return tt


def graphconv_narrow_out(x, seg_ptr, col, pno, C, type_term=None, out=None):
    N = x.shape[0]
    cout = pno.w.shape[1]
    E = col.numel()
    flops = 2.0 * N * pno.w.shape[0] * cout
    pwid = pno.width
    agg_bytes = 4.0 * (N * pwid + E + 7 * N + 2 * N * cout)
    nbytes = agg_bytes + 4.0 * (N * C + N * pwid + pno.w.numel())
    with _layer_bracket(flops, nbytes, cout, ('graph', N, C, cout)):
        P = gemm(x, pno.pw.get(pno.wd, 'kn'))
        out, ldc = _out2d(out, N, cout, x.device)
        _chk(type_term)
        assert type_term is None or (type_term.is_contiguous() and tuple(type_term.shape) == (N, cout))
        _meta('graphconv_narrow', flops, agg_bytes, (N, C, cout, 'narrow_out'))
        call('ofx_graphconv_narrow_out', ptr(P), P.stride(0), cout, N, ptr(seg_ptr), ptr(col), ptr(type_term), ptr(out),
             ldc, stream())
    return out


def gemm_tn(p, q):
    _chk(p), _chk(q)
    assert p.shape[0] == q.shape[0]
    K0, N0 = p.shape[1], q.shape[1]

    def pad4(t):
        c = t.shape[1]
        if c % 4 == 0 and t.stride(0) % 4 == 0 and t.stride(1) == 1 and t.data_ptr() % 16 == 0:
            return t
        out = torch.zeros(t.shape[0], (c + 3) // 4 * 4, dtype=torch.float32, device=t.device)
        out[:, :c] = t
        return out
    p, q = pad4(p), pad4(q)
    if (K0, N0) != (p.shape[1], q.shape[1]):
        return gemm_tn(p, q)[:K0, :N0].contiguous()
    p, ldp = _row_major(p)
    q, ldq = _row_major(q)
    K, N = p.shape[1], q.shape[1]
    out = torch.empty(K, N, dtype=torch.float32, device=p.device)
    ws = workspace(p.device)
    call('ofx_gemm_tn_f32', ptr(p), ldp, ptr(q), ldq, p.shape[0], K, N, ptr(out), ptr(ws), ws.numel(), stream())
    return out


GRAD_TOP_EXP = 8


def grad_pow2(dy):
    lo, hi = torch.aminmax(dy) if dy.numel() else (dy.new_zeros(()), dy.new_zeros(()))
    _, e = torch.frexp(torch.maximum(-lo, hi))
    s = (GRAD_TOP_EXP - e).clamp(-100, 100)
    return torch.ldexp(dy, s), torch.ldexp(torch.ones_like(hi), -s)


def gemm_grad(dy, pw):
    dys, inv = grad_pow2(dy)
    return gemm(dys, pw).mul_(inv)


def linear_backward(x, dy, weight, need_dx=True):
    dW = gemm_tn(dy, x)
    dx = gemm_grad(dy, PackedWeight().get(weight, 'kn')) if need_dx else None
    return dx, dW, dy.sum(0)


def graphconv_backward(x, dy, doctree, d, weights, n_node_type, need_dx=True, need_dw=True):
    x, ldx = _row_major(x)
    dy, ldy = _row_major(dy)
    _chk(x), _chk(dy), _chk(weights)
    N, cin = x.shape
    cout = dy.shape[1]
    nt = n_node_type if n_node_type > 1 else 0
    assert weights.shape == (7 * (cin + nt), cout)
    seg_ptr, col, Ng, E = doctree.csr(d)
    assert N == Ng and dy.shape[0] == N
    ws = workspace(x.device)
    dx = dW = None
    if need_dx:
        rv = doctree.rev(d)
        wt = weights.detach().view(7, cin + nt, cout)[:, :cin, :].permute(0, 2, 1).reshape(7 * cout, cin).contiguous()
        pwt = PackedWeight().get(wt, 'graphconv', cout, 0)
        dx = torch.empty(N, cin, dtype=torch.float32, device=x.device)
        dys, inv = grad_pow2(dy)
        lds = dys.stride(0)
        fast = cout % 32 == 0 and lds % 4 == 0
        aux = torch.empty((rv['V'] + 1) * lds, dtype=torch.float32, device=x.device) if fast else None
        call('ofx_graphconv_bwd_data', ptr(dys), lds, cout, N, ptr(rv['nbr']), ptr(rv['rev_ptr']), ptr(rv['rev_row']),
             ptr(rv['rev_w']), ptr(rv['nbr_ext']) if fast else None, ptr(rv['multi_seg']) if fast else None,
             rv['V'] if fast else 0, ptr(aux), ptr(pwt.t), pwt.Kp, cin, ptr(dx), cin, ptr(ws), ws.numel(), stream())
        dx.mul_(inv)
    if need_dw:
        L = _lib.lib()
        Kp = L.ofx_graphconv_packed_k(cin, nt)
        Kf = Kp - (((7 * nt + 31) // 32) * 32 if nt else 0)
        tf = doctree.type_frac(d, nt) if nt else None
        fast = cin % 32 == 0 and ldx % 4 == 0
        nbr_ext, multi_seg, V = doctree.ext(d)
        aux = torch.empty((V + 1) * ldx, dtype=torch.float32, device=x.device) if fast else None
        dyw, ldw, cw = dy, ldy, cout
        if cout % 4 or ldy % 4 or dy.data_ptr() % 16:
            cw = (cout + 3) // 4 * 4
            dyw = torch.zeros(N, cw, dtype=torch.float32, device=x.device)
            dyw[:, :cout] = dy
            ldw = cw
        dwp = torch.empty(Kp, cw, dtype=torch.float32, device=x.device)
        call('ofx_graphconv_bwd_weight', ptr(x), ldx, cin, N, ptr(doctree.nbr(d)), ptr(seg_ptr), ptr(col),
             ptr(nbr_ext) if fast else None, ptr(multi_seg) if fast else None, V if fast else 0, ptr(aux),
             ptr(tf), tf.stride(0) if tf is not None else 0, tf.shape[1] if tf is not None else 0,
             ptr(dyw), ldw, cw, ptr(dwp), Kp, ptr(ws), ws.numel(), stream())
        dwp = dwp[:, :cout]
        dev = x.device
        dirs = torch.arange(7, device=dev).view(7, 1)
        idx = [dirs * cin + torch.arange(cin, device=dev).view(1, cin)]
        if nt:
            idx.append(Kf + dirs * nt + torch.arange(nt, device=dev).view(1, nt))
        dW = dwp.index_select(0, torch.cat(idx, 1).reshape(-1))
    return dx, dW


class PackedConv3d:

    def __init__(self):
        self.t = None
        self.key = None
        self.cin = self.N = 0

    def get(self, w):
        key = (w.data_ptr(), w._version, tuple(w.shape), _lib.lib().ofx_get_precision() == 3)
        if key == self.key:
            return self
        _chk(w)
        cout, cin = w.shape[:2]
        assert tuple(w.shape[2:]) == (3, 3, 3)
        w = w.detach().contiguous()
        Kp = _lib.lib().ofx_conv3d_packed_k(cin)
        out = torch.empty(_lib.lib().ofx_packed_floats(Kp, cout), dtype=torch.float32, device=w.device)
        call('ofx_pack_conv3d', ptr(w), cin, cout, ptr(out), stream())
        self.t, self.key, self.cin, self.N = out, key, cin, cout
        return self


def gridconv(x, tables, n_out, pw, bias=None, emb=None, batch_id=None, res=None, out=None):
    x, ldx = _row_major(x)
    if x.shape[1] != pw.cin:
        raise ValueError('cin mismatch')
    out, ldc = _out2d(out, n_out, pw.N, x.device)
    emb, lde = _row_major(emb)
    if emb is not None:
        _chk(batch_id, torch.int32)
    res, ldr = _row_major(res)
    _chk(bias)
    ws = workspace(x.device)
    fast = pw.cin % 32 == 0 and ldx % 4 == 0
    flops = 2.0 * n_out * 27 * pw.cin * pw.N
    nbytes = 4.0 * (27.0 * n_out * pw.cin + n_out * pw.N + 27.0 * pw.cin * pw.N) + 4.0 * 27 * n_out
    with _layer_bracket(flops, nbytes, pw.N, ('grid', n_out, pw.cin, pw.N)):
        _meta('gridconv_27tap', flops,
              4.0 * (x.shape[0] * pw.cin + n_out * pw.N * (2 if res is not None else 1) + 27.0 * pw.cin * pw.N) + 4.0 * 27 * n_out,
              (n_out, pw.cin, pw.N))
        call('ofx_gridconv_fwd', ptr(x), ldx, pw.cin, x.shape[0], n_out, None if fast else ptr(tables(False)),
             ptr(tables(True)) if fast else None, ptr(zero_row(x.device)), ptr(pw.t), pw.N, ptr(bias), ptr(emb), lde,
             ptr(batch_id) if emb is not None else None, ptr(res), ldr, ptr(out), ldc, ptr(ws), ws.numel(), stream())
    return out


def grid_conv_table(mode, depth_out, batch_size, device, pad=-1):
    n = (8 ** depth_out) * batch_size
    t = torch.empty(n, 27, dtype=torch.int32, device=device)
    call('ofx_grid_conv_table', mode, depth_out, batch_size, pad, ptr(t), stream())
    return t


def attention(qkv, batch_size, T, heads, out=None):
    qkv, ldq = _row_major(qkv)
    C = qkv.shape[1] // 3
    ch = C // heads
    out, ldo = _out2d(out, qkv.shape[0], C, qkv.device)
    _meta('attention', 4.0 * batch_size * heads * T * T * ch, 4.0 * qkv.shape[0] * 4 * C, (batch_size, T, heads, ch))
    call('ofx_attention', ptr(qkv), ldq, batch_size, T, heads, ch, ptr(out), ldo, stream())
    return out


def attention_backward(qkv, dout, batch_size, T, heads):
    qkv, ldq = _row_major(qkv)
    dout, ldo = _row_major(dout)
    _chk(qkv), _chk(dout)
    C = qkv.shape[1] // 3
    ch = C // heads
    dqkv = torch.empty(qkv.shape[0], 3 * C, dtype=torch.float32, device=qkv.device)
    rowstat = torch.empty(batch_size * heads * T * 3, dtype=torch.float32, device=qkv.device)
    call('ofx_attention_bwd', ptr(qkv), ldq, ptr(dout), ldo, batch_size, T, heads, ch, ptr(rowstat), ptr(dqkv), 3 * C,
         stream())
    return dqkv


def gather_mean(x, seg_ptr, col):
    x, ldx = _row_major(x)
    N, C = x.shape
    out = torch.empty(N, 7, C, dtype=torch.float32, device=x.device)
    call('ofx_gather_mean', ptr(x), ldx, C, N, ptr(seg_ptr), ptr(col), ptr(out), stream())
    return out


AUX_ATTR = '_ofx_aux'
GN_FINALIZE_LAUNCH = False
GN_ROWS_TWO_KERNELS = int(os.environ.get('OFX_GN_ROWS_TWO_KERNELS', '2048'))
GN_FUSE_AUX_FINALIZE = os.environ.get('OFX_GN_FUSE_AUX_FINALIZE', '0') == '1'
GN_OCT_FINALIZE = os.environ.get('OFX_GN_OCT_FINALIZE', '1') == '1'
GN_OCT_FINALIZE_MAX_ELEMS = int(os.environ.get('OFX_GN_OCT_FINALIZE_MAX_ELEMS', str(9 << 20)))
AUX_PLAN = {'1': 'oct', '0': ''}.get(os.environ.get('OFX_AUX_PLAN', 'oct'), os.environ.get('OFX_AUX_PLAN', 'oct'))


class AuxGraph(NamedTuple):
    seg_ptr: torch.Tensor
    col: torch.Tensor
    multi_seg: torch.Tensor
    n_multi: int
    oct_plan: tuple = None
    block_plan: tuple = None


def _gn_launch(planes, aux_graph, elems):
    g = aux_graph if planes else None
    oct_plan, block_plan = (g.oct_plan, g.block_plan) if g is not None and AUX_PLAN else (None, None)
    oct_fin = GN_OCT_FINALIZE and AUX_PLAN == 'oct' and oct_plan is not None and elems <= GN_OCT_FINALIZE_MAX_ELEMS
    finalize = GN_FINALIZE_LAUNCH or (g is not None and not GN_FUSE_AUX_FINALIZE and not oct_fin)
    if not planes:
        return 'fp32', finalize
    if oct_plan is not None:
        return ('oct' if finalize or oct_fin else 'plain'), finalize
    return ('block' if block_plan is not None else 'plain'), finalize


def group_norm(x, batch_id, count, batch_size, weight, bias, groups, eps=1e-5, act=None, out=None,
               count_eps=None, stats=None, rows_per_batch=None, planes=0, aux_graph=None):
    if count_eps is None:
        count_eps = eps
    x, ldx = _row_major(x)
    n, C = x.shape
    dev = x.device
    range_words(dev)
    if (rows_per_batch is not None and stats is None and not planes and rows_per_batch * (C // groups) <= (1 << 16)
            and rows_per_batch < GN_ROWS_TWO_KERNELS):
        assert n == rows_per_batch * batch_size
        out, ldo = _out2d(out, n, C, dev)
        _meta('gn_fused_rows', 0, 8.0 * n * C, (n, C))
        call('ofx_gn_fused_rows', ptr(x), ldx, rows_per_batch, batch_size, C, groups, eps, count_eps,
             ptr(weight.detach().reshape(-1)), ptr(bias.detach().reshape(-1)), ACT[act], ptr(out), ldo, stream())
        return out
    if stats is not None:
        _chk(stats, torch.float64)
        assert stats.numel() == batch_size * C * 2
        sums = stats
    else:
        _meta('gn_stats', 0, 4.0 * n * C, (n, C))
        if stats_pool_has_room(batch_size * C * 2, dev):
            sums = stats_zeros(batch_size * C * 2, dev)
            call('ofx_gn_stats_acc', ptr(x), ldx, n, C, ptr(batch_id), batch_size, ptr(sums), stream())
        else:
            sums = torch.empty(batch_size * C * 2, dtype=torch.float64, device=dev)
            call('ofx_gn_stats', ptr(x), ldx, n, C, ptr(batch_id), batch_size, ptr(sums), stream())
    w = weight.detach().reshape(-1)
    b = bias.detach().reshape(-1)
    mean = rstd = None
    launch, finalize = _gn_launch(planes, aux_graph, n * C)
    if finalize:
        mean = torch.empty(batch_size * C, dtype=torch.float32, device=dev)
        rstd = torch.empty(batch_size * C, dtype=torch.float32, device=dev)
        _meta('gn_finalize', 0, 24.0 * batch_size * C, (batch_size, C))
        call('ofx_gn_finalize', ptr(sums), ptr(count), batch_size, C, groups, eps, count_eps, ptr(mean), ptr(rstd),
             stream())
    if planes:
        if aux_graph is not None and out is not None and out.data_ptr() == x.data_ptr():
            out = None
        out, ldo = _planes_out(n, C, planes, dev, out if planes_pairs(planes) else None)
        aux = seg_ptr = col = multi_seg = None
        n_multi = 0
        if aux_graph is not None:
            seg_ptr, col, multi_seg, n_multi = aux_graph[:4]
            aux = torch.empty((n_multi + 1) * ldo, dtype=torch.uint8, device=dev)
            setattr(out, AUX_ATTR, aux)
        setattr(out, PLANES_ATTR, planes)
        _meta('gn_apply', 0, 8.0 * n * C + (n_multi + 1) * float(ldo), (n, C, 'planes+aux' if aux is not None else 'planes'))
        if launch == 'oct':
            op, shift, n_own, n_left, (o_ptr, o_ent, o_head, o_src) = aux_graph.oct_plan
            base = op.data_ptr()
            call('ofx_gn_apply_planes_oct', ptr(x), ldx, n, C, ptr(batch_id), ptr(mean), ptr(rstd), ptr(sums), ptr(count),
                 groups, eps, count_eps, ptr(w), ptr(b), ACT[act], planes, ptr(out), ldo, n_multi, ptr(aux), base + 4 * o_ptr,
                 base + 4 * o_ent, n_own, shift, base + 4 * o_head, base + 4 * o_src, n_left, stream())
        else:
            plan, n_left = aux_graph.block_plan if launch == 'block' else (None, 0)
            call('ofx_gn_apply_planes', ptr(x), ldx, n, C, ptr(batch_id), ptr(mean), ptr(rstd), ptr(sums), ptr(count), groups,
                 eps, count_eps, ptr(w), ptr(b), ACT[act], planes, ptr(out), ldo, ptr(seg_ptr), ptr(col), ptr(multi_seg),
                 n_multi, ptr(aux), ptr(plan), n_left, stream())
        return out
    out, ldo = _out2d(out, n, C, dev)
    _meta('gn_apply', 0, 8.0 * n * C, (n, C, 'fp32'))
    call('ofx_gn_apply', ptr(x), ldx, n, C, ptr(batch_id), ptr(mean), ptr(rstd), ptr(sums), ptr(count), groups, eps, count_eps,
         ptr(w), ptr(b), ACT[act], ptr(out), ldo, stream())
    return out


def group_norm_backward(x, dy, batch_id, count, batch_size, weight, bias, groups, eps=1e-5, act=None, count_eps=None):
    if count_eps is None:
        count_eps = eps
    x, ldx = _row_major(x)
    dy, ldy = _row_major(dy)
    _chk(x), _chk(dy)
    n, C = x.shape
    dev = x.device
    mean = torch.empty(batch_size * C, dtype=torch.float32, device=dev)
    rstd = torch.empty(batch_size * C, dtype=torch.float32, device=dev)
    sums = torch.empty(batch_size * C * 2, dtype=torch.float64, device=dev)
    call('ofx_gn_stats', ptr(x), ldx, n, C, ptr(batch_id), batch_size, ptr(sums), stream())
    call('ofx_gn_finalize', ptr(sums), ptr(count), batch_size, C, groups, eps, count_eps, ptr(mean), ptr(rstd),
         stream())
    w = weight.detach().reshape(-1).contiguous()
    b = bias.detach().reshape(-1).contiguous()
    coef = torch.empty(batch_size * C * 3, dtype=torch.float32, device=dev)
    dx = torch.empty(n, C, dtype=torch.float32, device=dev)
    dgamma = torch.empty(C, dtype=torch.float32, device=dev)
    dbeta = torch.empty(C, dtype=torch.float32, device=dev)
    call('ofx_gn_backward', ptr(x), ldx, ptr(dy), ldy, n, C, ptr(batch_id), batch_size, ptr(count), groups, count_eps,
         ptr(mean), ptr(rstd), ptr(w), ptr(b), ACT[act], ptr(sums), ptr(coef), ptr(dx), C, ptr(dgamma), ptr(dbeta),
         stream())
    return dx, dgamma, dbeta


STATS_ATTR = '_ofx_gn_stats'


class _StatsPool:
    SIZE = 1 << 19

    def __init__(self):
        self.buf = None
        self.cur = 0
        self.depth = 0
        self.gen = 0


def _stats_pool_of(device):
    return _scratch('stats', device, True, _StatsPool)


@contextlib.contextmanager
def stats_scope(device):
    p = _stats_pool_of(device)
    if p.depth == 0:
        if p.buf is None:
            _no_capture('the GroupNorm statistics pool')
            p.buf = torch.empty(p.SIZE, dtype=torch.float64, device=device)
        p.buf.zero_()
        p.cur = 0
        p.gen += 1
    p.depth += 1
    try:
        yield
    finally:
        p.depth -= 1


def stats_pool_has_room(n, device):
    p = _stats_pool_of(device)
    return p.depth > 0 and p.cur + n <= p.SIZE


def stats_zeros(n, device):
    p = _stats_pool_of(device)
    if p.depth > 0 and p.cur + n <= p.SIZE:
        st = p.buf[p.cur:p.cur + n]
        p.cur += (n + 1) & ~1
        st._ofx_gen = p.gen
        st._ofx_pool = p
        return st
    return torch.zeros(n, dtype=torch.float64, device=device)


def get_stats(t):
    st = getattr(t, STATS_ATTR, None)
    pool = getattr(st, '_ofx_pool', None)
    if pool is not None and st._ofx_gen != pool.gen:
        return None
    return st

# ... 74 lines not shown
```

Baseline: 120.1.

## Fuse GroupNorm apply and activation into GEMM and gridconv operand loads

Adds GN-prologue variants of the fp16x3 pair GEMM kernel. Per-group mean and rstd and gamma/beta are staged in LDS, and normalization plus SiLU/GELU are applied to A tiles as they are split into hi/lo halves. ResBlock, attention and graphconv paths call these fused entry points instead of writing a normalized tensor and reading it back. This removes a full read-write pass over activations per norm, at the cost of extra LDS and per-element ALU in the load path. Gridconv repeats the normalization for every one of its 27 taps.

```diff
diff --git a/include/ofx.h b/include/ofx.h
--- a/include/ofx.h
+++ b/include/ofx.h
@@ -164,6 +164,12 @@
                         const float* res, int64_t ldr, float* out, int64_t ldc,
                         const int32_t* out_rows, void* ws, size_t ws_bytes, int out_mode, void* stream);
 
+int ofx_gemm_gn_f32(const float* A, int64_t lda, int64_t M, int64_t K, const float* Wp, int64_t Kp, int64_t N,
+                    const float* bias, const float* res, int64_t ldr, float* out, int64_t ldc,
+                    const int32_t* batch_id, const double* gn_sums, const float* gn_count, int groups, float eps,
+                    float count_eps, const float* gamma, const float* beta, int act, void* ws, size_t ws_bytes,
+                    void* stream);
+
 int ofx_graphconv_fwd(const float* x, int64_t ldx, int cin, int64_t n_nodes,
                       const int32_t* nbr, const int32_t* seg_ptr, const int32_t* col,
                       const int32_t* nbr_ext, const int32_t* multi_seg, int64_t n_multi, float* aux,
@@ -239,6 +245,11 @@
                      const float* Wp, int cout, const float* bias, const float* emb, int64_t lde,
                      const int32_t* batch_id, const float* res, int64_t ldr, float* out,
                      int64_t ldc, void* ws, size_t ws_bytes, void* stream);
+int ofx_gridconv_gn_fwd(const float* x, int64_t ldx, int cin, int64_t n_in, int64_t n_out, const int32_t* nbr27_ext,
+                        const float* zero_row, const float* Wp, int cout, const float* bias, const float* emb,
+                        int64_t lde, const int32_t* batch_id, const float* res, int64_t ldr, float* out, int64_t ldc,
+                        const double* gn_sums, const float* gn_count, int groups, float eps, float count_eps,
+                        const float* gamma, const float* beta, int act, void* ws, size_t ws_bytes, void* stream);
 int ofx_gather_gemm_f32(const float* x, int64_t ldx, int cin, int ntap, int64_t n_src, int64_t n_out, const int32_t* tab,
                         const float* zero_row, const float* Wp, int64_t Kp, int cout, const float* bias,
                         const float* res, int64_t ldr, float* out, int64_t ldc, const int32_t* out_rows, void* ws,
diff --git a/octfusion_amd/_lib.py b/octfusion_amd/_lib.py
--- a/octfusion_amd/_lib.py
+++ b/octfusion_amd/_lib.py
@@ -129,6 +129,10 @@
     'ofx_pack_conv3d': (c_i, [c_p, c_i, c_i, c_p, c_p], True),
     'ofx_gridconv_fwd': (c_i, [c_p, c_l, c_i, c_l, c_l, c_p, c_p, c_p, c_p, c_i, c_p, c_p, c_l, c_p, c_p, c_l, c_p,
                                c_l, c_p, c_sz, c_p], True),
+    'ofx_gridconv_gn_fwd': (c_i, [c_p, c_l, c_i, c_l, c_l, c_p, c_p, c_p, c_i, c_p, c_p, c_l, c_p, c_p, c_l, c_p, c_l,
+                                  c_p, c_p, c_i, c_f, c_f, c_p, c_p, c_i, c_p, c_sz, c_p], True),
+    'ofx_gemm_gn_f32': (c_i, [c_p, c_l, c_l, c_l, c_p, c_l, c_l, c_p, c_p, c_l, c_p, c_l, c_p, c_p, c_p, c_i, c_f, c_f,
+                              c_p, c_p, c_i, c_p, c_sz, c_p], True),
     'ofx_attention': (c_i, [c_p, c_l, c_i, c_i, c_i, c_i, c_p, c_l, c_p], True),
     'ofx_gather_mean': (c_i, [c_p, c_l, c_i, c_l, c_p, c_p, c_p, c_p], True),
     'ofx_gn_stats': (c_i, [c_p, c_l, c_l, c_i, c_p, c_i, c_p, c_p], True),
diff --git a/octfusion_amd/csrc/ofx_gemm.hip b/octfusion_amd/csrc/ofx_gemm.hip
--- a/octfusion_amd/csrc/ofx_gemm.hip
+++ b/octfusion_amd/csrc/ofx_gemm.hip
@@ -1,4 +1,5 @@
 #include "ofx_gemm_common.h"
+#include "ofx_gn.h"
 
 constexpr int BM = 128;
 constexpr int BK = 32;
@@ -506,8 +507,18 @@
     return __builtin_amdgcn_mfma_f32_32x32x16_f16(__builtin_bit_cast(f16x8h_t, a), __builtin_bit_cast(f16x8h_t, b), c, 0, 0, 0);
 }
 
-template <int MODE, int WM, int WN, int MI, int NI, int H16>
-__global__ void __launch_bounds__(256, 2) gemm_pairs_x3_kernel(const GemmArgs g) {
+constexpr int GN_SLOTS = 16, GN_MAX_G = 64, GN_MAX_C = 1024;
+constexpr int GN_LDS_BYTES = (GN_SLOTS * GN_MAX_G * 2 + 2 * GN_MAX_C) * (int)sizeof(float);
+struct GemmGnArgs : GemmArgs {
+  GnFin fin;
+  const float* gamma; const float* beta;
+  int C, cpg_shift, act;
+};
+template <int GN> struct GemmArgsOf { typedef GemmArgs type; };
+template <> struct GemmArgsOf<1> { typedef GemmGnArgs type; };
+
+template <int MODE, int WM, int WN, int MI, int NI, int H16, int GN = 0>
+__global__ void __launch_bounds__(256, 2) gemm_pairs_x3_kernel(const typename GemmArgsOf<GN>::type g) {
   constexpr int BN = WN * NI * 32;
   constexpr int A_BYTES = BM * 80;
   constexpr int BUF_BYTES = 2 * A_BYTES;
@@ -584,8 +595,66 @@
   char* const a_st = smem8 + (r0 * 80 + c4 * 8);
   const char* const a_ld = smem8 + ((wm * MI * 32 + l31) * 80 + 16 * h);
 
+  float* const gn_ms = reinterpret_cast<float*>(smem8 + 2 * BUF_BYTES);
+  float* const gn_gb = gn_ms + GN_SLOTS * GN_MAX_G * 2;
+  int gn_b0 = 0, gn_nb = 0, bl0 = 0, bl1 = 0, bl2 = 0, bl3 = 0;
+  if constexpr (GN) {
+    __shared__ int gn_rng[2];
+    if (threadIdx.x == 0) { gn_rng[0] = INT32_MAX; gn_rng[1] = INT32_MIN; }
+    __syncthreads();
+    const int b0 = g.bid[m_0], b1 = g.bid[m_1], b2 = g.bid[m_2], b3 = g.bid[m_3];
+    atomicMin(&gn_rng[0], min(min(b0, b1), min(b2, b3)));
+    atomicMax(&gn_rng[1], max(max(b0, b1), max(b2, b3)));
+    __syncthreads();
+    gn_b0 = gn_rng[0];
+    gn_nb = gn_rng[1] - gn_b0 + 1;
+    gn_nb = gn_nb < GN_SLOTS ? gn_nb : GN_SLOTS;
+    bl0 = b0 - gn_b0; bl1 = b1 - gn_b0; bl2 = b2 - gn_b0; bl3 = b3 - gn_b0;
+    const int G = g.fin.G;
+    for (int t = threadIdx.x; t < gn_nb * G; t += 256) {
+      const int sl = t / G;
+      float mm, rr;
+      gn_group_stats(g.fin, gn_b0 + sl, t - sl * G, g.C, mm, rr);
+      gn_ms[2 * t] = mm; gn_ms[2 * t + 1] = rr;
+    }
+    for (int c = threadIdx.x; c < g.C; c += 256) { gn_gb[c] = g.gamma[c]; gn_gb[GN_MAX_C + c] = g.beta[c]; }
+    __syncthreads();
+  }
+  auto gn4 = [&](const float4& v, int bl, int cc, bool pad) -> float4 {
+    if constexpr (!GN) {
+      return v;
+    } else {
+      const float4 ww = *reinterpret_cast<const float4*>(gn_gb + cc);
+      const float4 bb = *reinterpret_cast<const float4*>(gn_gb + GN_MAX_C + cc);
+      const int sh = g.cpg_shift;
+      float mm[4], rr[4];
+      if ((unsigned)bl < (unsigned)gn_nb) {
+        const float* ms = gn_ms + bl * g.fin.G * 2;
+        if (sh >= 2) {
+          const float2 t = *reinterpret_cast<const float2*>(ms + 2 * (cc >> sh));
+          mm[0] = mm[1] = mm[2] = mm[3] = t.x; rr[0] = rr[1] = rr[2] = rr[3] = t.y;
+        } else {
+#pragma unroll
+          for (int k = 0; k < 4; ++k) {
+            const float2 t = *reinterpret_cast<const float2*>(ms + 2 * ((cc + k) >> sh));
+            mm[k] = t.x; rr[k] = t.y;
+          }
+        }
+      } else {
+        mm[0] = mm[1] = mm[2] = mm[3] = __builtin_nanf("");
+        rr[0] = rr[1] = rr[2] = rr[3] = 0.f;
+      }
+      float4 y;
+      y.x = pad ? 0.f : gn_affine_act(v.x, mm[0], rr[0], ww.x, bb.x, g.act);
+      y.y = pad ? 0.f : gn_affine_act(v.y, mm[1], rr[1], ww.y, bb.y, g.act);
+      y.z = pad ? 0.f : gn_affine_act(v.z, mm[2], rr[2], ww.z, bb.z, g.act);
+      y.w = pad ? 0.f : gn_affine_act(v.w, mm[3], rr[3], ww.w, bb.w, g.act);
+      return y;
+    }
+  };
+
   struct BFrag { u32x4 h[2][NI], l[2][NI]; };
-  struct RegSet { float4 a0, a1, a2, a3; };
+  struct RegSet { float4 a0, a1, a2, a3; unsigned pad; };
   struct IdxSet { uint32_t i0, i1, i2, i3; };
 
   auto load_bfrag = [&](int ktw, BFrag& F) {
@@ -666,6 +735,10 @@
         R.a1 = ldg4(xp + src_off(I.i1, ldx, n_src, aux_delta) + cc);
         R.a2 = ldg4(xp + src_off(I.i2, ldx, n_src, aux_delta) + cc);
         R.a3 = ldg4(xp + src_off(I.i3, ldx, n_src, aux_delta) + cc);
+        if constexpr (GN) {
+          const uint32_t z = (uint32_t)n_src;
+          R.pad = (I.i0 == z ? 1u : 0u) | (I.i1 == z ? 2u : 0u) | (I.i2 == z ? 4u : 0u) | (I.i3 == z ? 8u : 0u);
+        }
       }
     };
     auto load_bchunk = [&](int ktw, int c, BFrag& F) {
@@ -680,6 +753,20 @@
       *reinterpret_cast<uint2*>(a) = hi; *reinterpret_cast<uint2*>(a + A_BYTES) = lo;
       split16x4<H16>(v1, hi, lo);
       *reinterpret_cast<uint2*>(a + 32 * 80) = hi; *reinterpret_cast<uint2*>(a + 32 * 80 + A_BYTES) = lo;
+    };
+    auto cc_of = [&](int it) {
+      const int itc = clampg(it);
+      if (MODE == MODE_DENSE) {
+        const int cc = itc * BK + c4 * 4;
+        return cc < kclamp ? cc : kclamp;
+      }
+      return (itc / ndir) * BK + c4 * 4;
+    };
+    auto store_half_gn = [&](int buf, int it, const RegSet& R, int half) {
+      const int cc = cc_of(it);
+      const unsigned pm = MODE == MODE_DENSE ? 0u : R.pad;
+      if (half == 0) store_half(buf, gn4(R.a0, bl0, cc, pm & 1u), gn4(R.a1, bl1, cc, pm & 2u), 0);
+      else store_half(buf, gn4(R.a2, bl2, cc, pm & 4u), gn4(R.a3, bl3, cc, pm & 8u), 64);
     };
 #define OFX_FENCE() __builtin_amdgcn_sched_barrier(0)
     auto step = [&](int it, int buf, const IdxSet& Iuse, IdxSet& Iload, const BFrag& Fcur, BFrag& Fnext,
@@ -714,11 +801,13 @@
       OFX_FENCE();
       OFX_MFMA_GROUP(al, h, 1);
       OFX_FENCE();
-      store_half(buf ^ 1, Rold.a0, Rold.a1, 0);
+      if constexpr (GN) store_half_gn(buf ^ 1, it + 1, Rold, 0);
+      else store_half(buf ^ 1, Rold.a0, Rold.a1, 0);
       OFX_FENCE();
       OFX_MFMA_GROUP(ah, l, 1);
       OFX_FENCE();
-      store_half(buf ^ 1, Rold.a2, Rold.a3, 64);
+      if constexpr (GN) store_half_gn(buf ^ 1, it + 1, Rold, 1);
+      else store_half(buf ^ 1, Rold.a2, Rold.a3, 64);
       OFX_FENCE();
       OFX_MFMA_GROUP(ah, h, 1);
 #undef OFX_MFMA_GROUP
@@ -736,8 +825,13 @@
     OFX_FENCE();
     load_rows(g_begin + 1, I1, R1);
     OFX_FENCE();
-    store_half(0, R0.a0, R0.a1, 0);
-    store_half(0, R0.a2, R0.a3, 64);
+    if constexpr (GN) {
+      store_half_gn(0, g_begin, R0, 0);
+      store_half_gn(0, g_begin, R0, 1);
+    } else {
+      store_half(0, R0.a0, R0.a1, 0);
+      store_half(0, R0.a2, R0.a3, 64);
+    }
     __syncthreads();
     int it = g_begin;
     for (; it + 1 < g_end; it += 2) {
@@ -931,6 +1025,17 @@
 static int launch_bf16x3_cfg(GemmArgs& g, hipStream_t st) {
   return g_precision == 3 ? launch_bf16x3_h<MODE, WM, WN, MI, NI, 1>(g, st) : launch_bf16x3_h<MODE, WM, WN, MI, NI, 0>(g, st);
 }
+template <int MODE, int WM, int WN, int MI, int NI, int H16>
+static int launch_gn_h(GemmGnArgs& g, hipStream_t st) {
+  constexpr size_t lds = 2 * (2 * BM * 80) + GN_LDS_BYTES;
+  static_assert(lds <= 64 * 1024, "LDS");
+  gemm_pairs_x3_kernel<MODE, WM, WN, MI, NI, H16, 1><<<g.ntm * g.ntn * g.nsplit, 256, lds, st>>>(g);
+  return OFX_OK;
+}
+template <int MODE, int WM, int WN, int MI, int NI>
+static int launch_gn_cfg(GemmGnArgs& g, hipStream_t st) {
+  return g_precision == 3 ? launch_gn_h<MODE, WM, WN, MI, NI, 1>(g, st) : launch_gn_h<MODE, WM, WN, MI, NI, 0>(g, st);
+}
 
 __global__ void __launch_bounds__(256) stats_reduce_kernel(const float* __restrict__ part, int64_t nwr, int wr_rows,
                                                             int64_t N, const int32_t* __restrict__ bid,
@@ -995,7 +1100,7 @@
 }
 
 template <int MODE>
-static int launch_gemm(GemmArgs& g, float* ws, size_t ws_bytes, hipStream_t st) {
+static int launch_gemm(GemmArgs& g, float* ws, size_t ws_bytes, hipStream_t st, const GemmGnArgs* gn = nullptr) {
   if (g.M <= 0 || g.N <= 0) return OFX_OK;
   {
     auto al16 = [](const void* p) { return (reinterpret_cast<uintptr_t>(p) & 15) == 0; };
@@ -1035,7 +1140,14 @@
         (size_t)nwr * g.N * 2 * sizeof(float) <= g.stats_part_bytes && (((uintptr_t)g.stats_part) & 15) == 0))
     g.stats_part = nullptr;
   g.oscale_p = (fast && g.W16) ? g.Wp + 2 * g.Kp * g.N : nullptr;
-  if (fast && g.W16) {
+  if (gn) {
+    if (!(fast && g.W16) || g.a_rows || g.stats) return OFX_EINVAL;
+    GemmGnArgs gg = *gn;
+    static_cast<GemmArgs&>(gg) = g;
+    if (bn == 32) rc = launch_gn_cfg<MODE, 4, 1, 1, 1>(gg, st);
+    else if (bn == 64) rc = launch_gn_cfg<MODE, 2, 2, 2, 1>(gg, st);
+    else rc = launch_gn_cfg<MODE, 2, 2, 2, 2>(gg, st);
+  } else if (fast && g.W16) {
     if (bn == 32) rc = launch_bf16x3_cfg<MODE, 4, 1, 1, 1>(g, st);
     else if (bn == 64) rc = launch_bf16x3_cfg<MODE, 2, 2, 2, 1>(g, st);
     else rc = launch_bf16x3_cfg<MODE, 2, 2, 2, 2>(g, st);
@@ -1166,6 +1278,38 @@
   return ofx_gemm_f32_planes(A, lda, a_rows, M, K, Wp, Kp, N, bias, res, ldr, out, ldc, out_rows, ws, ws_bytes, 0, stream);
 }
 
+static int gn_common(GemmGnArgs& gn, int C, const double* sums, const float* count, const int32_t* batch_id, int groups,
+                     float eps, float count_eps, const float* gamma, const float* beta, int act) {
+  if (!sums || !count || !batch_id || !gamma || !beta || groups < 1 || groups > GN_MAX_G || C < 4 || (C & 3) ||
+      C > GN_MAX_C || C % groups || act < 0 || act > OFX_ACT_GELU || g_precision == 1)
+    return OFX_EINVAL;
+  const int cpg = C / groups;
+  if (cpg & (cpg - 1)) return OFX_EINVAL;
+  gn = GemmGnArgs{};
+  gn.fin = GnFin{sums, count, groups, eps, count_eps};
+  gn.gamma = gamma; gn.beta = beta; gn.C = C; gn.act = act;
+  gn.cpg_shift = __builtin_ctz((unsigned)cpg);
+  return OFX_OK;
+}
+
+extern "C" int ofx_gemm_gn_f32(const float* A, int64_t lda, int64_t M, int64_t K, const float* Wp, int64_t Kp, int64_t N,
+                               const float* bias, const float* res, int64_t ldr, float* out, int64_t ldc,
+                               const int32_t* batch_id, const double* gn_sums, const float* gn_count, int groups,
+                               float eps, float count_eps, const float* gamma, const float* beta, int act, void* ws,
+                               size_t ws_bytes, void* stream) {
+  if (M == 0 && K >= 1 && N >= 1) return OFX_OK;
+  if (M < 0 || K < 4 || (K & 3) || N < 1 || !Wp || !out || !A || Kp != pad32(K) || lda < K || (lda & 3) || ldc < N ||
+      (res && ldr < N) || (((uintptr_t)Wp | (uintptr_t)A) & 15) || K > INT32_MAX)
+    return OFX_EINVAL;
+  GemmGnArgs gn;
+  if (int rc = gn_common(gn, (int)K, gn_sums, gn_count, batch_id, groups, eps, count_eps, gamma, beta, act)) return rc;
+  GemmArgs g = {};
+  g.A = A; g.lda = lda;
+  g.M = M; g.K = K; g.Wp = Wp; g.Kp = Kp; g.N = N; g.bias = bias;
+  g.res = res; g.ldr = ldr; g.out = out; g.ldc = ldc; g.bid = batch_id;
+  return launch_gemm<MODE_DENSE>(g, (float*)ws, ws_bytes, ofx_stream(stream), &gn);
+}
+
 static int gather_common(GemmArgs& g, const float* x, int64_t ldx, int cin, int ndir, int64_t n_rows,
                          const int32_t* nbr, const int32_t* seg_ptr, const int32_t* col, const float* Wp, int64_t Kp,
                          int cout, const float* bias, const float* emb, int64_t lde, const int32_t* batch_id,
@@ -1196,7 +1340,7 @@
   }
 }
 
-template <int MODE> static int launch_gemm(GemmArgs& g, float* ws, size_t ws_bytes, hipStream_t st);
+template <int MODE> static int launch_gemm(GemmArgs& g, float* ws, size_t ws_bytes, hipStream_t st, const GemmGnArgs* gn);
 
 static int launch_gather_via_col(const GemmArgs& g, float* ws, size_t ws_bytes, hipStream_t st) {
   if (!ws || (((uintptr_t)ws) & 15)) return -1;
@@ -1657,6 +1801,27 @@
   return launch_gemm<MODE_GATHER>(g, (float*)ws, ws_bytes, ofx_stream(stream));
 }
 
+extern "C" int ofx_gridconv_gn_fwd(const float* x, int64_t ldx, int cin, int64_t n_in, int64_t n_out,
+                                   const int32_t* nbr27_ext, const float* zero_row, const float* Wp, int cout,
+                                   const float* bias, const float* emb, int64_t lde, const int32_t* batch_id,
+                                   const float* res, int64_t ldr, float* out, int64_t ldc, const double* gn_sums,
+                                   const float* gn_count, int groups, float eps, float count_eps, const float* gamma,
+                                   const float* beta, int act, void* ws, size_t ws_bytes, void* stream) {
+  if (n_out == 0 && cin >= 1 && cout >= 1) return OFX_OK;
+  GemmArgs g = {};
+  const int64_t Kp = ofx_conv3d_packed_k(cin);
+  int rc = gather_common(g, x, ldx, cin, 27, n_out, nbr27_ext, nullptr, nullptr, Wp, Kp, cout, bias, emb, lde, batch_id,
+                         res, ldr, out, ldc);
+  if (rc) return rc;
+  if (n_in < 1 || !g.fast || !zero_row || ((uintptr_t)zero_row & 15)) return OFX_EINVAL;
+  GemmGnArgs gn;
+  if ((rc = gn_common(gn, cin, gn_sums, gn_count, batch_id, groups, eps, count_eps, gamma, beta, act))) return rc;
+  g.bid = batch_id;
+  g.nbr_ext = nbr27_ext; g.aux = zero_row; g.ldaux = ldx; g.n_src = n_in;
+  g.tf = x; g.ldt = ldx;
+  return launch_gemm<MODE_GATHER>(g, (float*)ws, ws_bytes, ofx_stream(stream), &gn);
+}
+
 extern "C" int ofx_gather_gemm_f32(const float* x, int64_t ldx, int cin, int ntap, int64_t n_src, int64_t n_out,
                                    const int32_t* tab, const float* zero_row, const float* Wp, int64_t Kp, int cout,
                                    const float* bias, const float* res, int64_t ldr, float* out, int64_t ldc,
diff --git a/octfusion_amd/csrc/ofx_gn.h b/octfusion_amd/csrc/ofx_gn.h
--- /dev/null
+++ b/octfusion_amd/csrc/ofx_gn.h
@@ -0,0 +1,29 @@
+#pragma once
+#include "ofx_common.h"
+
+__device__ __forceinline__ float ofx_apply_act(float v, int act) {
+  if (act == OFX_ACT_SILU) return v / (1.f + __expf(-v));
+  if (act == OFX_ACT_GELU) return 0.5f * v * (1.f + erff(v * 0.70710678118654752440f));
+  return v;
+}
+
+struct GnFin { const double* sums; const float* count; int G; float eps, count_eps; };
+__device__ __forceinline__ void gn_group_stats(const GnFin& f, int b, int g, int C, float& mean, float& rstd) {
+  const int cpg = C / f.G;
+  double S = 0, SS = 0;
+  for (int c = g * cpg; c < (g + 1) * cpg; ++c) {
+    S += f.sums[((int64_t)b * C + c) * 2];
+    SS += f.sums[((int64_t)b * C + c) * 2 + 1];
+  }
+  const float cnt = f.count[b] * (float)cpg;
+  const float inv = 1.0f / (cnt + f.count_eps);
+  const double m = S * (double)inv;
+  const double ssd = SS - 2.0 * m * S + (double)cnt * m * m;
+  const double var = (ssd > 0 ? ssd : 0) * (double)inv;
+  mean = (float)m;
+  rstd = (float)(1.0 / sqrt(var + (double)f.eps));
+}
+
+__device__ __forceinline__ float gn_affine_act(float v, float mean, float rstd, float gamma, float beta, int act) {
+  return ofx_apply_act((v - mean) * rstd * gamma + beta, act);
+}
diff --git a/octfusion_amd/csrc/ofx_norm.hip b/octfusion_amd/csrc/ofx_norm.hip
--- a/octfusion_amd/csrc/ofx_norm.hip
+++ b/octfusion_amd/csrc/ofx_norm.hip
@@ -1,4 +1,5 @@
 #include "ofx_planes.h"
+#include "ofx_gn.h"
 
 constexpr int GN_ROWS_PER_BLOCK = 64;
 
@@ -136,29 +137,7 @@
   return OFX_OK;
 }
 
-__device__ __forceinline__ float ofx_apply_act(float v, int act) {
-  if (act == OFX_ACT_SILU) return v / (1.f + __expf(-v));
-  if (act == OFX_ACT_GELU) return 0.5f * v * (1.f + erff(v * 0.70710678118654752440f));
-  return v;
-}
-
 constexpr int GN_APPLY_ROWS = 64;
-struct GnFin { const double* sums; const float* count; int G; float eps, count_eps; };
-__device__ __forceinline__ void gn_group_stats(const GnFin& f, int b, int g, int C, float& mean, float& rstd) {
-  const int cpg = C / f.G;
-  double S = 0, SS = 0;
-  for (int c = g * cpg; c < (g + 1) * cpg; ++c) {
-    S += f.sums[((int64_t)b * C + c) * 2];
-    SS += f.sums[((int64_t)b * C + c) * 2 + 1];
-  }
-  const float cnt = f.count[b] * (float)cpg;
-  const float inv = 1.0f / (cnt + f.count_eps);
-  const double m = S * (double)inv;
-  const double ssd = SS - 2.0 * m * S + (double)cnt * m * m;
-  const double var = (ssd > 0 ? ssd : 0) * (double)inv;
-  mean = (float)m;
-  rstd = (float)(1.0 / sqrt(var + (double)f.eps));
-}
 template <int MODE, bool FIN>
 __global__ void __launch_bounds__(256) gn_apply_kernel(const float* __restrict__ x, int64_t ldx, int64_t n, int C,
                                                        const int32_t* __restrict__ bid, const float* __restrict__ mean,
diff --git a/octfusion_amd/graph_unet_hr.py b/octfusion_amd/graph_unet_hr.py
--- a/octfusion_amd/graph_unet_hr.py
+++ b/octfusion_amd/graph_unet_hr.py
@@ -227,9 +227,8 @@
             else:
                 pending = module(pending, doctree, dd, out=out_slot)
         h = pending
-        h = self.end_norm(h, doctree, self.input_depth, act='silu', out=out_mid if as_middle else None)
         if as_middle:
-            return h
-        out = self.out(h, doctree, self.input_depth)
+            return self.end_norm(h, doctree, self.input_depth, act='silu', out=out_mid)
+        out = self.out(h, doctree, self.input_depth, pre_norm=(self.end_norm, 'silu'))
         assert out.shape[0] == x.shape[0]
         return out
diff --git a/octfusion_amd/graph_unet_lr.py b/octfusion_amd/graph_unet_lr.py
--- a/octfusion_amd/graph_unet_lr.py
+++ b/octfusion_amd/graph_unet_lr.py
@@ -110,6 +110,13 @@
                               self.bias, self.num_groups, self.eps, act, out, count_eps=0.0,
                               rows_per_batch=8 ** gs.depth)
 
+    @torch.no_grad()
+    def prologue(self, x, gs, act=None, taps=1):
+        if not ops.gn_prologue_ok(x, self.num_groups, taps):
+            return None
+        return ops.gn_prologue(x, gs.cache.batch_id(gs.depth), gs.cache.count(gs.depth), gs.B, self.weight, self.bias,
+                               self.num_groups, self.eps, act, count_eps=0.0)
+
 
 def convnormalization(channels):
     return GroupNorm32(min(channels, 32), channels)
@@ -136,13 +143,14 @@
         return depth + (0, -1, 1)[self.mode]
 
     @torch.no_grad()
-    def forward(self, x, gs, emb=None, res=None, out=None):
+    def forward(self, x, gs, emb=None, res=None, out=None, gn=None):
         d_out = self.out_depth(gs.depth)
         n_out = gs.B * 8 ** d_out
         bid = gs.cache.batch_id(d_out) if emb is not None else None
         mode = self.mode
+        assert gn is None or mode == 0
         return ops.gridconv(x, lambda fast: gs.cache.table(mode, d_out, fast), n_out, self._pw.get(self.weight),
-                            self.bias, emb, bid, res, out)
+                            self.bias, emb, bid, res, out, gn=gn)
 
 
 class _PointConv(nn.Module):
@@ -156,9 +164,9 @@
         self._pw = ops.PackedWeight()
 
     @torch.no_grad()
-    def forward(self, x, res=None, out=None):
+    def forward(self, x, res=None, out=None, gn=None):
         w = self.weight.view(self.weight.shape[0], self.weight.shape[1])
-        return ops.gemm(x, self._pw.get(w, 'nk'), self.bias, res, out)
+        return ops.gemm(x, self._pw.get(w, 'nk'), self.bias, res, out, gn=gn)
 
 
 class ConvUpsample(nn.Module):
@@ -215,14 +223,19 @@
                     skip = self.res_conv(x)
             else:
                 skip = self.res_conv(x)
-        h = self.block1[0](x, gs, act='silu')
         if t is None:
             t = self.time_mlp[1](emb_act)
-        h = self.block1[2](h, gs, emb=t)
-        h = self.block2[0](h, gs, act='silu', out=h)
+        gn1 = self.block1[0].prologue(x, gs, act='silu', taps=27)
+        if gn1 is not None:
+            h = self.block1[2](x, gs, emb=t, gn=gn1)
+        else:
+            h = self.block1[2](self.block1[0](x, gs, act='silu'), gs, emb=t)
+        gn2 = self.block2[0].prologue(h, gs, act='silu', taps=27)
+        if gn2 is None:
+            h = self.block2[0](h, gs, act='silu', out=h)
         if fork is not None:
             main.wait_stream(fork)
-        return self.block2[3](h, gs, res=skip, out=out)
+        return self.block2[3](h, gs, res=skip, out=out, gn=gn2)
 
 
 class QKVAttention(nn.Module):
@@ -247,7 +260,8 @@
         if gs is None:
             rows, gs, back = _dense_io(x)
             return back(self.forward(rows, gs), gs.depth)
-        qkv = self.qkv(self.norm(x, gs))
+        gn = self.norm.prologue(x, gs)
+        qkv = self.qkv(x, gn=gn) if gn is not None else self.qkv(self.norm(x, gs))
         h = ops.attention(qkv, gs.B, 8 ** gs.depth, self.num_heads)
         return self.proj_out(h, res=x, out=out)
 
diff --git a/octfusion_amd/modules.py b/octfusion_amd/modules.py
--- a/octfusion_amd/modules.py
+++ b/octfusion_amd/modules.py
@@ -58,9 +58,19 @@
             nn.init.zeros_(self.bias)
 
     @torch.no_grad()
-    def forward(self, x, doctree, d, emb=None, res=None, out=None, split_input=False):
+    def forward(self, x, doctree, d, emb=None, res=None, out=None, split_input=False, pre_norm=None):
         nt = self.n_node_type if self.n_node_type > 1 else 0
         seg_ptr, col, N, E = doctree.csr(d)
+        gn = None
+        if pre_norm is not None:
+            norm, act = pre_norm
+            if (emb is None and res is None and not ops.narrow_in_ok(self.in_channels, self.out_channels, nt)
+                    and ops.NARROW_OUT and self.out_channels <= 8 and self.in_channels % 32 == 0 and N >= 4096
+                    and ops.gn_prologue_ok(x, norm.group)):
+                gn = ops.gn_prologue(x, doctree.batch_id32(d), doctree.count(d), doctree.batch_size, norm.weights,
+                                     norm.bias, norm.group, norm.eps, act, stats=ops.get_stats(x))
+            else:
+                x = norm(x, doctree, d, act=act)
         assert x.shape[0] == N, 'x has %d rows, graph depth %d has %d nodes' % (x.shape[0], d, N)
         stats = None
         if self.emit_stats and N * self.out_channels >= (1 << 14) and self.out_channels % 4 == 0:
@@ -84,7 +94,7 @@
                 tt = doctree._tf.get(tkey)
                 if tt is None and (nt or bias is not None):
                     tt = doctree._tf[tkey] = pno.type_term(doctree.type_frac(d, nt) if nt else None, nt, N, self.in_channels, bias)
-                return ops.graphconv_narrow_out(x, seg_ptr, col, pno, self.in_channels, tt, out)
+                return ops.graphconv_narrow_out(x, seg_ptr, col, pno, self.in_channels, tt, out, gn=gn)
         if not mode and split_input:
             mode = self.planes_mode(doctree, d)
             if mode:
diff --git a/octfusion_amd/ops.py b/octfusion_amd/ops.py
--- a/octfusion_amd/ops.py
+++ b/octfusion_amd/ops.py
@@ -413,8 +413,23 @@
         return self
 
 
-def gemm(a, pw, bias=None, res=None, out=None, a_rows=None, out_rows=None, m=None, out_planes=0):
+def gemm(a, pw, bias=None, res=None, out=None, a_rows=None, out_rows=None, m=None, out_planes=0, gn=None):
     a, lda = _row_major(a)
+    if gn is not None:
+        assert a_rows is None and out_rows is None and m is None and not out_planes
+        M = a.shape[0]
+        if a.shape[1] != pw.K:
+            raise ValueError('K mismatch: %d vs %d' % (a.shape[1], pw.K))
+        out, ldc = _out2d(out, M, pw.N, a.device)
+        res, ldr = _row_major(res)
+        _chk(bias)
+        ws = workspace(a.device)
+        _meta('dense_gemm', 2.0 * M * pw.K * pw.N, 4.0 * (M * pw.K + pw.K * pw.N + M * pw.N * (2 if res is not None else 1)),
+              (M, pw.K, pw.N, 'gn'))
+        call('ofx_gemm_gn_f32', ptr(a), lda, M, pw.K, ptr(pw.t), pw.Kp, pw.N, ptr(bias), ptr(res), ldr, ptr(out), ldc,
+             ptr(gn.batch_id), ptr(gn.sums), ptr(gn.count), gn.groups, gn.eps, gn.count_eps, ptr(gn.weight), ptr(gn.bias),
+             ACT[gn.act], ptr(ws), ws.numel(), stream())
+        return out
     M = m if m is not None else (a_rows.numel() if a_rows is not None else a.shape[0])
     if a.shape[1] != pw.K:
         raise ValueError('K mismatch: %d vs %d' % (a.shape[1], pw.K))
@@ -653,7 +668,7 @@
         return tt
 
 
-def graphconv_narrow_out(x, seg_ptr, col, pno, C, type_term=None, out=None):
+def graphconv_narrow_out(x, seg_ptr, col, pno, C, type_term=None, out=None, gn=None):
     N = x.shape[0]
     cout = pno.w.shape[1]
     E = col.numel()
@@ -662,7 +677,7 @@
     agg_bytes = 4.0 * (N * pwid + E + 7 * N + 2 * N * cout)
     nbytes = agg_bytes + 4.0 * (N * C + N * pwid + pno.w.numel())
     with _layer_bracket(flops, nbytes, cout, ('graph', N, C, cout)):
-        P = gemm(x, pno.pw.get(pno.wd, 'kn'))
+        P = gemm(x, pno.pw.get(pno.wd, 'kn'), gn=gn)
         out, ldc = _out2d(out, N, cout, x.device)
         _chk(type_term)
         assert type_term is None or (type_term.is_contiguous() and tuple(type_term.shape) == (N, cout))
@@ -793,7 +808,7 @@
         return self
 
 
-def gridconv(x, tables, n_out, pw, bias=None, emb=None, batch_id=None, res=None, out=None):
+def gridconv(x, tables, n_out, pw, bias=None, emb=None, batch_id=None, res=None, out=None, gn=None):
     x, ldx = _row_major(x)
     if x.shape[1] != pw.cin:
         raise ValueError('cin mismatch')
@@ -811,6 +826,13 @@
         _meta('gridconv_27tap', flops,
               4.0 * (x.shape[0] * pw.cin + n_out * pw.N * (2 if res is not None else 1) + 27.0 * pw.cin * pw.N) + 4.0 * 27 * n_out,
               (n_out, pw.cin, pw.N))
+        if gn is not None:
+            assert fast
+            call('ofx_gridconv_gn_fwd', ptr(x), ldx, pw.cin, x.shape[0], n_out, ptr(tables(True)), ptr(zero_row(x.device)),
+                 ptr(pw.t), pw.N, ptr(bias), ptr(emb), lde, ptr(gn.batch_id), ptr(res), ldr, ptr(out), ldc, ptr(gn.sums),
+                 ptr(gn.count), gn.groups, gn.eps, gn.count_eps, ptr(gn.weight), ptr(gn.bias), ACT[gn.act], ptr(ws),
+                 ws.numel(), stream())
+            return out
         call('ofx_gridconv_fwd', ptr(x), ldx, pw.cin, x.shape[0], n_out, None if fast else ptr(tables(False)),
              ptr(tables(True)) if fast else None, ptr(zero_row(x.device)), ptr(pw.t), pw.N, ptr(bias), ptr(emb), lde,
              ptr(batch_id) if emb is not None else None, ptr(res), ldr, ptr(out), ldc, ptr(ws), ws.numel(), stream())
@@ -954,6 +976,52 @@
     return out
 
 
+GN_PROLOGUE_MAX_ACTS = int(os.environ.get('OFX_GN_PROLOGUE_MAX_ACTS', str(1 << 25)))
+
+
+class GnPrologue(NamedTuple):
+    sums: torch.Tensor
+    count: torch.Tensor
+    batch_id: torch.Tensor
+    weight: torch.Tensor
+    bias: torch.Tensor
+    groups: int
+    eps: float
+    count_eps: float
+    act: str
+
+
+def gn_prologue_ok(x, groups, taps=1):
+    n, C = x.shape
+    cpg = C // groups if groups > 0 and C % groups == 0 else 0
+    return (x.dim() == 2 and x.dtype == torch.float32 and x.stride(1) == 1 and x.stride(0) % 4 == 0 and x.data_ptr() % 16 == 0
+            and C % 32 == 0 and C <= 1024 and groups <= 64 and cpg > 0 and cpg & (cpg - 1) == 0
+            and _lib.lib().ofx_get_precision() != PRECISIONS['fp32'] and n * C * taps <= GN_PROLOGUE_MAX_ACTS)
+
+
+def gn_prologue(x, batch_id, count, batch_size, weight, bias, groups, eps=1e-5, act=None, count_eps=None, stats=None):
+    if count_eps is None:
+        count_eps = eps
+    x, ldx = _row_major(x)
+    n, C = x.shape
+    if stats is not None:
+        _chk(stats, torch.float64)
+        assert stats.numel() == batch_size * C * 2
+        sums = stats
+    else:
+        _meta('gn_stats', 0, 4.0 * n * C, (n, C))
+        if stats_pool_has_room(batch_size * C * 2, x.device):
+            sums = stats_zeros(batch_size * C * 2, x.device)
+            call('ofx_gn_stats_acc', ptr(x), ldx, n, C, ptr(batch_id), batch_size, ptr(sums), stream())
+        else:
+            sums = torch.empty(batch_size * C * 2, dtype=torch.float64, device=x.device)
+            call('ofx_gn_stats', ptr(x), ldx, n, C, ptr(batch_id), batch_size, ptr(sums), stream())
+    _chk(count)
+    _chk(batch_id, torch.int32)
+    return GnPrologue(sums, count, batch_id, weight.detach().reshape(-1), bias.detach().reshape(-1), groups,
+                      eps, count_eps, act)
+
+
 def group_norm_backward(x, dy, batch_id, count, batch_size, weight, bias, groups, eps=1e-5, act=None, count_eps=None):
     if count_eps is None:
         count_eps = eps
```

Measured after the change: 115.4. 3.9% lower.
